# cloneofsimo/paint-with-words-sd

Measured on AMD Instinct MI355X. Metric: 512x512 images/sec (30 steps, CFG) SD1.5+PwW, higher is better.
Workload: dtype bf16

## Files before the change

paint-with-words-sd_amd/build.py:

```python
import os
import subprocess
import sys

HERE = os.path.dirname(os.path.abspath(__file__))
REPO = os.path.dirname(HERE)
CSRC = os.path.join(HERE, "csrc")
LIB = os.path.join(HERE, "pww_hip", "libpww_hip.so")
LIB_EXPERIMENTS = os.path.join(HERE, "pww_hip", "libpww_hip_experiments.so")
UNITS = [("pww_api.hip", [], ""), ("pww_attn.hip", [], ""), ("pww_cross.hip", [], ""), ("pww_cross_lean.hip", [], ""), ("pww_reduce.hip", [], ""),
         ("pww_mask.hip", [], ""), ("pww_qproj.hip", [], ""), ("pww_norm.hip", [], ""), ("pww_blocks.hip", [], ""), ("pww_conv.hip", [], ""), ("pww_probs.hip", [], ""),
         ("pww_attn_inst.hip", ["-DPWW_INST_F16"], ".f16"), ("pww_attn_inst.hip", ["-DPWW_INST_BF16"], ".bf16"),
         ("pww_cross_inst.hip", ["-DPWW_INST_F16", "-DPWW_INST_NW=2"], ".f16.nw2"), ("pww_cross_inst.hip", ["-DPWW_INST_F16", "-DPWW_INST_NW=4"], ".f16.nw4"),
         ("pww_cross_inst.hip", ["-DPWW_INST_BF16", "-DPWW_INST_NW=2"], ".bf16.nw2"), ("pww_cross_inst.hip", ["-DPWW_INST_BF16", "-DPWW_INST_NW=4"], ".bf16.nw4")]
EXPERIMENT_UNITS = [("pww_cross_out.hip", [], "")]
_ATTN_HEADERS = ["pww_tile.h", "pww_attn_core.h", "pww_cross_tile.h"]
SIDE_FLAGS = ["-fvisibility=hidden"]
SIDE_LIBS = {
    "long": ("pww_long.hip", _ATTN_HEADERS, "the long-prompt launches"),
    "scope": ("pww_scope.hip", _ATTN_HEADERS, "cross-attention with per-head / per-row score statistics"),
    "linear": ("pww_linear.hip", [], "linear layers with a bias / residual / GEGLU epilogue"),
    "regions": ("pww_regions.hip", [], "region masks and the per-pixel blend of the noise predictions"),
    "lora": ("pww_lora.hip", [], "the per-row low-rank update of unmerged LoRA adapters"),
}
SIDE_LIBS_CONV = {
    "convtail": ("pww_conv_tail.hip", [], "conv2 of a ResnetBlock2D with the 1 x 1 shortcut as further K-slabs"),
}
SIDE_LIBS_EXTRA = {
    "canvas": ("pww_canvas.hip", [], "canvases larger than the UNet's window: the windows' gather and the combine of their noise predictions"),
    "concat": ("pww_concat.hip", [], "the up blocks without torch.cat: GroupNorm and conv2 + shortcut over the two halves of the concatenation"),
    "hold": ("pww_hold.hip", [], "region strength: the strength map, its feather and the per-step hold of the pixels not yet released"),
}
ALL_SIDE_LIBS = {**SIDE_LIBS, **SIDE_LIBS_CONV, **SIDE_LIBS_EXTRA}
SOURCES = sorted({u[0] for u in UNITS + EXPERIMENT_UNITS})
HEADERS = ["pww_common.h", "pww_tile.h", "pww_attn_core.h", "pww_attn_kernel.h", "pww_cross_tile.h", "pww_cross_kernel.h", os.path.join(REPO, "include", "pww_hip.h")]
SIDE_PATHS = {n: os.path.join(HERE, "pww_hip", "libpww_hip_%s.so" % n) for n in ALL_SIDE_LIBS}
SIDE_UNITS = {n: [(v[0], SIDE_FLAGS, "")] for n, v in ALL_SIDE_LIBS.items()}
LIB_LONG, LIB_SCOPE, LIB_LINEAR, LIB_REGIONS, LIB_LORA = (SIDE_PATHS[n] for n in ("long", "scope", "linear", "regions", "lora"))
LONG_UNITS, SCOPE_UNITS, LINEAR_UNITS, REGIONS_UNITS, LORA_UNITS = (SIDE_UNITS[n] for n in ("long", "scope", "linear", "regions", "lora"))
LIB_CONVTAIL, CONVTAIL_UNITS = SIDE_PATHS["convtail"], SIDE_UNITS["convtail"]
LIB_CANVAS, CANVAS_UNITS = SIDE_PATHS["canvas"], SIDE_UNITS["canvas"]
LIB_CONCAT, CONCAT_UNITS = SIDE_PATHS["concat"], SIDE_UNITS["concat"]
LIB_HOLD, HOLD_UNITS = SIDE_PATHS["hold"], SIDE_UNITS["hold"]
SIDE_PUBLIC_HEADERS = {"canvas": ["pww_hip_regions.h"]}
HIPCC = os.environ.get("HIPCC", "/opt/rocm/bin/hipcc")
FLAGS = ["--offload-arch=gfx950", "-O3", "-std=c++17", "-fPIC", "-Wall",
         "-Wno-unused-function", "-mllvm", "-amdgpu-kernarg-preload-count=16"]


PER_FILE_FLAGS = {"pww_mask.hip": ["-ffp-contract=off"], "pww_regions.hip": ["-ffp-contract=off"], "pww_canvas.hip": ["-ffp-contract=off"],
                  "pww_hold.hip": ["-ffp-contract=off"]}


def _newer(target, deps):
    if not os.path.exists(target):
        return True
    t = os.path.getmtime(target)
    return any(os.path.getmtime(d) > t for d in deps)


def _deps():
    return ([os.path.join(CSRC, s) for s in SOURCES] + [h if os.path.isabs(h) else os.path.join(CSRC, h) for h in HEADERS] + [__file__])


def _build(lib, units, defines, objdir, verbose, jobs=None):
    os.makedirs(objdir, exist_ok=True)
    order = sorted(units, key=lambda u: {"pww_cross_inst.hip": 0, "pww_attn_inst.hip": 1, "pww_cross_lean.hip": 2}.get(u[0], 3))
    jobs = jobs or max(2, min(len(order), os.cpu_count() or 4, int(os.environ.get("MAX_JOBS", 16))))
    pending, running, objs = list(order), [], []
    while pending or running:
        while pending and len(running) < jobs:
            src, defs, suffix = pending.pop(0)
            o = os.path.join(objdir, src + suffix + ".o")
            objs.append(o)
            cmd = [HIPCC] + FLAGS + defines + defs + PER_FILE_FLAGS.get(src, []) + ["-c", os.path.join(CSRC, src), "-o", o]
            if verbose:
                print(" ".join(cmd))
            running.append((cmd, subprocess.Popen(cmd, stdout=subprocess.PIPE, stderr=subprocess.STDOUT, text=True)))
        cmd, p = running.pop(0)
        out, _ = p.communicate()
        if p.returncode != 0:
            for _, q in running:
                q.kill()
            raise RuntimeError("hipcc failed: %s\n%s" % (" ".join(cmd), out))
        if verbose and out.strip():
            print(out)
    subprocess.run([HIPCC, "--offload-arch=gfx950", "-shared", "-fPIC", "-s"] + sorted(objs) + ["-o", lib], check=True)
    return lib


def build_lib(force=False, verbose=False):
    if not force and not _newer(LIB, _deps()):
        return LIB
    return _build(LIB, UNITS, [], os.path.join(HERE, "build"), verbose)


def build_experiments(force=False, verbose=False):
    if not force and not _newer(LIB_EXPERIMENTS, _deps()):
        return LIB_EXPERIMENTS
    return _build(LIB_EXPERIMENTS, UNITS + EXPERIMENT_UNITS, ["-DPWW_EXPERIMENTS=1"], os.path.join(HERE, "build", "experiments"), verbose)


def build_side(name, force=False, verbose=False):
    unit, headers, _ = ALL_SIDE_LIBS[name]
    lib = SIDE_PATHS[name]
    public = ["pww_hip.h", "pww_hip_%s.h" % name] + SIDE_PUBLIC_HEADERS.get(name, [])
    deps = [os.path.join(CSRC, f) for f in [unit, "pww_common.h", "pww_side_host.h"] + headers] + [os.path.join(REPO, "include", h) for h in public] + [__file__]
    if not force and not _newer(lib, deps):
        return lib
    return _build(lib, SIDE_UNITS[name], [], os.path.join(HERE, "build", name), verbose)


def build_long(force=False, verbose=False): return build_side("long", force, verbose)
def build_scope(force=False, verbose=False): return build_side("scope", force, verbose)
def build_linear(force=False, verbose=False): return build_side("linear", force, verbose)
def build_regions(force=False, verbose=False): return build_side("regions", force, verbose)
def build_lora(force=False, verbose=False): return build_side("lora", force, verbose)
def build_convtail(force=False, verbose=False): return build_side("convtail", force, verbose)
def build_canvas(force=False, verbose=False): return build_side("canvas", force, verbose)
def build_concat(force=False, verbose=False): return build_side("concat", force, verbose)
def build_hold(force=False, verbose=False): return build_side("hold", force, verbose)


def _build_check(exe, lib, libname, defines, force):
    src = os.path.join(REPO, "tests", "native", "attn_check.cpp")
    if not force and not _newer(exe, [src, lib, os.path.join(REPO, "include", "pww_hip.h")]):
        return exe
    cmd = [HIPCC, "--offload-arch=gfx950", "-O2", "-std=c++17"] + defines + [src, "-o", exe, "-L" + os.path.dirname(lib), "-l" + libname,
                                                                              "-Wl,-rpath,$ORIGIN/../../paint-with-words-sd_amd/pww_hip"]
    subprocess.run(cmd, check=True)
    return exe


def build_native_check(force=False):
    return _build_check(os.path.join(REPO, "tests", "native", "attn_check"), build_lib(), "pww_hip", [], force)


def build_native_check_experiments(force=False):
    return _build_check(os.path.join(REPO, "tests", "native", "attn_check_experiments"), build_experiments(), "pww_hip_experiments", ["-DPWW_EXPERIMENTS=1"], force)


if __name__ == "__main__":
    force = "--force" in sys.argv
    print(build_lib(force=force, verbose=True))
    print(build_native_check(force=force))
    for name in ALL_SIDE_LIBS:
        print(build_side(name, force=force, verbose=True))
    if "--experiments" in sys.argv:
        print(build_experiments(force=force, verbose=True))
        print(build_native_check_experiments(force=force))
```

paint-with-words-sd_amd/csrc/pww_common.h:

```cpp
#pragma once
#include <hip/hip_runtime.h>
#include <hip/hip_ext.h>
#include <stdint.h>
#include <stdio.h>
#include <stdarg.h>
#include "../../include/pww_hip.h"

#ifndef PWW_EXPERIMENTS
#define PWW_EXPERIMENTS 0
#endif

namespace pww {

typedef _Float16 f16;
typedef __bf16 bf16;
typedef float f32x16 __attribute__((ext_vector_type(16)));
typedef _Float16 f16x8 __attribute__((ext_vector_type(8)));
typedef __bf16 bf16x8 __attribute__((ext_vector_type(8)));
typedef unsigned int u32x4 __attribute__((ext_vector_type(4)));
typedef unsigned int u32x2 __attribute__((ext_vector_type(2)));
typedef float f32x4 __attribute__((ext_vector_type(4)));
typedef _Float16 f16x4 __attribute__((ext_vector_type(4)));
typedef __bf16 bf16x4 __attribute__((ext_vector_type(4)));

template <typename T> struct Vec;
template <> struct Vec<f16> { typedef f16x8 v8; typedef f16x4 v4; };
template <> struct Vec<bf16> { typedef bf16x8 v8; typedef bf16x4 v4; };

__device__ __forceinline__ f32x16 mfma32(f16x8 a, f16x8 b, f32x16 c) {
    return __builtin_amdgcn_mfma_f32_32x32x16_f16(a, b, c, 0, 0, 0);
}
__device__ __forceinline__ f32x16 mfma32(bf16x8 a, bf16x8 b, f32x16 c) {
    return __builtin_amdgcn_mfma_f32_32x32x16_bf16(a, b, c, 0, 0, 0);
}

template <typename V8> __device__ __forceinline__ V8 zero8() {
    const u32x4 z = {0u, 0u, 0u, 0u};
    return __builtin_bit_cast(V8, z);
}

__device__ __forceinline__ int swap23(int i) { return (i & ~12) | ((i & 4) << 1) | ((i & 8) >> 1); }

struct DebugKnobs {
    int attn_rf = 1;
    int attn_ksplit = 1;
    int attn_fold = 1;
    int attn_nw8 = 1;
    int attn_pair_major = 16;
    int attn_head_pairs = 2;
    int cross_head_major = 1;
    int attn_wide_store = 1;
    int cross_wg_per_cu = 4;
    int cross_assume_resident = 0;
    int cross_gate_weight = 2;
    int cross_tile_nbuf = 2;
    int cross_bias_lds = 2;
    int cross_lean = 1;
    int cross_lean_multi = 1;
    int cross_lean_nw = 0;
    int attn_ksplit1 = 0;
    int attn_hot_sum = 8;
    int attn_fold_limit_f16 = 0;
    int attn_ksplit_half = 0;
    int attn_ksplit_nw = 2;
};
const DebugKnobs &debug_knobs();

void set_error(const char *fmt, ...);
int check_hip(hipError_t e, const char *what);
bool arch_ok();

bool profile_take(hipEvent_t *start, hipEvent_t *stop, hipStream_t stream);

unsigned long long *debug_timeline();
size_t debug_timeline_bytes();

void record_attn_route(int kind, int ks, int dt, int nw, int kg, int nsub, bool has_bias, bool rowsum_mfma, bool rf);

template <typename K, typename P>
static inline void launch_attn_kernel(K kern, dim3 grid, dim3 block, size_t lds, hipStream_t stream, const P &params) {
    hipEvent_t e0, e1;
    if (profile_take(&e0, &e1, stream)) hipExtLaunchKernelGGL(kern, grid, block, (unsigned)lds, stream, e0, e1, 0, params);
    else hipLaunchKernelGGL(kern, grid, block, lds, stream, params);
}

template <typename K, typename... A>
static inline void launch_timed(K kern, dim3 grid, dim3 block, size_t lds, hipStream_t stream, A... args) {
    hipEvent_t e0, e1;
    if (profile_take(&e0, &e1, stream)) hipExtLaunchKernelGGL(kern, grid, block, (unsigned)lds, stream, e0, e1, 0, args...);
    else hipLaunchKernelGGL(kern, grid, block, lds, stream, args...);
}

}
```

paint-with-words-sd_amd/csrc/pww_concat.hip:

```cpp
#define PWW_SIDE_LIB "libpww_hip_concat"
#include "pww_side_host.h"
#include "../../include/pww_hip_concat.h"

#define PWW_CONCAT_API extern "C" __attribute__((visibility("default")))

namespace pww {

namespace {

constexpr int GN_NT = 256;
constexpr int GN_UN = 8;
constexpr int GN_MAX_SLABS = 64;
constexpr int GN_GROUP_PIECES = 24;

struct CatGnCold {
    const void *gamma, *beta;
    void *y;
    float eps;
};
#define CG_KARGS const void *x1_, const void *x2_, double *partial_, int C1_, int C2_, int HW_, int G_, int cg_, int nslab_, int slab_px_, int apply_px_, const CatGnCold cold_
struct CatGnParams {
    const void *x1, *x2, *gamma, *beta;
    void *y;
    double *partial;
// ... 52 lines not shown
    const T *base = reinterpret_cast<const T *>(second ? p.x2 : p.x1);
    return base + (long)b * p.HW * pitch + (second ? c0 - p.C1 : c0);
}

template <typename T, int NT>
__global__ void __launch_bounds__(NT) cat_gn_moments(CG_KARGS) {
    CG_UNPACK
    extern __shared__ __attribute__((aligned(16))) char smem[];
    typedef typename Vec<T>::v8 V8;
    const int tid = threadIdx.x, b = blockIdx.y, slab = blockIdx.x;
    const int CH = p.C >> 3, PL = NT / CH;
    const int pl = tid / CH, ch = tid - pl * CH;
    float *ls = reinterpret_cast<float *>(smem);
    float *lq = ls + PL * p.C;
    double *lk = reinterpret_cast<double *>(lq + PL * p.C);

    if (pl < PL) {
        float s[8], q[8];
#pragma unroll
        for (int j = 0; j < 8; ++j) s[j] = q[j] = 0.f;
        int pitch;
        const T *x = cat_source<T>(p, b, ch * 8, pitch);
        float c = 0.f;
        const int p0 = slab * p.slab_px, p1 = min(p0 + p.slab_px, p.HW);
#pragma unroll 1
        for (int px = p0 + pl; px < p1; px += GN_UN * PL) {
            V8 r[GN_UN];
#pragma unroll
            for (int u = 0; u < GN_UN; ++u) {
                const int pu = px + u * PL;
                r[u] = *reinterpret_cast<const V8 *>(x + (long)(pu < p1 ? pu : px) * pitch);
            }
            if constexpr (GnPivot<T>::on) {
                if (px == p0 + pl) c = (float)r[0][0];
            }
#pragma unroll
            for (int u = 0; u < GN_UN; ++u) {
                const bool ok = px + u * PL < p1;
#pragma unroll
                for (int j = 0; j < 8; ++j) {
                    float h = (float)r[u][j];
                    if constexpr (GnPivot<T>::on) h -= c;
                    h = ok ? h : 0.f;
                    s[j] += h;
                    q[j] = fmaf(h, h, q[j]);
                }
            }
        }
#pragma unroll
        for (int j = 0; j < 8; ++j) { ls[pl * p.C + ch * 8 + j] = s[j]; lq[pl * p.C + ch * 8 + j] = q[j]; }
        if constexpr (GnPivot<T>::on) reinterpret_cast<float *>(lk + (NT / p.G) * p.G * 2)[tid] = c;
    }
    __syncthreads();
    const int K = NT / p.G, g = tid % p.G, k = tid / p.G;
    if (k < K) {
        double S = 0.0, Q = 0.0;
        const int n = PL * p.cg;
        for (int e = k; e < n; e += K) {
            const int r = e / p.cg, c = g * p.cg + (e - r * p.cg);
            if constexpr (GnPivot<T>::on) {
                const float *lc = reinterpret_cast<const float *>(lk + K * p.G * 2);
                const int p0 = slab * p.slab_px, p1 = min(p0 + p.slab_px, p.HW);
                const int cnt = p0 + r < p1 ? (p1 - p0 - r + PL - 1) / PL : 0;
                unpivot(S, Q, (double)ls[r * p.C + c], (double)lq[r * p.C + c], (double)lc[r * CH + (c >> 3)], (double)cnt);
            } else {
                S += (double)ls[r * p.C + c]; Q += (double)lq[r * p.C + c];
            }
        }
        lk[(k * p.G + g) * 2] = S; lk[(k * p.G + g) * 2 + 1] = Q;
    }
    __syncthreads();
    if (tid < p.G) {
        double S = 0.0, Q = 0.0;
        for (int r = 0; r < K; ++r) { S += lk[(r * p.G + tid) * 2]; Q += lk[(r * p.G + tid) * 2 + 1]; }
        f64x2 v; v[0] = S; v[1] = Q;
        reinterpret_cast<f64x2 *>(p.partial)[((long)b * p.nslab + slab) * p.G + tid] = v;
    }
}

template <typename T, int ACT, int NT>
__global__ void __launch_bounds__(NT) cat_gn_apply(CG_KARGS) {
    CG_UNPACK
    extern __shared__ __attribute__((aligned(16))) char smem[];
    typedef typename Vec<T>::v8 V8;
    constexpr int NPART = 8;
    const int tid = threadIdx.x, b = blockIdx.y;
    const int CH = p.C >> 3, PL = NT / CH;
    const int pl = tid / CH, ch = tid - pl * CH;
    const bool active = pl < PL;
    double *lk = reinterpret_cast<double *>(smem);
    const int K = NT / p.G, g = tid % p.G, k = tid / p.G;
    float *stat = reinterpret_cast<float *>(lk + K * p.G * 2);

    f64x2 part[NPART];
#pragma unroll
    for (int i = 0; i < NPART; ++i) {
        const int sl = k + i * K;
        part[i] = reinterpret_cast<const f64x2 *>(p.partial)[((long)b * p.nslab + (k < K && sl < p.nslab ? sl : 0)) * p.G + g];
    }
    const int c0 = ch * 8;
    V8 gv = zero8<V8>(), bv = zero8<V8>();
    int pitch;
    const T *x = cat_source<T>(p, b, c0, pitch);
    T *y = reinterpret_cast<T *>(p.y) + (long)b * p.HW * p.C + c0;
    const int p0 = blockIdx.x * p.apply_px, p1 = min(p0 + p.apply_px, p.HW);
    V8 r[GN_UN];
    if (active) {
        if (p.gamma) gv = *reinterpret_cast<const V8 *>(reinterpret_cast<const T *>(p.gamma) + c0);
        if (p.beta) bv = *reinterpret_cast<const V8 *>(reinterpret_cast<const T *>(p.beta) + c0);
#pragma unroll
        for (int u = 0; u < GN_UN; ++u) {
            const int pu = p0 + pl + u * PL;
            r[u] = *reinterpret_cast<const V8 *>(x + (long)(pu < p1 ? pu : p0) * pitch);
        }
    }
    if (k < K) {
        double S = 0.0, Q = 0.0;
#pragma unroll
        for (int i = 0; i < NPART; ++i)
            if (k + i * K < p.nslab) { S += part[i][0]; Q += part[i][1]; }
        lk[(k * p.G + g) * 2] = S; lk[(k * p.G + g) * 2 + 1] = Q;
    }
    __syncthreads();
    if (tid < p.G) {
        double S = 0.0, Q = 0.0;
        for (int rr = 0; rr < K; ++rr) { S += lk[(rr * p.G + tid) * 2]; Q += lk[(rr * p.G + tid) * 2 + 1]; }
        float mean, rstd;
        mean_rstd(S, Q, (double)p.cg * (double)p.HW, p.eps, mean, rstd);
        stat[tid * 2] = mean; stat[tid * 2 + 1] = rstd;
    }
    __syncthreads();
    if (!active) return;
    float a[8], bb[8];
#pragma unroll
    for (int j = 0; j < 8; ++j) {
        const int gg = (c0 + j) / p.cg;
        a[j] = stat[gg * 2 + 1] * (p.gamma ? (float)gv[j] : 1.f);
        bb[j] = (p.beta ? (float)bv[j] : 0.f) - a[j] * stat[gg * 2];
    }
    for (int px = p0 + pl; px < p1; px += GN_UN * PL) {
        if (px != p0 + pl) {
#pragma unroll
            for (int u = 0; u < GN_UN; ++u) {
                const int pu = px + u * PL;
                r[u] = *reinterpret_cast<const V8 *>(x + (long)(pu < p1 ? pu : px) * pitch);
            }
        }
#pragma unroll
        for (int u = 0; u < GN_UN; ++u) {
            V8 o;
#pragma unroll
            for (int j = 0; j < 8; ++j) o[j] = (T)finish<T, ACT>((float)r[u][j], a[j], bb[j]);
            if (px + u * PL < p1) *reinterpret_cast<V8 *>(y + (long)(px + u * PL) * p.C) = o;
        }
    }
}

template <typename T, int ACT>
__global__ void __launch_bounds__(GN_NT) cat_gn_group(CG_KARGS) {
    CG_UNPACK
    typedef T TV __attribute__((ext_vector_type(4)));
    __shared__ double red[GN_NT / 64][2];
    const int tid = threadIdx.x, g = blockIdx.x, b = blockIdx.y;
    const int ppp = p.cg >> 2, PLs = GN_NT / ppp;
    const int pl = tid / ppp, sub = tid - pl * ppp;
    const bool active = pl < PLs;
    const int pc = pl < p.HW ? pl : 0;
    const int c0 = g * p.cg + sub * 4;
    int pitch;
    const T *x = cat_source<T>(p, b, c0, pitch);
    T *y = reinterpret_cast<T *>(p.y) + (long)b * p.HW * p.C + c0;
    TV raw[GN_GROUP_PIECES];
    const TV z = {(T)0.f, (T)0.f, (T)0.f, (T)0.f};
    TV gv = z, bv = z;
    if (active) {
#pragma unroll
        for (int j = 0; j < GN_GROUP_PIECES; ++j) {
            const int px = pl + j * PLs;
            raw[j] = *reinterpret_cast<const TV *>(x + (long)(px < p.HW ? px : pc) * pitch);
        }
        if (p.gamma) gv = *reinterpret_cast<const TV *>(reinterpret_cast<const T *>(p.gamma) + c0);
        if (p.beta) bv = *reinterpret_cast<const TV *>(reinterpret_cast<const T *>(p.beta) + c0);
    }
    float v[GN_GROUP_PIECES][4];
    float s = 0.f, q = 0.f, c = 0.f;
    int cnt = 0;
    if (active) {
#pragma unroll
        for (int j = 0; j < GN_GROUP_PIECES; ++j) {
            const bool ok = pl + j * PLs < p.HW;
#pragma unroll
            for (int e = 0; e < 4; ++e) {
                float h = (float)raw[j][e];
                h = ok ? h : 0.f;
                v[j][e] = h;
                if constexpr (GnPivot<T>::on) {
                    if (j == 0 && e == 0) c = h;
                    h = ok ? h - c : 0.f;
                }
                s += h;
                q = fmaf(h, h, q);
            }
            if constexpr (GnPivot<T>::on) cnt += ok ? 4 : 0;
        }
    }
    double S = (double)s, Q = (double)q;
    if constexpr (GnPivot<T>::on) { S = 0.0; Q = 0.0; unpivot(S, Q, (double)s, (double)q, (double)c, (double)cnt); }
    wg_sum(S, Q, red, tid);
    float mean, rstd;
    mean_rstd(S, Q, (double)p.cg * (double)p.HW, p.eps, mean, rstd);
    if (!active) return;
    float a[4], bb[4];
#pragma unroll
    for (int e = 0; e < 4; ++e) {
        a[e] = rstd * (p.gamma ? (float)gv[e] : 1.f);
        bb[e] = (p.beta ? (float)bv[e] : 0.f) - a[e] * mean;
    }
#pragma unroll
    for (int j = 0; j < GN_GROUP_PIECES; ++j) {
        const int px = pl + j * PLs;
        if (px < p.HW) {
            TV o;
#pragma unroll
            for (int e = 0; e < 4; ++e) o[e] = (T)finish<T, ACT>(v[j][e], a[e], bb[e]);
            *reinterpret_cast<TV *>(y + (long)px * p.C) = o;
        }
    }
}

struct CatGnPlan { int nslab, slab_px, apply_px, nt; bool group; size_t partial_bytes, lds_m, lds_a; };

bool desc_ok(const void *d, uint32_t size, size_t want, const char *what) {
    if (d && size >= want) return true;
    set_error("%s: descriptor missing or older than this library (size %u)", what, d ? size : 0u);
    return false;
}

bool cat_gn_plan(const pww_concat_gn_desc_t *d, CatGnPlan &pl) {
    const long C = (long)d->C1 + d->C2;
    const bool ok = d->B >= 1 && d->B <= 65535 && d->C1 >= 8 && d->C2 >= 8 && d->C1 % 8 == 0 && d->C2 % 8 == 0 && C <= 4096 && d->HW >= 8 && d->HW % 8 == 0
                    && d->G >= 1 && d->G <= 32 && C % d->G == 0 && (d->dtype == PWW_DTYPE_F16 || d->dtype == PWW_DTYPE_BF16)
                    && (d->act == PWW_ACT_NONE || d->act == PWW_ACT_SILU) && (long)d->B * d->HW * C < (1L << 40);
    if (!ok) {
        set_error("concat_group_norm: unsupported (dtype %d B %d C1 %d C2 %d HW %d G %d act %d): C1, C2 and HW multiples of 8, (C1 + C2) %% G == 0, "
                  "G <= 32, C1 + C2 <= 4096", d->dtype, d->B, d->C1, d->C2, d->HW, d->G, d->act);
        return false;
    }
    pl = CatGnPlan();
    const int Ct = (int)C, cg = Ct / d->G, CH = Ct / 8;
    pl.nt = CH <= 256 ? 256 : 512;
    const int PL = pl.nt / CH;
    if (cg % 4 == 0 && cg / 4 <= GN_NT) {
        const int PLs = GN_NT / (cg / 4);
        pl.group = (d->HW + PLs - 1) / PLs <= GN_GROUP_PIECES;
    }
    int px = (d->HW + GN_MAX_SLABS - 1) / GN_MAX_SLABS;
    if (px < GN_UN * PL) px = GN_UN * PL;
    if (px > d->HW) px = d->HW;
    pl.slab_px = px;
    pl.nslab = (d->HW + px - 1) / px;
    int want = (512 + d->B - 1) / d->B;
    int apx = (d->HW + want - 1) / want;
    if (apx < GN_UN * PL) apx = GN_UN * PL;
    if (apx > d->HW) apx = d->HW;
    pl.apply_px = apx;
    pl.partial_bytes = (size_t)d->B * pl.nslab * d->G * 2 * sizeof(double);
    const size_t lk = (size_t)(pl.nt / d->G) * d->G * 2 * sizeof(double);
    pl.lds_m = (size_t)2 * PL * Ct * sizeof(float) + lk + (d->dtype == PWW_DTYPE_F16 ? (size_t)pl.nt * sizeof(float) : 0);
    pl.lds_a = lk + (size_t)d->G * 2 * sizeof(float);
    return true;
}

template <typename T>
int cat_gn_launch(const CatGnParams &p, const pww_concat_gn_desc_t *d, const CatGnPlan &pl, hipStream_t stream) {
    const bool silu = d->act == PWW_ACT_SILU;
    if (pl.group) {
        const dim3 grid(d->G, d->B);
        if (silu) hipLaunchKernelGGL((cat_gn_group<T, 1>), grid, dim3(GN_NT), 0, stream, CG_LARGS(p));
        else hipLaunchKernelGGL((cat_gn_group<T, 0>), grid, dim3(GN_NT), 0, stream, CG_LARGS(p));
        return check_hip(hipGetLastError(), "concat_group_norm launch");
    }
    const dim3 gm(pl.nslab, d->B), ga((d->HW + pl.apply_px - 1) / pl.apply_px, d->B);
    if (pl.nt == 256) {
        hipLaunchKernelGGL((cat_gn_moments<T, 256>), gm, dim3(256), pl.lds_m, stream, CG_LARGS(p));
        if (silu) hipLaunchKernelGGL((cat_gn_apply<T, 1, 256>), ga, dim3(256), pl.lds_a, stream, CG_LARGS(p));
        else hipLaunchKernelGGL((cat_gn_apply<T, 0, 256>), ga, dim3(256), pl.lds_a, stream, CG_LARGS(p));
    } else {
        hipLaunchKernelGGL((cat_gn_moments<T, 512>), gm, dim3(512), pl.lds_m, stream, CG_LARGS(p));
        if (silu) hipLaunchKernelGGL((cat_gn_apply<T, 1, 512>), ga, dim3(512), pl.lds_a, stream, CG_LARGS(p));
        else hipLaunchKernelGGL((cat_gn_apply<T, 0, 512>), ga, dim3(512), pl.lds_a, stream, CG_LARGS(p));
    }
    return check_hip(hipGetLastError(), "concat_group_norm launch");
}

constexpr int CT_BM = 128, CT_THREADS = 256;
constexpr int CT_PF = 2;

__device__ __forceinline__ f32x4 mfma16(f16x8 a, f16x8 b, f32x4 c) { return __builtin_amdgcn_mfma_f32_16x16x32_f16(a, b, c, 0, 0, 0); }
__device__ __forceinline__ f32x4 mfma16(bf16x8 a, bf16x8 b, f32x4 c) { return __builtin_amdgcn_mfma_f32_16x16x32_bf16(a, b, c, 0, 0, 0); }

struct CatTailCold {
    const void *x1, *x2, *wsc, *bias, *bias2;
    int nsplit, nmain, ntail;
};

__device__ __forceinline__ int xcd_remap(int orig, int nwg) {
    const int xcd = orig & 7, q = nwg >> 3, r = nwg & 7;
    return (xcd < r ? xcd * (q + 1) : r * (q + 1) + (xcd - r) * q) + (orig >> 3);
}

template <typename T>
__device__ __forceinline__ void epilogue4(const f32x4 &a, const CatTailCold &cold, T *y, long off, int n) {
    typedef typename Vec<T>::v4 V4;
    const V4 b = *reinterpret_cast<const V4 *>(reinterpret_cast<const T *>(cold.bias) + n);
    const V4 b2 = *reinterpret_cast<const V4 *>(reinterpret_cast<const T *>(cold.bias2) + n);
    V4 o;
#pragma unroll
    for (int j = 0; j < 4; ++j) o[j] = (T)(a[j] + (float)b[j] + (float)b2[j]);
    *reinterpret_cast<V4 *>(y + off) = o;
}

template <typename T, int BN>
__global__ void __launch_bounds__(CT_THREADS, 2) cat_tail_kernel(const T *__restrict__ x, const T *__restrict__ w, void *__restrict__ out, int M, int N,
                                                                 int Cin, int C1, int C2, int H, int W, const CatTailCold cold) {
    typedef typename Vec<T>::v8 V8;
    constexpr int BM = CT_BM, PF = CT_PF, XL = BM * 8 / CT_THREADS, WL = BN * 8 / CT_THREADS, RM = 4, RN = BN / 32;
    constexpr int XBYTES = BM * 128, STAGE = (BM + BN) * 128;
    __shared__ __attribute__((aligned(16))) char lds[2 * STAGE];

    const int tid = threadIdx.x, lane = tid & 63, wave = tid >> 6, wm = wave >> 1, wn = wave & 1;
    const int ntm = (M + BM - 1) / BM;
    const int bid = xcd_remap(blockIdx.x, gridDim.x);
    const bool split = cold.nsplit > 1;
    const int tile = bid / cold.nsplit, ks = bid - tile * cold.nsplit;
    const int tm = tile % ntm, tn = tile / ntm;
    const int nmain = cold.nmain, nslab = nmain + cold.ntail;
    const int s_begin = (int)((long)ks * nslab / cold.nsplit), s_end = (int)((long)(ks + 1) * nslab / cold.nsplit);
    const int K9 = 9 * Cin, HW = H * W, Ct = C1 + C2;
    const T *__restrict__ xa = reinterpret_cast<const T *>(cold.x1);
    const T *__restrict__ xb2 = reinterpret_cast<const T *>(cold.x2);
    const T *__restrict__ w2 = reinterpret_cast<const T *>(cold.wsc);

    const int c = tid & 7;
    int pix[XL], y0[XL], x0[XL];
#pragma unroll
    for (int i = 0; i < XL; ++i) {
        int m = tm * BM + (tid >> 3) + 32 * i;
        m = m < M ? m : M - 1;
        const int b = m / HW, rem = m - b * HW, oy = rem / W, ox = rem - oy * W;
        pix[i] = b * HW;
        y0[i] = oy - 1;
        x0[i] = ox - 1;
    }
    const unsigned wrow = (unsigned)(tn * BN + (tid >> 3));
    const unsigned woff_main = wrow * (unsigned)K9 + c * 8, woff_tail = wrow * (unsigned)Ct + c * 8;
    const int swz = ((c ^ ((tid >> 3) & 7)) << 4);

    u32x4 xr[PF][XL], wr[PF][WL];
    unsigned xok[PF];
    const bool tail0 = s_begin >= nmain;
    int tap = tail0 ? 9 : s_begin / (Cin >> 6);
    int ci0 = tail0 ? (s_begin - nmain) << 6 : (s_begin - tap * (Cin >> 6)) << 6;
    int kmain = s_begin * 64;
    const bool second0 = tail0 && ci0 >= C1;
    const T *xs = second0 ? xb2 - C1 : xa;
    int ps = second0 ? C2 : C1;
    auto load = [&](int p) {
        const bool tail = tap >= 9;
        const int ky = tail ? 1 : tap / 3, kx = tail ? 1 : tap - (tap / 3) * 3;
        const T *xb = tail ? xs : x;
        const T *wb = tail ? w2 : w;
        const int pitch = tail ? ps : Cin;
        const unsigned wpitch = (unsigned)(tail ? Ct : K9);
        const unsigned wo = (tail ? woff_tail : woff_main) + (unsigned)(tail ? ci0 : kmain);
        xok[p] = 0;
#pragma unroll
        for (int i = 0; i < XL; ++i) {
            const int iy = y0[i] + ky, ix = x0[i] + kx;
            const bool ok = (unsigned)iy < (unsigned)H && (unsigned)ix < (unsigned)W;
            xr[p][i] = *reinterpret_cast<const u32x4 *>(xb + (unsigned)((pix[i] + (ok ? iy : 0) * W + (ok ? ix : 0)) * pitch + ci0 + c * 8));
            xok[p] |= (unsigned)ok << i;
        }
#pragma unroll
        for (int j = 0; j < WL; ++j) wr[p][j] = *reinterpret_cast<const u32x4 *>(wb + (wo + (unsigned)(32 * j) * wpitch));
        kmain += 64;
        ci0 += 64;
        const bool wrap = ci0 == Cin && !tail;
        ci0 = wrap ? 0 : ci0;
        tap += wrap ? 1 : 0;
        const bool cross = ci0 == C1 && tail;
        xs = cross ? xb2 - C1 : xs;
        ps = cross ? C2 : ps;
    };
    auto store = [&](int p, int buf) {
        char *base = lds + buf * STAGE;
#pragma unroll
        for (int i = 0; i < XL; ++i) {
            const u32x4 z = {0u, 0u, 0u, 0u};
            *reinterpret_cast<u32x4 *>(base + ((tid >> 3) + 32 * i) * 128 + swz) = (xok[p] >> i) & 1u ? xr[p][i] : z;
        }
#pragma unroll
        for (int j = 0; j < WL; ++j) *reinterpret_cast<u32x4 *>(base + XBYTES + ((tid >> 3) + 32 * j) * 128 + swz) = wr[p][j];
    };

    f32x4 acc[RN][RM];
#pragma unroll
    for (int r = 0; r < RN; ++r)
#pragma unroll
        for (int i = 0; i < RM; ++i) acc[r][i] = f32x4{0.f, 0.f, 0.f, 0.f};

    const int fr = lane & 15, fq = lane >> 4;
    auto compute = [&](int buf) {
        const char *bx = lds + buf * STAGE, *bw = bx + XBYTES;
#pragma unroll
        for (int kk = 0; kk < 2; ++kk) {
            V8 xf[RM], wf[RN];
#pragma unroll
            for (int q = 0; q < RM; ++q) {
                const int row = wm * 64 + q * 16 + fr;
                xf[q] = *reinterpret_cast<const V8 *>(bx + row * 128 + (((kk * 4 + fq) ^ (row & 7)) << 4));
            }
#pragma unroll
            for (int r = 0; r < RN; ++r) {
                const int row = wn * (BN / 2) + r * 16 + fr;
                wf[r] = *reinterpret_cast<const V8 *>(bw + row * 128 + (((kk * 4 + fq) ^ (row & 7)) << 4));
            }
#pragma unroll
            for (int r = 0; r < RN; ++r)
#pragma unroll
                for (int q = 0; q < RM; ++q) acc[r][q] = mfma16(wf[r], xf[q], acc[r][q]);
        }
    };

    const int n = s_end - s_begin;
    load(0);
#pragma unroll
    for (int p = 1; p < PF; ++p)
        if (p < n) load(p);
    store(0, 0);
    __syncthreads();
    int i = 0;
    for (; i + 2 * PF <= n; i += PF) {
#pragma unroll
        for (int p = 0; p < PF; ++p) {
            load(p);
            compute((i + p) & 1);
            __builtin_amdgcn_sched_barrier(0);
            store((p + 1) % PF, (i + p + 1) & 1);
            __syncthreads();
        }
    }
#pragma unroll
    for (int t = 0; t < 2 * PF - 1; ++t) {
        if (i + t < n) {
            if (i + t + PF < n) load(t % PF);
            compute((i + t) & 1);
            if (i + t + 1 < n) store((t + 1) % PF, (i + t + 1) & 1);
            __syncthreads();
        }
    }

#pragma unroll
    for (int i = 0; i < RM; ++i) {
        const int m = tm * BM + wm * 64 + i * 16 + fr;
        if (m >= M) continue;
#pragma unroll
        for (int r = 0; r < RN; ++r) {
            const int n = tn * BN + wn * (BN / 2) + r * 16 + fq * 4;
            if (split) *reinterpret_cast<f32x4 *>(reinterpret_cast<float *>(out) + ((long)ks * M + m) * N + n) = acc[r][i];
            else epilogue4<T>(acc[r][i], cold, reinterpret_cast<T *>(out), (long)m * N + n, n);
        }
    }
}

template <typename T>
__global__ void __launch_bounds__(256) cat_tail_fold_kernel(const float *__restrict__ ws, T *__restrict__ y, long n4, int N, long MN, const CatTailCold cold) {
    const long q = (long)blockIdx.x * 256 + threadIdx.x;
    if (q >= n4) return;
    const long off = q * 4;
    f32x4 a = *reinterpret_cast<const f32x4 *>(ws + off);
    for (int s = 1; s < cold.nsplit; ++s) a += *reinterpret_cast<const f32x4 *>(ws + s * MN + off);
    epilogue4<T>(a, cold, y, off, (int)(off % N));
}

struct TailTune { int M, N, nmain, ntail, bn, nsplit; };
constexpr TailTune TAIL_TUNED[] = {
    {128, 1280, 180, 40, 64, 12},
    {512, 1280, 180, 40, 128, 12}, {512, 1280, 180, 30, 128, 12}, {512, 1280, 180, 10, 128, 12},
    {2048, 640, 90, 30, 128, 6}, {2048, 640, 90, 20, 128, 6}, {2048, 640, 90, 15, 128, 6}, {2048, 640, 90, 5, 128, 6},
    {8192, 320, 45, 15, 64, 4}, {8192, 320, 45, 10, 64, 4},
};

struct TailPlan {
    int M, bn, nsplit, nmain, ntail, ntiles;
};

bool cat_tail_plan(const pww_concat_tail_desc_t *d, TailPlan *p) {
    if ((d->dtype != PWW_DTYPE_F16 && d->dtype != PWW_DTYPE_BF16) || d->B < 1 || d->H < 1 || d->W < 1 || d->Cin < 64 || d->Cin % 64 != 0 || d->C1 < 64
        || d->C1 % 64 != 0 || d->C2 < 64 || d->C2 % 64 != 0 || d->Cout < 64 || d->Cout % 64 != 0 || d->Cin > 65536 || d->C1 > 32768 || d->C2 > 32768
        || d->Cout > 65536) {
        set_error("concat_convtail: unsupported (dtype %d B %d %dx%d Cin %d C1 %d C2 %d Cout %d): Cin, C1, C2 and Cout multiples of 64", d->dtype, d->B,
                  d->H, d->W, d->Cin, d->C1, d->C2, d->Cout);
        return false;
    }
    const long M = (long)d->B * d->H * d->W, Ct = (long)d->C1 + d->C2;
    if (M * d->Cin >= (1L << 31) || M * Ct >= (1L << 31) || M * d->Cout >= (1L << 31) || 9L * d->Cin * d->Cout >= (1L << 31) || Ct * d->Cout >= (1L << 31)) {
        set_error("concat_convtail: tensor of 2^31 elements or more");
        return false;
    }
    p->M = (int)M;
    p->nmain = 9 * d->Cin / 64;
    p->ntail = (int)(Ct / 64);
    const int nslab = p->nmain + p->ntail;
    const TailTune *tuned = nullptr;
    for (const TailTune &t : TAIL_TUNED)
        if (t.M == p->M && t.N == d->Cout && t.nmain == p->nmain && t.ntail == p->ntail) tuned = &t;
    p->bn = d->tile_n ? d->tile_n : tuned ? tuned->bn : (d->Cout % 128 == 0 ? 128 : 64);
    if ((p->bn != 64 && p->bn != 128) || d->Cout % p->bn != 0) { set_error("concat_convtail: tile_n %d does not divide Cout %d", d->tile_n, d->Cout); return false; }
    p->ntiles = (p->M + CT_BM - 1) / CT_BM * (d->Cout / p->bn);
    int ns = d->splitk;
    if (ns <= 0 && tuned && p->bn == tuned->bn) ns = tuned->nsplit;
    if (ns <= 0) {
        ns = (480 + p->ntiles / 2) / p->ntiles;
        if (ns > nslab / 8) ns = nslab / 8;
        if (ns < 1) ns = 1;
    }
    if (ns > nslab || ns > 64) { set_error("concat_convtail: split %d exceeds the %d K-slabs (or 64)", ns, nslab); return false; }
    p->nsplit = ns;
    return true;
}

template <typename T>
int cat_tail_launch(const TailPlan &p, const pww_concat_tail_desc_t *d, const void *x, const void *w, const CatTailCold &cold, void *y, void *ws,
                    hipStream_t stream) {
    const T *xt = static_cast<const T *>(x), *wt = static_cast<const T *>(w);
    const int N = d->Cout;
    const dim3 grid(p.ntiles * p.nsplit), block(CT_THREADS);
    void *out = p.nsplit == 1 ? y : ws;
    if (p.bn == 128) launch_timed(cat_tail_kernel<T, 128>, grid, block, 0, stream, xt, wt, out, p.M, N, d->Cin, d->C1, d->C2, d->H, d->W, cold);
    else launch_timed(cat_tail_kernel<T, 64>, grid, block, 0, stream, xt, wt, out, p.M, N, d->Cin, d->C1, d->C2, d->H, d->W, cold);
    if (p.nsplit == 1) return check_hip(hipGetLastError(), "concat_convtail launch");
    const long MN = (long)p.M * N, n4 = MN / 4;
    launch_timed(cat_tail_fold_kernel<T>, dim3((unsigned)((n4 + 255) / 256)), dim3(256), 0, stream, static_cast<const float *>(ws), static_cast<T *>(y), n4,
                 N, MN, cold);
    return check_hip(hipGetLastError(), "concat_convtail fold launch");
}

}

size_t concat_group_norm_workspace_bytes(const pww_concat_gn_desc_t *d) {
    CatGnPlan pl;
    if (!desc_ok(d, d ? d->size : 0u, sizeof(pww_concat_gn_desc_t), "concat_group_norm") || !cat_gn_plan(d, pl)) return 0;
    return pl.group ? 16 : pl.partial_bytes;
}

int concat_group_norm_fwd(const void *x1, const void *x2, const void *gamma, const void *beta, void *y, const pww_concat_gn_desc_t *d, void *workspace,
                          size_t workspace_bytes, hipStream_t stream) {
    if (!desc_ok(d, d ? d->size : 0u, sizeof(pww_concat_gn_desc_t), "concat_group_norm")) return PWW_EINVAL;
    CatGnPlan pl;
    if (!cat_gn_plan(d, pl)) return PWW_ENOTSUP;
    if (!x1 || !x2 || !y || !workspace) { set_error("concat_group_norm: x1, x2, y and workspace are required"); return PWW_EINVAL; }
    if (!aligned16(x1) || !aligned16(x2) || !aligned16(y) || !aligned16(workspace) || !aligned16(gamma) || !aligned16(beta)) {
        set_error("concat_group_norm: pointers must be 16-byte aligned");
        return PWW_EINVAL;
    }
    const size_t need = pl.group ? 16 : pl.partial_bytes;
    if (workspace_bytes < need) { set_error("concat_group_norm: workspace of %zu bytes, need %zu", workspace_bytes, need); return PWW_EINVAL; }
    if (!arch_ok()) return PWW_ENOTSUP;
    CatGnParams p;
    p.x1 = x1; p.x2 = x2; p.gamma = gamma; p.beta = beta; p.y = y;
    p.partial = static_cast<double *>(workspace);
    p.C1 = d->C1; p.C2 = d->C2; p.C = d->C1 + d->C2; p.HW = d->HW; p.G = d->G; p.cg = p.C / d->G;
    p.nslab = pl.nslab; p.slab_px = pl.slab_px; p.apply_px = pl.apply_px;
    p.eps = d->eps;
    return d->dtype == PWW_DTYPE_F16 ? cat_gn_launch<f16>(p, d, pl, stream) : cat_gn_launch<bf16>(p, d, pl, stream);
}

size_t concat_convtail_workspace_bytes(const pww_concat_tail_desc_t *d) {
    TailPlan p;
    if (!desc_ok(d, d ? d->size : 0u, sizeof(pww_concat_tail_desc_t), "concat_convtail") || !cat_tail_plan(d, &p)) return 0;
    return p.nsplit > 1 ? (size_t)p.nsplit * p.M * d->Cout * sizeof(float) : 0;
}

int concat_convtail_fwd(const void *x, const void *w, const void *x1, const void *x2, const void *wsc, const void *bias, const void *bias2, void *y,
                        const pww_concat_tail_desc_t *d, void *workspace, size_t workspace_bytes, hipStream_t stream) {
    if (!desc_ok(d, d ? d->size : 0u, sizeof(pww_concat_tail_desc_t), "concat_convtail")) return PWW_EINVAL;
    TailPlan p;
    if (!cat_tail_plan(d, &p)) return PWW_ENOTSUP;
    if (!x || !w || !x1 || !x2 || !wsc || !bias || !bias2 || !y) { set_error("concat_convtail: x, w, x1, x2, wsc, bias, bias2 and y are required"); return PWW_EINVAL; }
    if (!aligned16(x) || !aligned16(w) || !aligned16(x1) || !aligned16(x2) || !aligned16(wsc) || !aligned16(y) || (reinterpret_cast<uintptr_t>(bias) & 7)
        || (reinterpret_cast<uintptr_t>(bias2) & 7)) {
        set_error("concat_convtail: x, w, x1, x2, wsc, y must be 16-byte aligned, the biases 8-byte aligned");
        return PWW_EINVAL;
    }
    const size_t need = p.nsplit > 1 ? (size_t)p.nsplit * p.M * d->Cout * sizeof(float) : 0;
    if (need && (!workspace || !aligned16(workspace) || workspace_bytes < need)) {
        set_error("concat_convtail: split %d needs a 16-byte aligned workspace of %zu bytes (got %zu)", p.nsplit, need, workspace_bytes);
        return PWW_EINVAL;
    }
    if (!arch_ok()) return PWW_ENOTSUP;
    const CatTailCold cold{x1, x2, wsc, bias, bias2, p.nsplit, p.nmain, p.ntail};
    if (d->dtype == PWW_DTYPE_F16) return cat_tail_launch<f16>(p, d, x, w, cold, y, workspace, stream);
    return cat_tail_launch<bf16>(p, d, x, w, cold, y, workspace, stream);
}

}

PWW_CONCAT_API int pww_concat_version(void) { return PWW_CONCAT_VERSION; }
PWW_CONCAT_API const char *pww_concat_last_error(void) { return pww::last_error(); }
PWW_CONCAT_API size_t pww_concat_group_norm_workspace_bytes(const pww_concat_gn_desc_t *desc) { return pww::concat_group_norm_workspace_bytes(desc); }
PWW_CONCAT_API int pww_concat_group_norm_fwd(const void *x1, const void *x2, const void *gamma, const void *beta, void *y, const pww_concat_gn_desc_t *desc,
                                             void *workspace, size_t workspace_bytes, void *stream) {
    return pww::concat_group_norm_fwd(x1, x2, gamma, beta, y, desc, workspace, workspace_bytes, static_cast<hipStream_t>(stream));
}
PWW_CONCAT_API size_t pww_concat_convtail_workspace_bytes(const pww_concat_tail_desc_t *desc) { return pww::concat_convtail_workspace_bytes(desc); }
PWW_CONCAT_API int pww_concat_convtail_fwd(const void *x, const void *w, const void *x1, const void *x2, const void *wsc, const void *bias, const void *bias2,
                                           void *y, const pww_concat_tail_desc_t *desc, void *workspace, size_t workspace_bytes, void *stream) {
    return pww::concat_convtail_fwd(x, w, x1, x2, wsc, bias, bias2, y, desc, workspace, workspace_bytes, static_cast<hipStream_t>(stream));
}
```

paint-with-words-sd_amd/csrc/pww_conv.hip:

```cpp
#include "pww_common.h"

namespace pww {

namespace {

constexpr int CV_BM = 128, CV_THREADS = 256;
constexpr int CV_PF = 2;

__device__ __forceinline__ f32x4 mfma16(f16x8 a, f16x8 b, f32x4 c) { return __builtin_amdgcn_mfma_f32_16x16x32_f16(a, b, c, 0, 0, 0); }
__device__ __forceinline__ f32x4 mfma16(bf16x8 a, bf16x8 b, f32x4 c) { return __builtin_amdgcn_mfma_f32_16x16x32_bf16(a, b, c, 0, 0, 0); }

struct ConvCold {
    const void *bias, *residual;
    int nsplit, nslab;
};

__device__ __forceinline__ int xcd_remap(int orig, int nwg) {
    const int xcd = orig & 7, q = nwg >> 3, r = nwg & 7;
    return (xcd < r ? xcd * (q + 1) : r * (q + 1) + (xcd - r) * q) + (orig >> 3);
}

template <typename T>
__device__ __forceinline__ void epilogue4(const f32x4 &a, const ConvCold &cold, T *y, long off, int n) {
    typedef typename Vec<T>::v4 V4;
    V4 o;
#pragma unroll
    for (int j = 0; j < 4; ++j) o[j] = (T)a[j];
    if (cold.bias) {
        const V4 b = *reinterpret_cast<const V4 *>(reinterpret_cast<const T *>(cold.bias) + n);
#pragma unroll
        for (int j = 0; j < 4; ++j) o[j] = (T)((float)o[j] + (float)b[j]);
    }
    if (cold.residual) {
        const V4 r = *reinterpret_cast<const V4 *>(reinterpret_cast<const T *>(cold.residual) + off);
#pragma unroll
        for (int j = 0; j < 4; ++j) o[j] = (T)((float)r[j] + (float)o[j]);
    }
    *reinterpret_cast<V4 *>(y + off) = o;
}

template <typename T, int BN>
__global__ void __launch_bounds__(CV_THREADS, 2) conv3x3_kernel(const T *__restrict__ x, const T *__restrict__ w, void *__restrict__ out, int M, int N,
                                                            int Cin, int Hin, int Win, int Wo, int HWo, const ConvCold cold) {
    typedef typename Vec<T>::v8 V8;
    constexpr int BM = CV_BM, PF = CV_PF, XL = BM * 8 / CV_THREADS, WL = BN * 8 / CV_THREADS, RM = 4, RN = BN / 32;
    constexpr int XBYTES = BM * 128, STAGE = (BM + BN) * 128;
    __shared__ __attribute__((aligned(16))) char lds[2 * STAGE];

    const int geo = cold.nslab >> 24;
    const int nslab = cold.nslab & 0xffffff;
    const int stride = geo & 15, up = geo >> 4;
    const int Hv = Hin << up, Wv = Win << up;
    const int tid = threadIdx.x, lane = tid & 63, wave = tid >> 6, wm = wave >> 1, wn = wave & 1;
    const int ntm = (M + BM - 1) / BM;
    const int bid = xcd_remap(blockIdx.x, gridDim.x);
    const bool split = cold.nsplit > 1;
    const int tile = bid / cold.nsplit, ks = bid - tile * cold.nsplit;
    const int tm = tile % ntm, tn = tile / ntm;
    const int s_begin = (int)((long)ks * nslab / cold.nsplit), s_end = (int)((long)(ks + 1) * nslab / cold.nsplit);
    const int K9 = 9 * Cin;

    const int c = tid & 7;
    int pix[XL], y0[XL], x0[XL];
#pragma unroll
    for (int i = 0; i < XL; ++i) {
        int m = tm * BM + (tid >> 3) + 32 * i;
        m = m < M ? m : M - 1;
        const int b = m / HWo, rem = m - b * HWo, oy = rem / Wo, ox = rem - oy * Wo;
        pix[i] = b * Hin * Win;
        y0[i] = oy * stride - 1;
        x0[i] = ox * stride - 1;
    }
    const T *wrow = w + (long)(tn * BN + (tid >> 3)) * K9 + c * 8;
    const int swz = ((c ^ ((tid >> 3) & 7)) << 4);

    u32x4 xr[PF][XL], wr[PF][WL];
    unsigned xok[PF];
    int tap = s_begin / (Cin >> 6), ci0 = (s_begin - tap * (Cin >> 6)) << 6;
    const T *wnext = wrow + s_begin * 64;
    auto load = [&](int p) {
        const int ky = tap / 3, kx = tap - ky * 3;
        xok[p] = 0;
#pragma unroll
        for (int i = 0; i < XL; ++i) {
            const int iyv = y0[i] + ky, ixv = x0[i] + kx;
            const bool ok = (unsigned)iyv < (unsigned)Hv && (unsigned)ixv < (unsigned)Wv;
            const int iy = ok ? iyv >> up : 0, ix = ok ? ixv >> up : 0;
            xr[p][i] = *reinterpret_cast<const u32x4 *>(x + (unsigned)((pix[i] + iy * Win + ix) * Cin + ci0 + c * 8));
            xok[p] |= (unsigned)ok << i;
        }
#pragma unroll
        for (int j = 0; j < WL; ++j) wr[p][j] = *reinterpret_cast<const u32x4 *>(wnext + (long)(32 * j) * K9);
        wnext += 64;
        ci0 += 64;
        if (ci0 == Cin) { ci0 = 0; ++tap; }
    };
    auto store = [&](int p, int buf) {
        char *base = lds + buf * STAGE;
#pragma unroll
        for (int i = 0; i < XL; ++i) {
            const u32x4 z = {0u, 0u, 0u, 0u};
            *reinterpret_cast<u32x4 *>(base + ((tid >> 3) + 32 * i) * 128 + swz) = (xok[p] >> i) & 1u ? xr[p][i] : z;
        }
#pragma unroll
        for (int j = 0; j < WL; ++j) *reinterpret_cast<u32x4 *>(base + XBYTES + ((tid >> 3) + 32 * j) * 128 + swz) = wr[p][j];
    };

    f32x4 acc[RN][RM];
#pragma unroll
    for (int r = 0; r < RN; ++r)
#pragma unroll
        for (int i = 0; i < RM; ++i) acc[r][i] = f32x4{0.f, 0.f, 0.f, 0.f};

    const int fr = lane & 15, fq = lane >> 4;
    auto compute = [&](int buf) {
        const char *bx = lds + buf * STAGE, *bw = bx + XBYTES;
#pragma unroll
        for (int kk = 0; kk < 2; ++kk) {
            V8 xf[RM], wf[RN];
#pragma unroll
            for (int q = 0; q < RM; ++q) {
                const int row = wm * 64 + q * 16 + fr;
                xf[q] = *reinterpret_cast<const V8 *>(bx + row * 128 + (((kk * 4 + fq) ^ (row & 7)) << 4));
            }
#pragma unroll
            for (int r = 0; r < RN; ++r) {
                const int row = wn * (BN / 2) + r * 16 + fr;
                wf[r] = *reinterpret_cast<const V8 *>(bw + row * 128 + (((kk * 4 + fq) ^ (row & 7)) << 4));
            }
#pragma unroll
            for (int r = 0; r < RN; ++r)
#pragma unroll
                for (int q = 0; q < RM; ++q) acc[r][q] = mfma16(wf[r], xf[q], acc[r][q]);
        }
    };

    const int n = s_end - s_begin;
    load(0);
#pragma unroll
    for (int p = 1; p < PF; ++p)
        if (p < n) load(p);
    store(0, 0);
    __syncthreads();
    int i = 0;
    for (; i + 2 * PF <= n; i += PF) {
#pragma unroll
        for (int p = 0; p < PF; ++p) {
            load(p);
            compute((i + p) & 1);
            store((p + 1) % PF, (i + p + 1) & 1);
            __syncthreads();
        }
    }
#pragma unroll
    for (int t = 0; t < 2 * PF - 1; ++t) {
        if (i + t < n) {
            if (i + t + PF < n) load(t % PF);
            compute((i + t) & 1);
            if (i + t + 1 < n) store((t + 1) % PF, (i + t + 1) & 1);
            __syncthreads();
        }
    }

#pragma unroll
    for (int i = 0; i < RM; ++i) {
        const int m = tm * BM + wm * 64 + i * 16 + fr;
        if (m >= M) continue;
#pragma unroll
        for (int r = 0; r < RN; ++r) {
            const int n = tn * BN + wn * (BN / 2) + r * 16 + fq * 4;
            if (split) *reinterpret_cast<f32x4 *>(reinterpret_cast<float *>(out) + ((long)ks * M + m) * N + n) = acc[r][i];
            else epilogue4<T>(acc[r][i], cold, reinterpret_cast<T *>(out), (long)m * N + n, n);
        }
    }
}

template <typename T>
__global__ void __launch_bounds__(256) conv3x3_fold_kernel(const float *__restrict__ ws, T *__restrict__ y, long n4, int N, long MN, const ConvCold cold) {
    const long q = (long)blockIdx.x * 256 + threadIdx.x;
    if (q >= n4) return;
    const long off = q * 4;
    f32x4 a = *reinterpret_cast<const f32x4 *>(ws + off);
    for (int s = 1; s < cold.nsplit; ++s) a += *reinterpret_cast<const f32x4 *>(ws + s * MN + off);
    epilogue4<T>(a, cold, y, off, (int)(off % N));
}

struct ConvTune { int M, N, nslab, bn, nsplit; };
constexpr ConvTune CONV_TUNED[] = {
    {8192, 320, 45, 64, 3}, {8192, 320, 90, 64, 4}, {8192, 320, 135, 64, 3}, {8192, 640, 90, 128, 3},
    {2048, 320, 45, 64, 6}, {2048, 640, 45, 64, 3}, {2048, 640, 90, 128, 6}, {2048, 640, 135, 128, 6}, {2048, 640, 180, 128, 6},
    {2048, 640, 270, 128, 6}, {2048, 1280, 180, 128, 3},
    {512, 640, 90, 64, 6}, {512, 1280, 90, 128, 6}, {512, 1280, 180, 128, 12}, {512, 1280, 270, 128, 12}, {512, 1280, 360, 128, 12},
    {128, 1280, 180, 64, 12}, {128, 1280, 360, 64, 24},
    {65536, 640, 90, 128, 1}, {16384, 1280, 180, 128, 1},
    {4096, 640, 90, 128, 3}, {4096, 1280, 90, 128, 3}, {4096, 1280, 180, 128, 3}, {4096, 1280, 270, 128, 3}, {4096, 1280, 360, 128, 3},
    {1024, 1280, 180, 128, 6}, {1024, 1280, 360, 128, 6},
};

struct ConvPlan {
    int M, Ho, Wo, bn, nsplit, nslab, ntiles;
};

bool plan_conv(const pww_conv_desc_t *d, ConvPlan *p) {
    if (!d || d->size < sizeof(pww_conv_desc_t)) { set_error("conv3x3: descriptor missing or older than this library (size %u)", d ? d->size : 0u); return false; }
    const int up = d->upsample, s = d->stride;
    if ((d->dtype != PWW_DTYPE_F16 && d->dtype != PWW_DTYPE_BF16) || d->B < 1 || d->Hin < 1 || d->Win < 1 || d->Cin < 64 || d->Cin % 64 != 0
        || d->Cout < 64 || d->Cout % 64 != 0 || (s != 1 && s != 2) || (up != 0 && up != 1) || (up && s != 1) || d->Cin > 65536 || d->Cout > 65536) {
        set_error("conv3x3: unsupported (dtype %d B %d %dx%d Cin %d Cout %d stride %d upsample %d): Cin and Cout multiples of 64, stride 1 or 2, "
                  "upsample only at stride 1", d->dtype, d->B, d->Hin, d->Win, d->Cin, d->Cout, s, up);
        return false;
    }
    const int Hv = d->Hin << up, Wv = d->Win << up;
    p->Ho = (Hv - 1) / s + 1;
    p->Wo = (Wv - 1) / s + 1;
    const long M = (long)d->B * p->Ho * p->Wo;
    if ((long)d->B * d->Hin * d->Win * d->Cin >= (1L << 31) || M * d->Cout >= (1L << 31)) { set_error("conv3x3: tensor of 2^31 elements or more"); return false; }
    p->M = (int)M;
    p->nslab = 9 * d->Cin / 64;
    const ConvTune *tuned = nullptr;
    for (const ConvTune &t : CONV_TUNED)
        if (t.M == p->M && t.N == d->Cout && t.nslab == p->nslab) tuned = &t;
    p->bn = d->tile_n ? d->tile_n : tuned ? tuned->bn : (d->Cout % 128 == 0 ? 128 : 64);
    if ((p->bn != 64 && p->bn != 128) || d->Cout % p->bn != 0) { set_error("conv3x3: tile_n %d does not divide Cout %d", d->tile_n, d->Cout); return false; }
    p->ntiles = (p->M + CV_BM - 1) / CV_BM * (d->Cout / p->bn);
    int ns = d->splitk;
    if (ns <= 0 && tuned && p->bn == tuned->bn) ns = tuned->nsplit;
    if (ns <= 0) {
        ns = (480 + p->ntiles / 2) / p->ntiles;
        if (ns > p->nslab / 8) ns = p->nslab / 8;
        if (ns < 1) ns = 1;
    }
    if (ns > p->nslab || ns > 64) { set_error("conv3x3: split %d exceeds the %d K-slabs (or 64)", ns, p->nslab); return false; }
    p->nsplit = ns;
    return true;
}

template <typename T>
int conv_launch(const ConvPlan &p, const pww_conv_desc_t *d, const void *x, const void *w, const void *bias, const void *residual, void *y, void *ws,
                hipStream_t stream) {
    ConvCold cold{bias, residual, p.nsplit, p.nslab | ((d->stride | (d->upsample << 4)) << 24)};
    const T *xt = static_cast<const T *>(x), *wt = static_cast<const T *>(w);
    const int N = d->Cout, HWo = p.Ho * p.Wo;
    const dim3 grid(p.ntiles * p.nsplit), block(CV_THREADS);
    void *out = p.nsplit == 1 ? y : ws;
    if (p.bn == 128) launch_timed(conv3x3_kernel<T, 128>, grid, block, 0, stream, xt, wt, out, p.M, N, d->Cin, d->Hin, d->Win, p.Wo, HWo, cold);
    else launch_timed(conv3x3_kernel<T, 64>, grid, block, 0, stream, xt, wt, out, p.M, N, d->Cin, d->Hin, d->Win, p.Wo, HWo, cold);
    if (p.nsplit == 1) return check_hip(hipGetLastError(), "conv3x3 launch");
    const long MN = (long)p.M * N, n4 = MN / 4;
    launch_timed(conv3x3_fold_kernel<T>, dim3((unsigned)((n4 + 255) / 256)), dim3(256), 0, stream, static_cast<const float *>(ws), static_cast<T *>(y), n4,
                 N, MN, cold);
    return check_hip(hipGetLastError(), "conv3x3 fold launch");
}

bool al16(const void *a) { return (reinterpret_cast<uintptr_t>(a) & 15) == 0; }

}

size_t conv3x3_workspace_bytes(const pww_conv_desc_t *d) {
    ConvPlan p;
    if (!plan_conv(d, &p)) return 0;
    return p.nsplit > 1 ? (size_t)p.nsplit * p.M * d->Cout * sizeof(float) : 0;
}

int conv3x3_fwd(const void *x, const void *w, const void *bias, const void *residual, void *y, const pww_conv_desc_t *d, void *workspace,
                size_t workspace_bytes, hipStream_t stream) {
    ConvPlan p;
    if (!plan_conv(d, &p)) return PWW_ENOTSUP;
    if (!x || !w || !y) { set_error("conv3x3: x, w and y are required"); return PWW_EINVAL; }
    if (!al16(x) || !al16(w) || !al16(y) || (reinterpret_cast<uintptr_t>(bias) & 7) || (reinterpret_cast<uintptr_t>(residual) & 7)) {
        set_error("conv3x3: x, w, y must be 16-byte aligned, bias and residual 8-byte aligned");
        return PWW_EINVAL;
    }
    if (p.nsplit > 1 && (!workspace || !al16(workspace) || workspace_bytes < (size_t)p.nsplit * p.M * d->Cout * sizeof(float))) {
        set_error("conv3x3: split %d needs a 16-byte aligned workspace of %zu bytes (got %zu)", p.nsplit, (size_t)p.nsplit * p.M * d->Cout * sizeof(float),
                  workspace_bytes);
        return PWW_EINVAL;
    }
    if (!arch_ok()) return PWW_ENOTSUP;
    if (d->dtype == PWW_DTYPE_F16) return conv_launch<f16>(p, d, x, w, bias, residual, y, workspace, stream);
    return conv_launch<bf16>(p, d, x, w, bias, residual, y, workspace, stream);
}

}
```

paint-with-words-sd_amd/csrc/pww_conv_tail.hip:

```cpp
#define PWW_SIDE_LIB "libpww_hip_convtail"
#include "pww_side_host.h"
#include "../../include/pww_hip_convtail.h"

#define PWW_CONVTAIL_API extern "C" __attribute__((visibility("default")))

namespace pww {

namespace {

constexpr int CT_BM = 128, CT_THREADS = 256;
constexpr int CT_PF = 2;

__device__ __forceinline__ f32x4 mfma16(f16x8 a, f16x8 b, f32x4 c) { return __builtin_amdgcn_mfma_f32_16x16x32_f16(a, b, c, 0, 0, 0); }
__device__ __forceinline__ f32x4 mfma16(bf16x8 a, bf16x8 b, f32x4 c) { return __builtin_amdgcn_mfma_f32_16x16x32_bf16(a, b, c, 0, 0, 0); }

struct TailCold {
    const void *x2, *w2, *bias, *bias2;
    int nsplit, nmain, ntail;
};

__device__ __forceinline__ int xcd_remap(int orig, int nwg) {
    const int xcd = orig & 7, q = nwg >> 3, r = nwg & 7;
    return (xcd < r ? xcd * (q + 1) : r * (q + 1) + (xcd - r) * q) + (orig >> 3);
}

template <typename T>
__device__ __forceinline__ void epilogue4(const f32x4 &a, const TailCold &cold, T *y, long off, int n) {
    typedef typename Vec<T>::v4 V4;
    const V4 b = *reinterpret_cast<const V4 *>(reinterpret_cast<const T *>(cold.bias) + n);
    const V4 b2 = *reinterpret_cast<const V4 *>(reinterpret_cast<const T *>(cold.bias2) + n);
    V4 o;
#pragma unroll
    for (int j = 0; j < 4; ++j) o[j] = (T)(a[j] + (float)b[j] + (float)b2[j]);
    *reinterpret_cast<V4 *>(y + off) = o;
}

template <typename T, int BN>
__global__ void __launch_bounds__(CT_THREADS, 2) convtail_kernel(const T *__restrict__ x, const T *__restrict__ w, void *__restrict__ out, int M, int N,
                                                                 int Cin, int C2, int H, int W, const TailCold cold) {
    typedef typename Vec<T>::v8 V8;
    constexpr int BM = CT_BM, PF = CT_PF, XL = BM * 8 / CT_THREADS, WL = BN * 8 / CT_THREADS, RM = 4, RN = BN / 32;
    constexpr int XBYTES = BM * 128, STAGE = (BM + BN) * 128;
    __shared__ __attribute__((aligned(16))) char lds[2 * STAGE];

    const int tid = threadIdx.x, lane = tid & 63, wave = tid >> 6, wm = wave >> 1, wn = wave & 1;
    const int ntm = (M + BM - 1) / BM;
    const int bid = xcd_remap(blockIdx.x, gridDim.x);
    const bool split = cold.nsplit > 1;
    const int tile = bid / cold.nsplit, ks = bid - tile * cold.nsplit;
    const int tm = tile % ntm, tn = tile / ntm;
    const int nmain = cold.nmain, nslab = nmain + cold.ntail;
    const int s_begin = (int)((long)ks * nslab / cold.nsplit), s_end = (int)((long)(ks + 1) * nslab / cold.nsplit);
    const int K9 = 9 * Cin, HW = H * W;
    const T *__restrict__ x2 = reinterpret_cast<const T *>(cold.x2);
    const T *__restrict__ w2 = reinterpret_cast<const T *>(cold.w2);

    const int c = tid & 7;
    int pix[XL], y0[XL], x0[XL];
#pragma unroll
    for (int i = 0; i < XL; ++i) {
        int m = tm * BM + (tid >> 3) + 32 * i;
        m = m < M ? m : M - 1;
        const int b = m / HW, rem = m - b * HW, oy = rem / W, ox = rem - oy * W;
        pix[i] = b * HW;
        y0[i] = oy - 1;
        x0[i] = ox - 1;
    }
    const unsigned wrow = (unsigned)(tn * BN + (tid >> 3));
    const unsigned woff_main = wrow * (unsigned)K9 + c * 8, woff_tail = wrow * (unsigned)C2 + c * 8;
    const int swz = ((c ^ ((tid >> 3) & 7)) << 4);

    u32x4 xr[PF][XL], wr[PF][WL];
    unsigned xok[PF];
    const bool tail0 = s_begin >= nmain;
    int tap = tail0 ? 9 : s_begin / (Cin >> 6);
    int ci0 = tail0 ? (s_begin - nmain) << 6 : (s_begin - tap * (Cin >> 6)) << 6;
    int kmain = s_begin * 64;
    auto load = [&](int p) {
        const bool tail = tap >= 9;
        const int ky = tail ? 1 : tap / 3, kx = tail ? 1 : tap - (tap / 3) * 3;
        const T *xb = tail ? x2 : x;
        const T *wb = tail ? w2 : w;
        const int pitch = tail ? C2 : Cin;
        const unsigned wpitch = (unsigned)(tail ? C2 : K9);
        const unsigned wo = (tail ? woff_tail : woff_main) + (unsigned)(tail ? ci0 : kmain);
        xok[p] = 0;
#pragma unroll
        for (int i = 0; i < XL; ++i) {
            const int iy = y0[i] + ky, ix = x0[i] + kx;
            const bool ok = (unsigned)iy < (unsigned)H && (unsigned)ix < (unsigned)W;
            xr[p][i] = *reinterpret_cast<const u32x4 *>(xb + (unsigned)((pix[i] + (ok ? iy : 0) * W + (ok ? ix : 0)) * pitch + ci0 + c * 8));
            xok[p] |= (unsigned)ok << i;
        }
#pragma unroll
        for (int j = 0; j < WL; ++j) wr[p][j] = *reinterpret_cast<const u32x4 *>(wb + (wo + (unsigned)(32 * j) * wpitch));
        kmain += 64;
        ci0 += 64;
        const bool wrap = ci0 == Cin && !tail;
        ci0 = wrap ? 0 : ci0;
        tap += wrap ? 1 : 0;
    };
    auto store = [&](int p, int buf) {
        char *base = lds + buf * STAGE;
#pragma unroll
        for (int i = 0; i < XL; ++i) {
            const u32x4 z = {0u, 0u, 0u, 0u};
            *reinterpret_cast<u32x4 *>(base + ((tid >> 3) + 32 * i) * 128 + swz) = (xok[p] >> i) & 1u ? xr[p][i] : z;
        }
#pragma unroll
        for (int j = 0; j < WL; ++j) *reinterpret_cast<u32x4 *>(base + XBYTES + ((tid >> 3) + 32 * j) * 128 + swz) = wr[p][j];
    };

    f32x4 acc[RN][RM];
#pragma unroll
    for (int r = 0; r < RN; ++r)
#pragma unroll
        for (int i = 0; i < RM; ++i) acc[r][i] = f32x4{0.f, 0.f, 0.f, 0.f};

    const int fr = lane & 15, fq = lane >> 4;
    auto compute = [&](int buf) {
        const char *bx = lds + buf * STAGE, *bw = bx + XBYTES;
#pragma unroll
        for (int kk = 0; kk < 2; ++kk) {
            V8 xf[RM], wf[RN];
#pragma unroll
            for (int q = 0; q < RM; ++q) {
                const int row = wm * 64 + q * 16 + fr;
                xf[q] = *reinterpret_cast<const V8 *>(bx + row * 128 + (((kk * 4 + fq) ^ (row & 7)) << 4));
            }
#pragma unroll
            for (int r = 0; r < RN; ++r) {
                const int row = wn * (BN / 2) + r * 16 + fr;
                wf[r] = *reinterpret_cast<const V8 *>(bw + row * 128 + (((kk * 4 + fq) ^ (row & 7)) << 4));
            }
#pragma unroll
            for (int r = 0; r < RN; ++r)
#pragma unroll
                for (int q = 0; q < RM; ++q) acc[r][q] = mfma16(wf[r], xf[q], acc[r][q]);
        }
    };

    const int n = s_end - s_begin;
    load(0);
#pragma unroll
    for (int p = 1; p < PF; ++p)
        if (p < n) load(p);
    store(0, 0);
    __syncthreads();
    int i = 0;
    for (; i + 2 * PF <= n; i += PF) {
#pragma unroll
        for (int p = 0; p < PF; ++p) {
            load(p);
            compute((i + p) & 1);
            __builtin_amdgcn_sched_barrier(0);
            store((p + 1) % PF, (i + p + 1) & 1);
            __syncthreads();
        }
    }
#pragma unroll
    for (int t = 0; t < 2 * PF - 1; ++t) {
        if (i + t < n) {
            if (i + t + PF < n) load(t % PF);
            compute((i + t) & 1);
            if (i + t + 1 < n) store((t + 1) % PF, (i + t + 1) & 1);
            __syncthreads();
        }
    }

#pragma unroll
    for (int i = 0; i < RM; ++i) {
        const int m = tm * BM + wm * 64 + i * 16 + fr;
        if (m >= M) continue;
#pragma unroll
        for (int r = 0; r < RN; ++r) {
            const int n = tn * BN + wn * (BN / 2) + r * 16 + fq * 4;
            if (split) *reinterpret_cast<f32x4 *>(reinterpret_cast<float *>(out) + ((long)ks * M + m) * N + n) = acc[r][i];
            else epilogue4<T>(acc[r][i], cold, reinterpret_cast<T *>(out), (long)m * N + n, n);
        }
    }
}

template <typename T>
__global__ void __launch_bounds__(256) convtail_fold_kernel(const float *__restrict__ ws, T *__restrict__ y, long n4, int N, long MN, const TailCold cold) {
    const long q = (long)blockIdx.x * 256 + threadIdx.x;
    if (q >= n4) return;
    const long off = q * 4;
    f32x4 a = *reinterpret_cast<const f32x4 *>(ws + off);
    for (int s = 1; s < cold.nsplit; ++s) a += *reinterpret_cast<const f32x4 *>(ws + s * MN + off);
    epilogue4<T>(a, cold, y, off, (int)(off % N));
}

struct TailTune { int M, N, nmain, ntail, bn, nsplit; };
constexpr TailTune TAIL_TUNED[] = {
    {128, 1280, 180, 40, 64, 12},
    {512, 1280, 180, 40, 128, 12}, {512, 1280, 180, 30, 128, 12}, {512, 1280, 180, 10, 128, 12},
    {2048, 640, 90, 30, 128, 6}, {2048, 640, 90, 20, 128, 6}, {2048, 640, 90, 15, 128, 6}, {2048, 640, 90, 5, 128, 6},
    {8192, 320, 45, 15, 64, 4}, {8192, 320, 45, 10, 64, 4},
};

struct TailPlan {
    int M, bn, nsplit, nmain, ntail, ntiles;
};

bool plan_tail(const pww_convtail_desc_t *d, TailPlan *p) {
    if (!d || d->size < sizeof(pww_convtail_desc_t)) { set_error("convtail: descriptor missing or older than this library (size %u)", d ? d->size : 0u); return false; }
    if ((d->dtype != PWW_DTYPE_F16 && d->dtype != PWW_DTYPE_BF16) || d->B < 1 || d->H < 1 || d->W < 1 || d->Cin < 64 || d->Cin % 64 != 0 || d->C2 < 64
        || d->C2 % 64 != 0 || d->Cout < 64 || d->Cout % 64 != 0 || d->Cin > 65536 || d->C2 > 65536 || d->Cout > 65536) {
        set_error("convtail: unsupported (dtype %d B %d %dx%d Cin %d C2 %d Cout %d): Cin, C2 and Cout multiples of 64", d->dtype, d->B, d->H, d->W, d->Cin,
                  d->C2, d->Cout);
        return false;
    }
    const long M = (long)d->B * d->H * d->W;
    if (M * d->Cin >= (1L << 31) || M * d->C2 >= (1L << 31) || M * d->Cout >= (1L << 31) || 9L * d->Cin * d->Cout >= (1L << 31)
        || (long)d->C2 * d->Cout >= (1L << 31)) {
        set_error("convtail: tensor of 2^31 elements or more");
        return false;
    }
    p->M = (int)M;
    p->nmain = 9 * d->Cin / 64;
    p->ntail = d->C2 / 64;
    const int nslab = p->nmain + p->ntail;
    const TailTune *tuned = nullptr;
    for (const TailTune &t : TAIL_TUNED)
        if (t.M == p->M && t.N == d->Cout && t.nmain == p->nmain && t.ntail == p->ntail) tuned = &t;
    p->bn = d->tile_n ? d->tile_n : tuned ? tuned->bn : (d->Cout % 128 == 0 ? 128 : 64);
    if ((p->bn != 64 && p->bn != 128) || d->Cout % p->bn != 0) { set_error("convtail: tile_n %d does not divide Cout %d", d->tile_n, d->Cout); return false; }
    p->ntiles = (p->M + CT_BM - 1) / CT_BM * (d->Cout / p->bn);
    int ns = d->splitk;
    if (ns <= 0 && tuned && p->bn == tuned->bn) ns = tuned->nsplit;
    if (ns <= 0) {
        ns = (480 + p->ntiles / 2) / p->ntiles;
        if (ns > nslab / 8) ns = nslab / 8;
        if (ns < 1) ns = 1;
    }
    if (ns > nslab || ns > 64) { set_error("convtail: split %d exceeds the %d K-slabs (or 64)", ns, nslab); return false; }
    p->nsplit = ns;
    return true;
}

template <typename T>
int tail_launch(const TailPlan &p, const pww_convtail_desc_t *d, const void *x, const void *w, const void *x2, const void *w2, const void *bias,
                const void *bias2, void *y, void *ws, hipStream_t stream) {
    TailCold cold{x2, w2, bias, bias2, p.nsplit, p.nmain, p.ntail};
    const T *xt = static_cast<const T *>(x), *wt = static_cast<const T *>(w);
    const int N = d->Cout;
    const dim3 grid(p.ntiles * p.nsplit), block(CT_THREADS);
    void *out = p.nsplit == 1 ? y : ws;
    if (p.bn == 128) launch_timed(convtail_kernel<T, 128>, grid, block, 0, stream, xt, wt, out, p.M, N, d->Cin, d->C2, d->H, d->W, cold);
    else launch_timed(convtail_kernel<T, 64>, grid, block, 0, stream, xt, wt, out, p.M, N, d->Cin, d->C2, d->H, d->W, cold);
    if (p.nsplit == 1) return check_hip(hipGetLastError(), "convtail launch");
    const long MN = (long)p.M * N, n4 = MN / 4;
    launch_timed(convtail_fold_kernel<T>, dim3((unsigned)((n4 + 255) / 256)), dim3(256), 0, stream, static_cast<const float *>(ws), static_cast<T *>(y), n4,
                 N, MN, cold);
    return check_hip(hipGetLastError(), "convtail fold launch");
}

}

size_t convtail_workspace_bytes(const pww_convtail_desc_t *d) {
    TailPlan p;
    if (!plan_tail(d, &p)) return 0;
    return p.nsplit > 1 ? (size_t)p.nsplit * p.M * d->Cout * sizeof(float) : 0;
}

int convtail_fwd(const void *x, const void *w, const void *x2, const void *w2, const void *bias, const void *bias2, void *y, const pww_convtail_desc_t *d,
                 void *workspace, size_t workspace_bytes, hipStream_t stream) {
    if (!d || d->size < sizeof(pww_convtail_desc_t)) { set_error("convtail: descriptor missing or older than this library (size %u)", d ? d->size : 0u); return PWW_EINVAL; }
    TailPlan p;
    if (!plan_tail(d, &p)) return PWW_ENOTSUP;
    if (!x || !w || !x2 || !w2 || !bias || !bias2 || !y) { set_error("convtail: x, w, x2, w2, bias, bias2 and y are required"); return PWW_EINVAL; }
    if (!aligned16(x) || !aligned16(w) || !aligned16(x2) || !aligned16(w2) || !aligned16(y) || (reinterpret_cast<uintptr_t>(bias) & 7)
        || (reinterpret_cast<uintptr_t>(bias2) & 7)) {
        set_error("convtail: x, w, x2, w2, y must be 16-byte aligned, the biases 8-byte aligned");
        return PWW_EINVAL;
    }
    const size_t need = p.nsplit > 1 ? (size_t)p.nsplit * p.M * d->Cout * sizeof(float) : 0;
    if (need && (!workspace || !aligned16(workspace) || workspace_bytes < need)) {
        set_error("convtail: split %d needs a 16-byte aligned workspace of %zu bytes (got %zu)", p.nsplit, need, workspace_bytes);
        return PWW_EINVAL;
    }
    if (!arch_ok()) return PWW_ENOTSUP;
    if (d->dtype == PWW_DTYPE_F16) return tail_launch<f16>(p, d, x, w, x2, w2, bias, bias2, y, workspace, stream);
    return tail_launch<bf16>(p, d, x, w, x2, w2, bias, bias2, y, workspace, stream);
}

}

PWW_CONVTAIL_API int pww_convtail_version(void) { return PWW_CONVTAIL_VERSION; }
PWW_CONVTAIL_API const char *pww_convtail_last_error(void) { return pww::last_error(); }
PWW_CONVTAIL_API size_t pww_convtail_workspace_bytes(const pww_convtail_desc_t *desc) { return pww::convtail_workspace_bytes(desc); }
PWW_CONVTAIL_API int pww_convtail_fwd(const void *x, const void *w, const void *x2, const void *w2, const void *bias, const void *bias2, void *y,
                                      const pww_convtail_desc_t *desc, void *workspace, size_t workspace_bytes, void *stream) {
    return pww::convtail_fwd(x, w, x2, w2, bias, bias2, y, desc, workspace, workspace_bytes, static_cast<hipStream_t>(stream));
}
```

paint-with-words-sd_amd/csrc/pww_linear.hip:

```cpp
#define PWW_SIDE_LIB "libpww_hip_linear"
#include "pww_side_host.h"
#include "../../include/pww_hip_linear.h"

#define PWW_LINEAR_API extern "C" __attribute__((visibility("default")))

namespace pww {

namespace {

constexpr int LN_BM = 128, LN_THREADS = 256;
constexpr int LN_PF = 2;

__device__ __forceinline__ f32x4 mfma16(f16x8 a, f16x8 b, f32x4 c) { return __builtin_amdgcn_mfma_f32_16x16x32_f16(a, b, c, 0, 0, 0); }
__device__ __forceinline__ f32x4 mfma16(bf16x8 a, bf16x8 b, f32x4 c) { return __builtin_amdgcn_mfma_f32_16x16x32_bf16(a, b, c, 0, 0, 0); }

struct LinCold {
    const void *bias, *residual;
    long ys, rs;
    int nsplit, nslab, mode, inner;
};

__device__ __forceinline__ int xcd_remap(int orig, int nwg) {
    const int xcd = orig & 7, q = nwg >> 3, r = nwg & 7;
    return (xcd < r ? xcd * (q + 1) : r * (q + 1) + (xcd - r) * q) + (orig >> 3);
}

template <typename T> __device__ __forceinline__ float rnd(float v) { return (float)(T)v; }

template <typename T>
__device__ __forceinline__ void epilogue4(const f32x4 &a, const LinCold &cold, T *y, int m, int n) {
    typedef typename Vec<T>::v4 V4;
    V4 o;
#pragma unroll
    for (int j = 0; j < 4; ++j) o[j] = (T)a[j];
    if (cold.mode >= PWW_LINEAR_BIAS) {
        const V4 b = *reinterpret_cast<const V4 *>(reinterpret_cast<const T *>(cold.bias) + n);
#pragma unroll
        for (int j = 0; j < 4; ++j) o[j] = (T)((float)o[j] + (float)b[j]);
    }
    if (cold.mode == PWW_LINEAR_BIAS_RESIDUAL) {
        const V4 r = *reinterpret_cast<const V4 *>(reinterpret_cast<const T *>(cold.residual) + (long)m * cold.rs + n);
#pragma unroll
        for (int j = 0; j < 4; ++j) o[j] = (T)((float)r[j] + (float)o[j]);
    }
    *reinterpret_cast<V4 *>(y + (long)m * cold.ys + n) = o;
}

template <typename T>
__device__ __forceinline__ void geglu4(const f32x4 &av, const f32x4 &ag, const LinCold &cold, T *y, int m, int j0) {
    typedef typename Vec<T>::v4 V4;
    const V4 bv = *reinterpret_cast<const V4 *>(reinterpret_cast<const T *>(cold.bias) + j0);
    const V4 bg = *reinterpret_cast<const V4 *>(reinterpret_cast<const T *>(cold.bias) + cold.inner + j0);
    V4 o;
#pragma unroll
    for (int j = 0; j < 4; ++j) {
        const float hv = rnd<T>(rnd<T>(av[j]) + (float)bv[j]);
        const float g = rnd<T>(rnd<T>(ag[j]) + (float)bg[j]);
        const float ge = rnd<T>(0.5f * g * (1.f + erff(g * 0.70710678118654752440f)));
        o[j] = (T)(hv * ge);
    }
    *reinterpret_cast<V4 *>(y + (long)m * cold.ys + j0) = o;
}

template <typename T, int BN>
__global__ void __launch_bounds__(LN_THREADS, 2) linear_kernel(const T *__restrict__ x, const T *__restrict__ w, void *out, int M, int N, int K, int xs,
                                                               const LinCold cold) {
    typedef typename Vec<T>::v8 V8;
    constexpr int BM = LN_BM, PF = LN_PF, XL = BM * 8 / LN_THREADS, WL = BN * 8 / LN_THREADS, RM = 4, RN = BN / 32;
    constexpr int XBYTES = BM * 128, STAGE = (BM + BN) * 128;
    __shared__ __attribute__((aligned(16))) char lds[2 * STAGE];

    const int tid = threadIdx.x, lane = tid & 63, wave = tid >> 6, wm = wave >> 1, wn = wave & 1;
    const int ntm = (M + BM - 1) / BM;
    const int bid = xcd_remap(blockIdx.x, gridDim.x);
    const bool split = cold.nsplit > 1;
    const bool geglu = cold.mode == PWW_LINEAR_BIAS_GEGLU;
    const int tile = bid / cold.nsplit, ks = bid - tile * cold.nsplit;
    const int tm = tile % ntm, tn = tile / ntm;
    const int s_begin = (int)((long)ks * cold.nslab / cold.nsplit), s_end = (int)((long)(ks + 1) * cold.nslab / cold.nsplit);

    const int c = tid & 7;
    unsigned xoff[XL], woff[WL];
#pragma unroll
    for (int i = 0; i < XL; ++i) {
        int m = tm * BM + (tid >> 3) + 32 * i;
        m = m < M ? m : M - 1;
        xoff[i] = (unsigned)(m * xs + c * 8);
    }
#pragma unroll
    for (int j = 0; j < WL; ++j) {
        const int t = (tid >> 3) + 32 * j;
        const int u = t % (BN / 2);
        const int row = geglu ? (u >= BN / 4 ? cold.inner : 0) + tn * (BN / 2) + (t / (BN / 2)) * (BN / 4) + u % (BN / 4) : tn * BN + t;
        woff[j] = (unsigned)(row * K + c * 8);
    }
    const int swz = ((c ^ ((tid >> 3) & 7)) << 4);

    u32x4 xr[PF][XL], wr[PF][WL];
    const T *xnext = x + s_begin * 64, *wnext = w + s_begin * 64;
    auto load = [&](int p) {
#pragma unroll
        for (int i = 0; i < XL; ++i) xr[p][i] = *reinterpret_cast<const u32x4 *>(xnext + xoff[i]);
#pragma unroll
        for (int j = 0; j < WL; ++j) wr[p][j] = *reinterpret_cast<const u32x4 *>(wnext + woff[j]);
        xnext += 64;
        wnext += 64;
    };
    auto store = [&](int p, int buf) {
        char *base = lds + buf * STAGE;
#pragma unroll
        for (int i = 0; i < XL; ++i) *reinterpret_cast<u32x4 *>(base + ((tid >> 3) + 32 * i) * 128 + swz) = xr[p][i];
#pragma unroll
        for (int j = 0; j < WL; ++j) *reinterpret_cast<u32x4 *>(base + XBYTES + ((tid >> 3) + 32 * j) * 128 + swz) = wr[p][j];
    };

    f32x4 acc[RN][RM];
#pragma unroll
    for (int r = 0; r < RN; ++r)
#pragma unroll
        for (int i = 0; i < RM; ++i) acc[r][i] = f32x4{0.f, 0.f, 0.f, 0.f};

    const int fr = lane & 15, fq = lane >> 4;
    auto compute = [&](int buf) {
        const char *bx = lds + buf * STAGE, *bw = bx + XBYTES;
#pragma unroll
        for (int kk = 0; kk < 2; ++kk) {
            V8 xf[RM], wf[RN];
#pragma unroll
            for (int q = 0; q < RM; ++q) {
                const int row = wm * 64 + q * 16 + fr;
                xf[q] = *reinterpret_cast<const V8 *>(bx + row * 128 + (((kk * 4 + fq) ^ (row & 7)) << 4));
            }
#pragma unroll
            for (int r = 0; r < RN; ++r) {
                const int row = wn * (BN / 2) + r * 16 + fr;
                wf[r] = *reinterpret_cast<const V8 *>(bw + row * 128 + (((kk * 4 + fq) ^ (row & 7)) << 4));
            }
#pragma unroll
            for (int r = 0; r < RN; ++r)
#pragma unroll
                for (int q = 0; q < RM; ++q) acc[r][q] = mfma16(wf[r], xf[q], acc[r][q]);
        }
    };

    const int n = s_end - s_begin;
    load(0);
#pragma unroll
    for (int p = 1; p < PF; ++p)
        if (p < n) load(p);
    store(0, 0);
    __syncthreads();
    int i = 0;
    for (; i + 2 * PF <= n; i += PF) {
#pragma unroll
        for (int p = 0; p < PF; ++p) {
            load(p);
            compute((i + p) & 1);
            store((p + 1) % PF, (i + p + 1) & 1);
            __syncthreads();
        }
    }
#pragma unroll
    for (int t = 0; t < 2 * PF - 1; ++t) {
        if (i + t < n) {
            if (i + t + PF < n) load(t % PF);
            compute((i + t) & 1);
            if (i + t + 1 < n) store((t + 1) % PF, (i + t + 1) & 1);
            __syncthreads();
        }
    }

#pragma unroll
    for (int i = 0; i < RM; ++i) {
        const int m = tm * BM + wm * 64 + i * 16 + fr;
        if (m >= M) continue;
        if (split) {
#pragma unroll
            for (int r = 0; r < RN; ++r) {
                const int col = geglu ? (r >= RN / 2 ? cold.inner : 0) + tn * (BN / 2) + wn * (BN / 4) + (r % (RN / 2)) * 16 + fq * 4
                                      : tn * BN + wn * (BN / 2) + r * 16 + fq * 4;
                *reinterpret_cast<f32x4 *>(reinterpret_cast<float *>(out) + ((long)ks * M + m) * N + col) = acc[r][i];
            }
        } else if (geglu) {
#pragma unroll
            for (int r = 0; r < RN / 2; ++r)
                geglu4<T>(acc[r][i], acc[r + RN / 2][i], cold, reinterpret_cast<T *>(out), m, tn * (BN / 2) + wn * (BN / 4) + r * 16 + fq * 4);
        } else {
#pragma unroll
            for (int r = 0; r < RN; ++r) epilogue4<T>(acc[r][i], cold, reinterpret_cast<T *>(out), m, tn * BN + wn * (BN / 2) + r * 16 + fq * 4);
        }
    }
}

template <typename T>
__global__ void __launch_bounds__(256) linear_fold_kernel(const float *__restrict__ ws, T *y, long n4, int N, long MN, const LinCold cold) {
    const long q = (long)blockIdx.x * 256 + threadIdx.x;
    if (q >= n4) return;
    const bool geglu = cold.mode == PWW_LINEAR_BIAS_GEGLU;
    const int nout = geglu ? cold.inner : N;
    const long o4 = q * 4;
    const int m = (int)(o4 / nout), n = (int)(o4 - (long)m * nout);
    const float *p = ws + (long)m * N + n;
    f32x4 a = *reinterpret_cast<const f32x4 *>(p);
    for (int s = 1; s < cold.nsplit; ++s) a += *reinterpret_cast<const f32x4 *>(p + s * MN);
    if (geglu) {
        f32x4 g = *reinterpret_cast<const f32x4 *>(p + cold.inner);
        for (int s = 1; s < cold.nsplit; ++s) g += *reinterpret_cast<const f32x4 *>(p + s * MN + cold.inner);
        geglu4<T>(a, g, cold, y, m, n);
    } else {
        epilogue4<T>(a, cold, y, m, n);
    }
}

struct LinTune { int M, N, nslab, geglu, bn, nsplit; };
constexpr LinTune LIN_TUNED[] = {
    {8192, 2560, 5, 1, 64, 1}, {2048, 5120, 10, 1, 64, 1}, {512, 10240, 20, 1, 64, 1}, {128, 10240, 20, 1, 64, 1},
    {8192, 320, 20, 0, 64, 1}, {8192, 320, 5, 0, 64, 1}, {2048, 640, 40, 0, 128, 3}, {2048, 640, 10, 0, 64, 1},
    {512, 1280, 80, 0, 64, 3}, {512, 1280, 20, 0, 64, 2}, {128, 1280, 80, 0, 64, 5}, {128, 1280, 20, 0, 64, 4},
};

struct LinPlan {
    int bn, nsplit, nslab, ntiles, nout;
    long xs, ys, rs;
};

bool plan_linear(const pww_linear_desc_t *d, LinPlan *p) {
    if (!d || d->size < sizeof(pww_linear_desc_t)) { set_error("linear: descriptor missing or older than this library (size %u)", d ? d->size : 0u); return false; }
    const int e = d->epilogue;
    const bool geglu = e == PWW_LINEAR_BIAS_GEGLU;
    if ((d->dtype != PWW_DTYPE_F16 && d->dtype != PWW_DTYPE_BF16) || d->M < 1 || d->K < 64 || d->K % 64 != 0 || d->N < 64 || d->N % 64 != 0
        || e < PWW_LINEAR_NONE || e > PWW_LINEAR_BIAS_GEGLU || (geglu && d->N % 128 != 0)) {
        set_error("linear: unsupported (dtype %d M %d N %d K %d epilogue %d): K and N multiples of 64, GEGLU's inner = N / 2 a multiple of 64", d->dtype,
                  d->M, d->N, d->K, e);
        return false;
    }
    p->nout = geglu ? d->N / 2 : d->N;
    p->xs = d->x_stride ? d->x_stride : d->K;
    p->ys = d->y_stride ? d->y_stride : p->nout;
    p->rs = d->r_stride ? d->r_stride : p->nout;
    if (p->xs < d->K || p->ys < p->nout || p->rs < p->nout || ((p->xs | p->ys | p->rs) & 7)) {
        set_error("linear: row strides must cover their rows and be multiples of 8 elements (x %ld y %ld r %ld)", p->xs, p->ys, p->rs);
        return false;
    }
    if ((long)d->M * p->xs >= (1L << 31) || (long)d->N * d->K >= (1L << 31) || (long)d->M * d->N >= (1L << 31)) { set_error("linear: tensor of 2^31 elements or more"); return false; }
    p->nslab = d->K / 64;
    const LinTune *tuned = nullptr;
    for (const LinTune &t : LIN_TUNED)
        if (t.M == d->M && t.N == d->N && t.nslab == p->nslab && t.geglu == (int)geglu) tuned = &t;
    p->bn = d->tile_n ? d->tile_n : tuned ? tuned->bn : (d->N % 128 == 0 ? 128 : 64);
    if ((p->bn != 64 && p->bn != 128) || d->N % p->bn != 0) { set_error("linear: tile_n %d does not divide N %d", d->tile_n, d->N); return false; }
    p->ntiles = (d->M + LN_BM - 1) / LN_BM * (d->N / p->bn);
    int ns = d->splitk;
    if (ns <= 0 && tuned && p->bn == tuned->bn) ns = tuned->nsplit;
    if (ns <= 0) {
        ns = (480 + p->ntiles / 2) / p->ntiles;
        if (ns > p->nslab / 4) ns = p->nslab / 4;
        if (ns < 1) ns = 1;
    }
    if (ns > p->nslab || ns > 64) { set_error("linear: split %d exceeds the %d K-slabs (or 64)", ns, p->nslab); return false; }
    p->nsplit = ns;
    return true;
}

template <typename T>
int linear_launch(const LinPlan &p, const pww_linear_desc_t *d, const void *x, const void *w, const void *bias, const void *residual, void *y, void *ws,
                  hipStream_t stream) {
    LinCold cold{bias, residual, p.ys, p.rs, p.nsplit, p.nslab, d->epilogue, d->N / 2};
    const T *xt = static_cast<const T *>(x), *wt = static_cast<const T *>(w);
    const dim3 grid(p.ntiles * p.nsplit), block(LN_THREADS);
    void *out = p.nsplit == 1 ? y : ws;
    if (p.bn == 128) launch_timed(linear_kernel<T, 128>, grid, block, 0, stream, xt, wt, out, d->M, d->N, d->K, (int)p.xs, cold);
    else launch_timed(linear_kernel<T, 64>, grid, block, 0, stream, xt, wt, out, d->M, d->N, d->K, (int)p.xs, cold);
    if (p.nsplit == 1) return check_hip(hipGetLastError(), "linear launch");
    const long MN = (long)d->M * d->N, n4 = (long)d->M * p.nout / 4;
    launch_timed(linear_fold_kernel<T>, dim3((unsigned)((n4 + 255) / 256)), dim3(256), 0, stream, static_cast<const float *>(ws), static_cast<T *>(y), n4,
                 d->N, MN, cold);
    return check_hip(hipGetLastError(), "linear fold launch");
}

bool al16(const void *a) { return (reinterpret_cast<uintptr_t>(a) & 15) == 0; }

}

size_t linear_workspace_bytes(const pww_linear_desc_t *d) {
    LinPlan p;
    if (!plan_linear(d, &p)) return 0;
    return p.nsplit > 1 ? (size_t)p.nsplit * d->M * d->N * sizeof(float) : 0;
}

int linear_fwd(const void *x, const void *w, const void *bias, const void *residual, void *y, const pww_linear_desc_t *d, void *workspace,
               size_t workspace_bytes, hipStream_t stream) {
    LinPlan p;
    if (!plan_linear(d, &p)) return PWW_ENOTSUP;
    if (!x || !w || !y) { set_error("linear: x, w and y are required"); return PWW_EINVAL; }
    if ((d->epilogue >= PWW_LINEAR_BIAS && !bias) || (d->epilogue == PWW_LINEAR_BIAS_RESIDUAL && !residual)) {
        set_error("linear: epilogue %d needs its bias%s", d->epilogue, d->epilogue == PWW_LINEAR_BIAS_RESIDUAL ? " and residual" : "");
        return PWW_EINVAL;
    }
    if (!al16(x) || !al16(w) || !al16(y) || (reinterpret_cast<uintptr_t>(bias) & 7) || (reinterpret_cast<uintptr_t>(residual) & 7)) {
        set_error("linear: x, w, y must be 16-byte aligned, bias and residual 8-byte aligned");
        return PWW_EINVAL;
    }
    const size_t need = p.nsplit > 1 ? (size_t)p.nsplit * d->M * d->N * sizeof(float) : 0;
    if (need && (!workspace || !al16(workspace) || workspace_bytes < need)) {
        set_error("linear: split %d needs a 16-byte aligned workspace of %zu bytes (got %zu)", p.nsplit, need, workspace_bytes);
        return PWW_EINVAL;
    }
    if (!arch_ok()) return PWW_ENOTSUP;
    if (d->dtype == PWW_DTYPE_F16) return linear_launch<f16>(p, d, x, w, bias, residual, y, workspace, stream);
    return linear_launch<bf16>(p, d, x, w, bias, residual, y, workspace, stream);
}

}

PWW_LINEAR_API int pww_linear_version(void) { return PWW_LINEAR_VERSION; }
PWW_LINEAR_API const char *pww_linear_last_error(void) { return pww::last_error(); }
PWW_LINEAR_API size_t pww_linear_workspace_bytes(const pww_linear_desc_t *desc) { return pww::linear_workspace_bytes(desc); }
PWW_LINEAR_API int pww_linear_fwd(const void *x, const void *w, const void *bias, const void *residual, void *y, const pww_linear_desc_t *desc,
                                  void *workspace, size_t workspace_bytes, void *stream) {
    return pww::linear_fwd(x, w, bias, residual, y, desc, workspace, workspace_bytes, static_cast<hipStream_t>(stream));
}
```

paint-with-words-sd_amd/pww_hip/_lib.py:

```python
import ctypes
import os

_HERE = os.path.dirname(os.path.abspath(__file__))
LIB_PATH = os.environ.get("PWW_HIP_LIB", os.path.join(_HERE, "libpww_hip.so"))
EXPERIMENTS_LIB_PATH = os.environ.get("PWW_HIP_EXPERIMENTS_LIB", os.path.join(_HERE, "libpww_hip_experiments.so"))

LONG_LIB_PATH = os.environ.get("PWW_HIP_LONG_LIB", os.path.join(_HERE, "libpww_hip_long.so"))
SCOPE_LIB_PATH = os.environ.get("PWW_HIP_SCOPE_LIB", os.path.join(_HERE, "libpww_hip_scope.so"))
LINEAR_LIB_PATH = os.environ.get("PWW_HIP_LINEAR_LIB", os.path.join(_HERE, "libpww_hip_linear.so"))
REGIONS_LIB_PATH = os.environ.get("PWW_HIP_REGIONS_LIB", os.path.join(_HERE, "libpww_hip_regions.so"))
LORA_LIB_PATH = os.environ.get("PWW_HIP_LORA_LIB", os.path.join(_HERE, "libpww_hip_lora.so"))
CONVTAIL_LIB_PATH = os.environ.get("PWW_HIP_CONVTAIL_LIB", os.path.join(_HERE, "libpww_hip_convtail.so"))
CANVAS_LIB_PATH = os.environ.get("PWW_HIP_CANVAS_LIB", os.path.join(_HERE, "libpww_hip_canvas.so"))
CONCAT_LIB_PATH = os.environ.get("PWW_HIP_CONCAT_LIB", os.path.join(_HERE, "libpww_hip_concat.so"))
HOLD_LIB_PATH = os.environ.get("PWW_HIP_HOLD_LIB", os.path.join(_HERE, "libpww_hip_hold.so"))

PWW_OK, PWW_EINVAL, PWW_ENOTSUP, PWW_EHIP = 0, -22, -95, -5
MIN_VERSION = 127
DTYPE_F16, DTYPE_BF16 = 0, 1
LAYOUT_NCHW, LAYOUT_NHWC = 0, 1
ACT_NONE, ACT_SILU = 0, 1
LINEAR_NONE, LINEAR_BIAS, LINEAR_BIAS_RESIDUAL, LINEAR_BIAS_GEGLU = 0, 1, 2, 3
MAX_HEAD_DIM = 160

EXPORTS = ("pww_version", "pww_has_experiments", "pww_last_error", "pww_device_arch", "pww_self_attn_fwd", "pww_cross_attn_fwd",
           "pww_cross_attn_fwd_stat", "pww_cross_attn_fwd_stat_ex",
           "pww_qk_reduce", "pww_mask_build", "pww_mask_build_rgb", "pww_mask_build_f32", "pww_resize_tokens", "pww_gauss_blur", "pww_inpaint_prep", "pww_cfg_combine", "pww_store_f32",
           "pww_workspace_bytes", "pww_profile_arm", "pww_profile_elapsed_us", "pww_profile_reset", "pww_debug_timeline", "pww_debug_path_counts",
           "pww_debug_last_attn_route",
           "pww_qproj_stat", "pww_qproj_parts", "pww_cross_attn_fwd_parts", "pww_mask_build_f32_levels", "pww_qk_parts", "pww_qk_parts_count",
           "pww_group_norm_fwd", "pww_group_norm_workspace_bytes", "pww_add_layer_norm", "pww_add_layer_norm_bias", "pww_geglu", "pww_bias_residual",
           "pww_conv3x3_workspace_bytes", "pww_conv3x3_fwd", "pww_cross_attn_probs")
EXPERIMENT_EXPORTS = ("pww_cross_attn_fwd_fused", "pww_cross_attn_fwd_fused_ex", "pww_cross_fused_workspace_bytes", "pww_cross_fused_state_bytes",
                      "pww_cross_attn_fwd_parts_out", "pww_cross_attn_out_supported")


LONG_EXPORTS = ("pww_long_version", "pww_long_last_error", "pww_long_qk_parts", "pww_long_qk_parts_count", "pww_long_cross_attn_fwd_parts",
                "pww_long_cross_attn_probs", "pww_long_profile_arm", "pww_long_profile_elapsed_us")
LONG_MIN_VERSION = 100
LONG_MIN_KEYS, LONG_MAX_KEYS = 129, 256


SCOPE_EXPORTS = ("pww_scope_version", "pww_scope_last_error", "pww_scope_head_parts_count", "pww_scope_head_parts", "pww_scope_cross_attn_fwd")
SCOPE_MIN_VERSION = 100
SCOPE_HEAD, SCOPE_ROW = 1, 2


LINEAR_EXPORTS = ("pww_linear_version", "pww_linear_last_error", "pww_linear_workspace_bytes", "pww_linear_fwd")
LINEAR_MIN_VERSION = 100


REGIONS_EXPORTS = ("pww_regions_version", "pww_regions_last_error", "pww_regions_masks", "pww_regions_combine")
REGIONS_MIN_VERSION = 100
REGIONS_MAX, REGIONS_MAX_PLANE, REGIONS_MAX_FEATHER = 8, 9216, 8.0


LORA_EXPORTS = ("pww_lora_version", "pww_lora_last_error", "pww_lora_fwd")
LORA_MIN_VERSION = 100
LORA_MAX_ADAPTERS, LORA_MAX_RANK, LORA_MAX_SEGMENTS = 8, 128, 3


CONVTAIL_EXPORTS = ("pww_convtail_version", "pww_convtail_last_error", "pww_convtail_workspace_bytes", "pww_convtail_fwd")
CONVTAIL_MIN_VERSION = 100


CANVAS_EXPORTS = ("pww_canvas_version", "pww_canvas_last_error", "pww_canvas_gather", "pww_canvas_combine")
CANVAS_MIN_VERSION = 100
CANVAS_MAX_WINDOWS, CANVAS_MAX_RAMP, CANVAS_MIN_WINDOW, CANVAS_MAX_WINDOW = 64, 64, 8, 128


CONCAT_EXPORTS = ("pww_concat_version", "pww_concat_last_error", "pww_concat_group_norm_workspace_bytes", "pww_concat_group_norm_fwd",
                  "pww_concat_convtail_workspace_bytes", "pww_concat_convtail_fwd")
CONCAT_MIN_VERSION = 100


HOLD_EXPORTS = ("pww_hold_version", "pww_hold_last_error", "pww_hold_strength_map", "pww_hold_feather", "pww_hold_apply", "pww_hold_taps",
                "pww_hold_thresholds")
HOLD_MIN_VERSION = 100
HOLD_MAX_COLORS, HOLD_MAX_FEATHER, HOLD_MAX_RADIUS, HOLD_MAX_STEPS = 8, 8.0, 24, 100000


class AttnDesc(ctypes.Structure):
    _fields_ = [("dtype", ctypes.c_int32), ("B", ctypes.c_int32), ("H", ctypes.c_int32), ("N", ctypes.c_int32),
                ("M", ctypes.c_int32), ("D", ctypes.c_int32),
                ("q_stride", ctypes.c_int64 * 3), ("k_stride", ctypes.c_int64 * 3),
                ("v_stride", ctypes.c_int64 * 3), ("o_stride", ctypes.c_int64 * 3),
                ("scale", ctypes.c_float), ("bias_stride", ctypes.c_int64 * 4)]


class CrossOpts(ctypes.Structure):
    _fields_ = [("size", ctypes.c_uint32), ("bias_cols", ctypes.c_int32), ("coeff_scalar_dev", ctypes.c_void_p),
                ("bias_compact", ctypes.c_void_p), ("col_idx", ctypes.c_void_p), ("R", ctypes.c_int32), ("gated_images", ctypes.c_int32),
                ("compact_stride", ctypes.c_int64 * 2), ("col_idx_stride", ctypes.c_int64)]


class QprojDesc(ctypes.Structure):
    _fields_ = [("dtype", ctypes.c_int32), ("B", ctypes.c_int32), ("N", ctypes.c_int32), ("Cin", ctypes.c_int32), ("H", ctypes.c_int32),
                ("D", ctypes.c_int32), ("M", ctypes.c_int32), ("x_stride", ctypes.c_int64 * 2), ("q_stride", ctypes.c_int64 * 2),
                ("k_stride", ctypes.c_int64 * 2)]


class GnDesc(ctypes.Structure):
    _fields_ = [("dtype", ctypes.c_int32), ("layout", ctypes.c_int32), ("B", ctypes.c_int32), ("C", ctypes.c_int32), ("HW", ctypes.c_int32),
                ("G", ctypes.c_int32), ("eps", ctypes.c_float), ("act", ctypes.c_int32), ("add_stride", ctypes.c_int32), ("_pad", ctypes.c_int32)]


class LnDesc(ctypes.Structure):
    _fields_ = [("dtype", ctypes.c_int32), ("C", ctypes.c_int32), ("rows", ctypes.c_int64), ("a_stride", ctypes.c_int64), ("x_stride", ctypes.c_int64),
                ("s_stride", ctypes.c_int64), ("y_stride", ctypes.c_int64), ("eps", ctypes.c_float), ("_pad", ctypes.c_int32)]


class ConvDesc(ctypes.Structure):
    _fields_ = [("size", ctypes.c_uint32), ("dtype", ctypes.c_int32), ("B", ctypes.c_int32), ("Hin", ctypes.c_int32), ("Win", ctypes.c_int32),
                ("Cin", ctypes.c_int32), ("Cout", ctypes.c_int32), ("stride", ctypes.c_int32), ("upsample", ctypes.c_int32), ("tile_n", ctypes.c_int32),
                ("splitk", ctypes.c_int32), ("_pad", ctypes.c_int32)]


class LinearDesc(ctypes.Structure):
    _fields_ = [("size", ctypes.c_uint32), ("dtype", ctypes.c_int32), ("M", ctypes.c_int32), ("N", ctypes.c_int32), ("K", ctypes.c_int32),
                ("epilogue", ctypes.c_int32), ("x_stride", ctypes.c_int64), ("y_stride", ctypes.c_int64), ("r_stride", ctypes.c_int64),
                ("tile_n", ctypes.c_int32), ("splitk", ctypes.c_int32)]


class ProbsDesc(ctypes.Structure):
    _fields_ = [("size", ctypes.c_uint32), ("images", ctypes.c_int32), ("accumulate", ctypes.c_int32), ("weight", ctypes.c_float),
                ("out_stride", ctypes.c_int64 * 2)]


class LoraDesc(ctypes.Structure):
    _fields_ = [("size", ctypes.c_uint32), ("dtype", ctypes.c_int32), ("R", ctypes.c_int32), ("T", ctypes.c_int32), ("K", ctypes.c_int32),
                ("N", ctypes.c_int32), ("n_seg", ctypes.c_int32), ("rank", ctypes.c_int32), ("n_adapters", ctypes.c_int32), ("_pad", ctypes.c_int32),
                ("x_row_stride", ctypes.c_int64), ("x_tok_stride", ctypes.c_int64), ("y_row_stride", ctypes.c_int64), ("y_tok_stride", ctypes.c_int64)]


class ConvTailDesc(ctypes.Structure):
    _fields_ = [("size", ctypes.c_uint32), ("dtype", ctypes.c_int32), ("B", ctypes.c_int32), ("H", ctypes.c_int32), ("W", ctypes.c_int32),
                ("Cin", ctypes.c_int32), ("C2", ctypes.c_int32), ("Cout", ctypes.c_int32), ("tile_n", ctypes.c_int32), ("splitk", ctypes.c_int32)]


class ConcatGnDesc(ctypes.Structure):
    _fields_ = [("size", ctypes.c_uint32), ("dtype", ctypes.c_int32), ("B", ctypes.c_int32), ("C1", ctypes.c_int32), ("C2", ctypes.c_int32),
                ("HW", ctypes.c_int32), ("G", ctypes.c_int32), ("eps", ctypes.c_float), ("act", ctypes.c_int32), ("_pad", ctypes.c_int32)]


class ConcatTailDesc(ctypes.Structure):
    _fields_ = [("size", ctypes.c_uint32), ("dtype", ctypes.c_int32), ("B", ctypes.c_int32), ("H", ctypes.c_int32), ("W", ctypes.c_int32),
                ("Cin", ctypes.c_int32), ("C1", ctypes.c_int32), ("C2", ctypes.c_int32), ("Cout", ctypes.c_int32), ("tile_n", ctypes.c_int32),
                ("splitk", ctypes.c_int32), ("_pad", ctypes.c_int32)]


class Region(ctypes.Structure):
    _fields_ = [("r", ctypes.c_uint8), ("g", ctypes.c_uint8), ("b", ctypes.c_uint8), ("_pad", ctypes.c_uint8),
                ("strength", ctypes.c_float)]


class PwwHipError(RuntimeError):
    pass


_lib = None
_exp = None


def _bind(lib, experiments):
    vp, i32, i64, f32 = ctypes.c_void_p, ctypes.c_int32, ctypes.c_int64, ctypes.c_float
    lib.pww_version.restype = ctypes.c_int
    if lib.pww_version() // 100 != 1 or lib.pww_version() < MIN_VERSION:
        raise PwwHipError("libpww_hip ABI version %d.%02d is not 1.x >= 1.%02d (rebuild: python paint-with-words-sd_amd/build.py)"
                          % (lib.pww_version() // 100, lib.pww_version() % 100, MIN_VERSION % 100))
    lib.pww_last_error.restype = ctypes.c_char_p
    lib.pww_device_arch.argtypes = [ctypes.c_char_p, ctypes.c_size_t]
    lib.pww_self_attn_fwd.argtypes = [vp, vp, vp, vp, ctypes.POINTER(AttnDesc), vp]
    lib.pww_cross_attn_fwd.argtypes = [vp, vp, vp, vp, vp, vp, ctypes.POINTER(AttnDesc), vp]
    lib.pww_cross_attn_fwd_stat.argtypes = [vp, vp, vp, vp, vp, vp, i32, ctypes.c_double, f32, vp, ctypes.POINTER(AttnDesc), vp]
    lib.pww_cross_attn_fwd_stat_ex.argtypes = [vp, vp, vp, vp, vp, vp, i32, ctypes.c_double, f32, vp, ctypes.POINTER(AttnDesc),
                                               ctypes.POINTER(CrossOpts), vp]
    lib.pww_qproj_stat.argtypes = [vp, vp, vp, vp, vp, ctypes.POINTER(QprojDesc), i32, vp, ctypes.c_size_t, vp]
    lib.pww_qproj_stat.restype = ctypes.c_int
    lib.pww_qproj_parts.argtypes = [ctypes.POINTER(QprojDesc)]
    lib.pww_qproj_parts.restype = ctypes.c_int32
    lib.pww_cross_attn_fwd_parts.argtypes = [vp, vp, vp, vp, vp, i32, f32, vp, ctypes.POINTER(AttnDesc), vp, i32, vp, ctypes.POINTER(CrossOpts), vp]
    lib.pww_cross_attn_fwd_parts.restype = ctypes.c_int
    lib.pww_qk_parts.argtypes = [vp, vp, vp, ctypes.POINTER(AttnDesc), i32, i32, vp, ctypes.c_size_t, vp]
    lib.pww_qk_parts.restype = ctypes.c_int
    lib.pww_qk_parts_count.argtypes = [ctypes.POINTER(AttnDesc)]
    lib.pww_qk_parts_count.restype = ctypes.c_int32
    lib.pww_mask_build_f32_levels.argtypes = [vp, i32, i32, i32, vp, vp, i32, vp, vp, vp, vp, vp]
    lib.pww_mask_build_f32_levels.restype = ctypes.c_int
    lib.pww_group_norm_workspace_bytes.argtypes = [ctypes.POINTER(GnDesc)]
    lib.pww_group_norm_workspace_bytes.restype = ctypes.c_size_t
    lib.pww_group_norm_fwd.argtypes = [vp, vp, vp, vp, vp, vp, ctypes.POINTER(GnDesc), vp, ctypes.c_size_t, vp]
    lib.pww_group_norm_fwd.restype = ctypes.c_int
    lib.pww_add_layer_norm.argtypes = [vp, vp, vp, vp, vp, vp, ctypes.POINTER(LnDesc), vp]
    lib.pww_add_layer_norm.restype = ctypes.c_int
    lib.pww_add_layer_norm_bias.argtypes = [vp, vp, vp, vp, vp, vp, vp, ctypes.POINTER(LnDesc), vp]
    lib.pww_add_layer_norm_bias.restype = ctypes.c_int
    lib.pww_geglu.argtypes = [vp, vp, ctypes.c_int64, i32, ctypes.c_int64, ctypes.c_int64, i32, vp]
    lib.pww_geglu.restype = ctypes.c_int
    lib.pww_bias_residual.argtypes = [vp, vp, vp, vp, i32, i32, i32, i32, i32, vp]
    lib.pww_bias_residual.restype = ctypes.c_int
    lib.pww_conv3x3_workspace_bytes.argtypes = [ctypes.POINTER(ConvDesc)]
    lib.pww_conv3x3_workspace_bytes.restype = ctypes.c_size_t
    lib.pww_conv3x3_fwd.argtypes = [vp, vp, vp, vp, vp, ctypes.POINTER(ConvDesc), vp, ctypes.c_size_t, vp]
    lib.pww_conv3x3_fwd.restype = ctypes.c_int
    lib.pww_cross_attn_probs.argtypes = [vp, vp, vp, vp, i32, ctypes.c_double, f32, vp, ctypes.POINTER(AttnDesc), ctypes.POINTER(CrossOpts), vp,
                                         ctypes.POINTER(ProbsDesc), vp]
    lib.pww_cross_attn_probs.restype = ctypes.c_int
    lib.pww_debug_timeline.argtypes = [vp, ctypes.c_size_t]
    lib.pww_debug_timeline.restype = None
    lib.pww_debug_path_counts.argtypes = [vp]
    lib.pww_debug_path_counts.restype = None
    lib.pww_debug_last_attn_route.argtypes = [ctypes.POINTER(i32), ctypes.c_int]
    lib.pww_debug_last_attn_route.restype = ctypes.c_int
    lib.pww_qk_reduce.argtypes = [vp, vp, ctypes.POINTER(AttnDesc), vp, vp, ctypes.c_size_t, vp]
    lib.pww_mask_build.argtypes = [vp, i32, i32, vp, i32, vp, vp, i32, vp, vp, vp, vp, vp]
    lib.pww_mask_build_rgb.argtypes = [vp, i32, i32, vp, i32, vp, vp, i32, i32, vp, vp]
    lib.pww_mask_build_f32.argtypes = [vp, i32, i32, i32, vp, vp, i32, i32, vp, vp]
    lib.pww_resize_tokens.argtypes = [vp, i32, i32, i32, i32, i32, i32, vp, vp]
    lib.pww_gauss_blur.argtypes = [vp, vp, i32, i32, vp, i32, vp, vp]
    lib.pww_inpaint_prep.argtypes = [vp, vp, i32, i32, i32, i32, vp, vp, vp, vp]
    lib.pww_cfg_combine.argtypes = [vp, vp, f32, vp, i64, i32, vp]
    lib.pww_store_f32.argtypes = [vp, ctypes.POINTER(ctypes.c_float), i32, vp]
    lib.pww_store_f32.restype = ctypes.c_int
    lib.pww_workspace_bytes.argtypes = [ctypes.POINTER(AttnDesc)]
    lib.pww_workspace_bytes.restype = ctypes.c_size_t
    lib.pww_profile_arm.argtypes = []
    lib.pww_profile_arm.restype = ctypes.c_int
    lib.pww_profile_elapsed_us.argtypes = [i32, ctypes.POINTER(ctypes.c_float)]
    lib.pww_profile_elapsed_us.restype = ctypes.c_int
    lib.pww_profile_reset.argtypes = []
    lib.pww_profile_reset.restype = None
    for name in ("pww_device_arch", "pww_self_attn_fwd", "pww_cross_attn_fwd", "pww_cross_attn_fwd_stat", "pww_cross_attn_fwd_stat_ex", "pww_qk_reduce",
                 "pww_mask_build", "pww_mask_build_rgb", "pww_mask_build_f32", "pww_resize_tokens", "pww_gauss_blur", "pww_inpaint_prep", "pww_cfg_combine"):
        getattr(lib, name).restype = ctypes.c_int
    lib.pww_has_experiments.restype = ctypes.c_int
    if experiments:
        lib.pww_cross_attn_fwd_fused.argtypes = [vp, vp, vp, vp, vp, i32, f32, vp, ctypes.POINTER(AttnDesc), vp, vp, ctypes.c_size_t, vp, ctypes.c_size_t, vp]
        lib.pww_cross_attn_fwd_fused_ex.argtypes = [vp, vp, vp, vp, vp, i32, f32, vp, ctypes.POINTER(AttnDesc), vp, vp, ctypes.c_size_t, vp,
                                                    ctypes.c_size_t, ctypes.POINTER(CrossOpts), vp]
        lib.pww_cross_attn_fwd_fused.restype = lib.pww_cross_attn_fwd_fused_ex.restype = ctypes.c_int
        lib.pww_cross_fused_workspace_bytes.argtypes = [ctypes.POINTER(AttnDesc)]
        lib.pww_cross_fused_workspace_bytes.restype = ctypes.c_size_t
        lib.pww_cross_fused_state_bytes.argtypes = [ctypes.POINTER(AttnDesc)]
        lib.pww_cross_fused_state_bytes.restype = ctypes.c_size_t
        lib.pww_cross_attn_fwd_parts_out.argtypes = [vp, vp, vp, vp, vp, i32, f32, vp, ctypes.POINTER(AttnDesc), vp, i32, vp, ctypes.POINTER(CrossOpts),
                                                     vp, vp, vp, ctypes.POINTER(ctypes.c_int64), vp]
        lib.pww_cross_attn_fwd_parts_out.restype = ctypes.c_int
        lib.pww_cross_attn_out_supported.argtypes = [ctypes.POINTER(AttnDesc), ctypes.c_int32, ctypes.c_int32]
        lib.pww_cross_attn_out_supported.restype = ctypes.c_int32
    return lib


def load():
    global _lib
    if _lib is not None:
        return _lib
    if not os.path.isfile(LIB_PATH):
        raise PwwHipError(
            "libpww_hip.so not found at %s. Build it with `python paint-with-words-sd_amd/build.py` "
            "(or __graft_entry__.build()). There is no CPU/PyTorch fallback for the PwW kernels." % LIB_PATH)
    lib = ctypes.CDLL(LIB_PATH)
    _lib = _bind(lib, hasattr(lib, "pww_has_experiments") and bool(lib.pww_has_experiments()))
    return _lib


def has_experiments():
    return bool(load().pww_has_experiments())


def load_experiments():
    global _exp
    if _exp is not None:
        return _exp
    if has_experiments():
        _exp = load()
        return _exp
    if not os.path.isfile(EXPERIMENTS_LIB_PATH):
        raise PwwHipError("libpww_hip_experiments.so not found at %s: this entry point is not part of the product library. Build it with "
                          "`python paint-with-words-sd_amd/build.py --experiments` (tests: the `experiments_lib` fixture does)." % EXPERIMENTS_LIB_PATH)
    lib = ctypes.CDLL(EXPERIMENTS_LIB_PATH)
    lib.pww_has_experiments.restype = ctypes.c_int
    if not lib.pww_has_experiments():
        raise PwwHipError("%s was not built with -DPWW_EXPERIMENTS=1" % EXPERIMENTS_LIB_PATH)
    _exp = _bind(lib, True)
    return _exp


_P = ctypes.POINTER
_vp, _i32, _i64, _f32, _f64, _sz, _int = ctypes.c_void_p, ctypes.c_int32, ctypes.c_int64, ctypes.c_float, ctypes.c_double, ctypes.c_size_t, ctypes.c_int
_HINT = "(rebuild: python paint-with-words-sd_amd/build.py, or __graft_entry__.build())"
SIDE = {
    "long": dict(path="LONG_LIB_PATH", exports=LONG_EXPORTS, min_version=LONG_MIN_VERSION, missing_ok=False, needs="prompts longer than 77 tokens need it", sigs={
        "pww_long_qk_parts": ([_vp, _vp, _vp, _P(AttnDesc), _i32, _i32, _vp, _sz, _vp], _int),
        "pww_long_qk_parts_count": ([_P(AttnDesc)], _i32),
        "pww_long_cross_attn_fwd_parts": ([_vp, _vp, _vp, _vp, _vp, _i32, _f32, _vp, _P(AttnDesc), _vp, _i32, _vp, _P(CrossOpts), _vp], _int),
        "pww_long_cross_attn_probs": ([_vp, _vp, _vp, _vp, _i32, _f64, _f32, _vp, _P(AttnDesc), _P(CrossOpts), _vp, _P(ProbsDesc), _vp], _int),
        "pww_long_profile_arm": ([], _int),
        "pww_long_profile_elapsed_us": ([_P(_f32)], _int)}),
    "scope": dict(path="SCOPE_LIB_PATH", exports=SCOPE_EXPORTS, min_version=SCOPE_MIN_VERSION, missing_ok=True, needs="per-head / per-row score statistics need it", sigs={
        "pww_scope_head_parts_count": ([_P(AttnDesc)], _i32),
        "pww_scope_head_parts": ([_vp, _vp, _vp, _P(AttnDesc), _i32, _vp, _sz, _vp], _int),
        "pww_scope_cross_attn_fwd": ([_vp, _vp, _vp, _vp, _vp, _i32, _i32, _f32, _vp, _P(AttnDesc), _vp, _i32, _vp, _P(CrossOpts), _vp], _int)}),
    "linear": dict(path="LINEAR_LIB_PATH", exports=LINEAR_EXPORTS, min_version=LINEAR_MIN_VERSION, missing_ok=False, needs="linear layers on the native kernel need it", sigs={
        "pww_linear_workspace_bytes": ([_P(LinearDesc)], _sz),
        "pww_linear_fwd": ([_vp, _vp, _vp, _vp, _vp, _P(LinearDesc), _vp, _sz, _vp], _int)}),
    "regions": dict(path="REGIONS_LIB_PATH", exports=REGIONS_EXPORTS, min_version=REGIONS_MIN_VERSION, missing_ok=False, needs="region prompts need it", sigs={
        "pww_regions_masks": ([_vp, _i32, _i32, _vp, _i32, _f32, _vp, _vp], _int),
        "pww_regions_combine": ([_vp, _vp, _vp, _vp, _f32, _vp, _i32, _i32, _i32, _i64, _i32, _vp], _int)}),
}
SIDE_MORE = {
    "lora": dict(path="LORA_LIB_PATH", exports=LORA_EXPORTS, min_version=LORA_MIN_VERSION, missing_ok=False, needs="LoRA adapters on the native kernel need it", sigs={
        "pww_lora_fwd": ([_vp, _vp, _vp, _vp, _vp, _vp, _P(LoraDesc), _vp], _int)}),
}
SIDE_CONV = {
    "convtail": dict(path="CONVTAIL_LIB_PATH", exports=CONVTAIL_EXPORTS, min_version=CONVTAIL_MIN_VERSION, missing_ok=True, needs="conv2 with the shortcut as K-slabs needs it", sigs={
        "pww_convtail_workspace_bytes": ([_P(ConvTailDesc)], _sz),
        "pww_convtail_fwd": ([_vp, _vp, _vp, _vp, _vp, _vp, _vp, _P(ConvTailDesc), _vp, _sz, _vp], _int)}),
}
SIDE_EXTRA = {
    "canvas": dict(path="CANVAS_LIB_PATH", exports=CANVAS_EXPORTS, min_version=CANVAS_MIN_VERSION, missing_ok=False, needs="canvases larger than the window need it", sigs={
        "pww_canvas_gather": ([_vp, _vp, _P(_i32), _i32, _P(_i32), _i32, _i32, _i32, _i32, _i32, _i32, _f32, _i32, _i32, _vp], _int),
        "pww_canvas_combine": ([_vp, _vp, _vp, _vp, _f32, _vp, _P(_i32), _i32, _P(_i32), _i32, _i32, _i32, _i32, _i32, _i32, _i32, _i32, _i32, _vp], _int)}),
    "concat": dict(path="CONCAT_LIB_PATH", exports=CONCAT_EXPORTS, min_version=CONCAT_MIN_VERSION, missing_ok=True, needs="the up blocks without torch.cat need it", sigs={
        "pww_concat_group_norm_workspace_bytes": ([_P(ConcatGnDesc)], _sz),
        "pww_concat_group_norm_fwd": ([_vp, _vp, _vp, _vp, _vp, _P(ConcatGnDesc), _vp, _sz, _vp], _int),
        "pww_concat_convtail_workspace_bytes": ([_P(ConcatTailDesc)], _sz),
        "pww_concat_convtail_fwd": ([_vp, _vp, _vp, _vp, _vp, _vp, _vp, _vp, _P(ConcatTailDesc), _vp, _sz, _vp], _int)}),
    "hold": dict(path="HOLD_LIB_PATH", exports=HOLD_EXPORTS, min_version=HOLD_MIN_VERSION, missing_ok=False, needs="region strengths (img2img) need it", sigs={
        "pww_hold_strength_map": ([_vp, _P(ctypes.c_uint8), _P(_f32), _f32, _vp, _i32, _i32, _i32, _vp], _int),
        "pww_hold_feather": ([_vp, _vp, _vp, _i32, _i32, _f32, _vp], _int),
        "pww_hold_apply": ([_vp, _vp, _vp, _vp, _f32, _f32, _f32, _i32, _i32, _i64, _vp], _int),
        "pww_hold_taps": ([_f32, _P(_f32), _i32], _int),
        "pww_hold_thresholds": ([_i32, _P(_f32)], _int)}),
}
_side = {}


def side_spec(name):
    for table in (SIDE, SIDE_MORE, SIDE_CONV):
        if name in table:
            return table[name]
    return SIDE_EXTRA[name]


def load_side(name):
    lib = _side.get(name)
    if lib is not None:
        return lib
    spec = side_spec(name)
    path, so, pre = globals()[spec["path"]], "libpww_hip_%s.so" % name, "pww_%s_" % name
    if not os.path.isfile(path):
        if spec["missing_ok"]:
            return None
        raise PwwHipError("%s not found at %s: %s %s" % (so, path, spec["needs"], _HINT))
    try:
        lib = ctypes.CDLL(path)
        getattr(lib, pre + "version").restype = _int
        version = getattr(lib, pre + "version")()
    except (OSError, AttributeError) as e:
        raise PwwHipError("%s at %s cannot be loaded: %s %s" % (so, path, e, _HINT))
    if version // 100 != 1 or version < spec["min_version"]:
        raise PwwHipError("%s ABI version %d is not 1.x >= %d %s" % (so[:-3], version, spec["min_version"], _HINT))
    missing = [n for n in spec["exports"] if not hasattr(lib, n)]
    if missing:
        raise PwwHipError("%s at %s lacks %s %s" % (so, path, missing, _HINT))
    for fn, (argtypes, restype) in spec["sigs"].items():
        getattr(lib, fn).argtypes, getattr(lib, fn).restype = argtypes, restype
    getattr(lib, pre + "last_error").restype = ctypes.c_char_p
    lib.pww_last_error = getattr(lib, pre + "last_error")
    _side[name] = lib
    return lib


def load_long():
    lib = _side.get("long")
    return lib if lib is not None else load_side("long")


def load_scope():
    lib = _side.get("scope")
    return lib if lib is not None else load_side("scope")


def load_linear():
    lib = _side.get("linear")
    return lib if lib is not None else load_side("linear")


def load_regions():
    lib = _side.get("regions")
    return lib if lib is not None else load_side("regions")


def load_lora():
    lib = _side.get("lora")
    return lib if lib is not None else load_side("lora")


def load_convtail():
    lib = _side.get("convtail")
    return lib if lib is not None else load_side("convtail")


def load_canvas():
    lib = _side.get("canvas")
    return lib if lib is not None else load_side("canvas")


def load_concat():
    lib = _side.get("concat")
    return lib if lib is not None else load_side("concat")


def load_hold():
    lib = _side.get("hold")
    return lib if lib is not None else load_side("hold")


class experiments:

    def __enter__(self):
        global _lib
        load()
        self._prev = _lib
        _lib = load_experiments()
        return _lib

    def __exit__(self, *exc):
        global _lib
        _lib = self._prev
        return False


def check(rc, what, lib=None):
    if rc != PWW_OK:
        msg = (lib or load()).pww_last_error().decode("utf-8", "replace")
        raise PwwHipError("%s failed (rc=%d): %s" % (what, rc, msg))


def device_arch():
    buf = ctypes.create_string_buffer(64)
    check(load().pww_device_arch(buf, 64), "pww_device_arch")
    return buf.value.decode()
```

paint-with-words-sd_amd/pww_hip/ops.py:

```python
import ctypes

import torch

from . import _lib
from ._lib import AttnDesc, CrossOpts, ProbsDesc, QprojDesc, Region, PwwHipError

_DT = {torch.float16: _lib.DTYPE_F16, torch.bfloat16: _lib.DTYPE_BF16}


def _stream():
    return ctypes.c_void_p(torch.cuda.current_stream().cuda_stream)


def _ptr(t):
    return ctypes.c_void_p(t.data_ptr()) if t is not None else ctypes.c_void_p(0)


def _require_gpu(*tensors):
    for t in tensors:
        if t is not None and not t.is_cuda:
            raise PwwHipError("pww_hip ops need tensors on a HIP device (got %s); there is no CPU path" % t.device)


def _rows_ok(t):
# ... 710 lines not shown
    _require_gpu(rgb)
    if rgb.dtype != torch.uint8 or rgb.dim() != 3 or rgb.shape[2] != 3:
        raise PwwHipError("region_masks needs a uint8 colour map [H, W, 3]")
    rgb = rgb.contiguous()
    H, W = int(rgb.shape[0]), int(rgb.shape[1])
    K = len(colors)
    flat = [int(v) for c in colors for v in c]
    if len(flat) != 3 * K or any(not 0 <= v <= 255 for v in flat):
        raise PwwHipError("region_masks needs (r, g, b) colours of 8-bit values")
    host = (ctypes.c_uint8 * max(len(flat), 1))(*flat)
    out = torch.empty((K, H // 8, W // 8), dtype=torch.float32, device=rgb.device)
    lib = _lib.load_regions()
    with torch.cuda.device(rgb.device):
        _lib.check(lib.pww_regions_masks(_ptr(rgb), H, W, host, K, float(feather), _ptr(out), _stream()), "pww_regions_masks", lib)
    return out


def region_combine(eps, masks, weights, scales, guidance_scale):
    _require_gpu(eps, masks, weights, scales)
    if eps.dtype not in _DT or eps.dim() != 4 or masks.dim() != 4:
        raise PwwHipError("region_combine needs a float16 / bfloat16 [(K + 2) n, C, h, w] tensor and fp32 masks [n, K, h, w]")
    n, K = int(masks.shape[0]), int(masks.shape[1])
    if (eps.shape[0] != (K + 2) * n or tuple(eps.shape[-2:]) != tuple(masks.shape[-2:]) or tuple(weights.shape) != (n, K) or tuple(scales.shape) != (n, K)
            or any(t.dtype != torch.float32 for t in (masks, weights, scales))):
        raise PwwHipError("region_combine: eps %s does not go with masks %s, weights %s and scales %s (fp32)"
                          % (tuple(eps.shape), tuple(masks.shape), tuple(weights.shape), tuple(scales.shape)))
    eps, masks, weights, scales = eps.contiguous(), masks.contiguous(), weights.contiguous(), scales.contiguous()
    C, h, w = (int(v) for v in eps.shape[1:])
    out = torch.empty((n, C, h, w), dtype=torch.float32, device=eps.device)
    lib = _lib.load_regions()
    with torch.cuda.device(eps.device):
        _lib.check(lib.pww_regions_combine(_ptr(eps), _ptr(masks), _ptr(weights), _ptr(scales), float(guidance_scale), _ptr(out), n, K, C, h * w,
                                           _DT[eps.dtype], _stream()), "pww_regions_combine", lib)
    return out


def canvas_windows(L, win, stride):
    L, win, stride = int(L), int(win), int(stride)
    if win < 1 or L < win or not 1 <= stride <= win:
        raise ValueError("canvas_windows: length %d, window %d, stride %d (1 <= stride <= window <= length)" % (L, win, stride))
    return tuple(range(0, L - win, stride)) + (L - win,)


def _canvas_origins(ys, xs):
    ys, xs = [int(v) for v in ys], [int(v) for v in xs]
    if not ys or not xs:
        raise PwwHipError("canvas: the window origins ys and xs must not be empty")
    return ys, xs, (ctypes.c_int32 * len(ys))(*ys), (ctypes.c_int32 * len(xs))(*xs)


def canvas_gather(canvas, ys, xs, h, w, denom, copies, dtype):
    _require_gpu(canvas)
    if canvas.dim() == 4 and canvas.shape[0] == 1:
        canvas = canvas[0]
    if canvas.dtype != torch.float32 or canvas.dim() != 3:
        raise PwwHipError("canvas_gather needs a float32 canvas [C, Hc, Wc] (or [1, C, Hc, Wc])")
    if dtype not in _DT:
        raise PwwHipError("canvas_gather: the output type must be float16 or bfloat16 (got %s)" % dtype)
    ys, xs, ys_c, xs_c = _canvas_origins(ys, xs)
    canvas = canvas.contiguous()
    C, Hc, Wc = (int(v) for v in canvas.shape)
    out = torch.empty((int(copies) * len(ys) * len(xs), C, int(h), int(w)), dtype=dtype, device=canvas.device)
    lib = _lib.load_canvas()
    with torch.cuda.device(canvas.device):
        _lib.check(lib.pww_canvas_gather(_ptr(canvas), _ptr(out), ys_c, len(ys), xs_c, len(xs), C, Hc, Wc, int(h), int(w), float(denom), int(copies),
                                         _DT[dtype], _stream()), "pww_canvas_gather", lib)
    return out


def canvas_combine(eps, ys, xs, canvas_hw, guidance_scale, ramp=0, masks=None, weights=None, scales=None):
    _require_gpu(eps, masks, weights, scales)
    ys, xs, ys_c, xs_c = _canvas_origins(ys, xs)
    n_w = len(ys) * len(xs)
    if eps.dtype not in _DT or eps.dim() != 4:
        raise PwwHipError("canvas_combine needs a float16 / bfloat16 [(K + 2) n_w, C, h, w] tensor")
    K = 0
    if masks is not None or weights is not None or scales is not None:
        if masks is None or weights is None or scales is None or masks.dim() != 4:
            raise PwwHipError("canvas_combine: region prompts need masks fp32 [n_w, K, h, w] with weights and scales fp32 [n_w, K]")
        K = int(masks.shape[1])
        if (int(masks.shape[0]) != n_w or tuple(eps.shape[-2:]) != tuple(masks.shape[-2:]) or tuple(weights.shape) != (n_w, K) or tuple(scales.shape) != (n_w, K)
                or any(t.dtype != torch.float32 for t in (masks, weights, scales))):
            raise PwwHipError("canvas_combine: eps %s of %d windows does not go with masks %s, weights %s and scales %s (fp32)"
                              % (tuple(eps.shape), n_w, tuple(masks.shape), tuple(weights.shape), tuple(scales.shape)))
        masks, weights, scales = masks.contiguous(), weights.contiguous(), scales.contiguous()
    if eps.shape[0] != (K + 2) * n_w:
        raise PwwHipError("canvas_combine: eps has %d rows for %d windows and %d regions ((K + 2) n_w = %d)" % (eps.shape[0], n_w, K, (K + 2) * n_w))
    eps = eps.contiguous()
    C, h, w = (int(v) for v in eps.shape[1:])
    Hc, Wc = (int(v) for v in canvas_hw)
    out = torch.empty((1, C, Hc, Wc), dtype=torch.float32, device=eps.device)
    lib = _lib.load_canvas()
    with torch.cuda.device(eps.device):
        _lib.check(lib.pww_canvas_combine(_ptr(eps), _ptr(masks), _ptr(weights), _ptr(scales), float(guidance_scale), _ptr(out), ys_c, len(ys), xs_c,
                                          len(xs), K, C, Hc, Wc, h, w, int(ramp), _DT[eps.dtype], _stream()), "pww_canvas_combine", lib)
    return out


def hold_strength_map(rgb, colors, strengths, s0, feather=0.0):
    import numpy as np
    _require_gpu(rgb)
    if rgb.dtype != torch.uint8 or rgb.dim() != 3 or rgb.shape[2] != 3:
        raise PwwHipError("hold_strength_map needs a uint8 colour map [H, W, 3]")
    rgb = rgb.contiguous()
    H, W = int(rgb.shape[0]), int(rgb.shape[1])
    K = len(colors)
    flat = [int(v) for c in colors for v in c]
    if len(flat) != 3 * K or any(not 0 <= v <= 255 for v in flat):
        raise PwwHipError("hold_strength_map needs (r, g, b) colours of 8-bit values")
    if len(strengths) != K:
        raise PwwHipError("hold_strength_map: %d strengths for %d colours" % (len(strengths), K))
    base = np.float32(s0)
    deltas = [float(np.float32(s) - base) for s in strengths]
    host_c = (ctypes.c_uint8 * max(len(flat), 1))(*flat)
    host_d = (ctypes.c_float * max(K, 1))(*deltas)
    out = torch.empty((H // 8, W // 8), dtype=torch.float32, device=rgb.device)
    lib = _lib.load_hold()
    with torch.cuda.device(rgb.device):
        _lib.check(lib.pww_hold_strength_map(_ptr(rgb), host_c, host_d, float(base), _ptr(out), H, W, K, _stream()), "pww_hold_strength_map", lib)
        if float(feather) != 0.0:
            tmp = torch.empty_like(out)
            _lib.check(lib.pww_hold_feather(_ptr(out), _ptr(tmp), _ptr(out), H // 8, W // 8, float(feather), _stream()), "pww_hold_feather", lib)
    return out


def hold_feather(plane, sigma):
    _require_gpu(plane)
    if plane.dtype != torch.float32 or plane.dim() != 2:
        raise PwwHipError("hold_feather needs a float32 plane [h, w]")
    plane = plane.contiguous()
    tmp, out = torch.empty_like(plane), torch.empty_like(plane)
    lib = _lib.load_hold()
    with torch.cuda.device(plane.device):
        _lib.check(lib.pww_hold_feather(_ptr(plane), _ptr(tmp), _ptr(out), int(plane.shape[0]), int(plane.shape[1]), float(sigma), _stream()),
                   "pww_hold_feather", lib)
    return out


def hold_apply(x, x0, z, S, theta, a, b):
    _require_gpu(x, x0, z, S)
    if any(t.dtype != torch.float32 for t in (x, x0, z, S)):
        raise PwwHipError("hold_apply needs float32 tensors (got %s)" % [str(t.dtype) for t in (x, x0, z, S)])
    if x.dim() < 2 or x0.shape != x.shape or z.shape != x.shape or tuple(S.shape) != (x.shape[0],) + tuple(x.shape[2:]):
        raise PwwHipError("hold_apply: x %s does not go with x0 %s, z %s and S %s ([n, C, ...] three times and [n, ...])"
                          % (tuple(x.shape), tuple(x0.shape), tuple(z.shape), tuple(S.shape)))
    if not all(t.is_contiguous() for t in (x, x0, z, S)):
        raise PwwHipError("hold_apply needs contiguous tensors (x is written in place)")
    if len({t.device for t in (x, x0, z, S)}) != 1:
        raise PwwHipError("hold_apply needs its tensors on one device")
    n, C = int(x.shape[0]), int(x.shape[1])
    hw = x[0, 0].numel()
    lib = _lib.load_hold()
    with torch.cuda.device(x.device):
        _lib.check(lib.pww_hold_apply(_ptr(x), _ptr(x0), _ptr(z), _ptr(S), float(theta), float(a), float(b), n, C, hw, _stream()), "pww_hold_apply", lib)
    return x


def group_norm(x, num_groups, weight=None, bias=None, eps=1e-5, add=None, act=None, workspace=None, out=None, pre_bias=None):
    _require_gpu(x)
    if x.dim() != 4 or x.dtype not in _DT:
        raise PwwHipError("group_norm needs a 4-d float16/bfloat16 tensor (got %s %s)" % (tuple(x.shape), x.dtype))
    B, C, H, W = x.shape
    if x.is_contiguous():
        layout = _lib.LAYOUT_NCHW
    elif x.is_contiguous(memory_format=torch.channels_last):
        layout = _lib.LAYOUT_NHWC
    else:
        x = x.contiguous()
        layout = _lib.LAYOUT_NCHW
    if out is None:
        out = torch.empty_like(x)
    elif out.shape != x.shape or out.dtype != x.dtype or out.stride() != x.stride():
        raise PwwHipError("group_norm: `out` must have x's shape, dtype and strides")
    for name, t, shape in (("weight", weight, (C,)), ("bias", bias, (C,)), ("add", add, (B, C)), ("pre_bias", pre_bias, (C,))):
        if t is not None and (t.dtype != x.dtype or tuple(t.shape) != shape or t.device != x.device):
            raise PwwHipError("group_norm: `%s` must be %s %s on %s (got %s %s)" % (name, x.dtype, shape, x.device, t.dtype, tuple(t.shape)))
    weight = weight.contiguous() if weight is not None else None
    bias = bias.contiguous() if bias is not None else None
    pre_bias = pre_bias.contiguous() if pre_bias is not None else None
    add_stride = 0
    if add is not None:
        if add.stride(1) != 1 or add.stride(0) % 8 != 0 or add.data_ptr() % 16 != 0:
            add = add.contiguous()
        add_stride = add.stride(0) if B > 1 else C
    if act not in (None, "silu"):
        raise PwwHipError("group_norm: act must be None or 'silu'")
    d = _lib.GnDesc(_DT[x.dtype], layout, B, C, H * W, int(num_groups), float(eps), _lib.ACT_SILU if act == "silu" else _lib.ACT_NONE, add_stride, 0)
    lib = _lib.load()
    need = lib.pww_group_norm_workspace_bytes(ctypes.byref(d))
    if need == 0:
        raise PwwHipError("group_norm: unsupported shape B %d C %d HW %d groups %d (C and H*W multiples of 8, C %% groups == 0, "
                          "groups <= 32, C <= 4096 in channels_last)" % (B, C, H * W, num_groups))
    ws = workspace if workspace is not None else torch.empty(int(need), dtype=torch.uint8, device=x.device)
    with torch.cuda.device(x.device):
        _lib.check(lib.pww_group_norm_fwd(_ptr(x), _ptr(pre_bias), _ptr(add), _ptr(weight), _ptr(bias), _ptr(out), ctypes.byref(d), _ptr(ws), ws.numel(),
                                          _stream()), "pww_group_norm_fwd")
    return out


def _rows(t, name):
    if t.dtype not in _DT or t.dim() < 2:
        raise PwwHipError("%s: a float16/bfloat16 tensor of at least two dims is needed (got %s %s)" % (name, t.dtype, tuple(t.shape)))
    if t.stride(-1) != 1 or t.stride(-2) % 8 != 0 or t.data_ptr() % 16 != 0:
        return None
    C = t.shape[-1]
    rows = t.numel() // C
    stride = t.stride(-2)
    exp = stride
    for d in range(t.dim() - 2, -1, -1):
        if t.shape[d] != 1 and t.stride(d) != exp:
            return None
        exp *= t.shape[d]
    return rows, C, stride


def add_layer_norm(x, weight, bias, eps, a=None, post_bias=None):
    _require_gpu(x)
    rx = _rows(x, "add_layer_norm")
    if rx is None:
        x = x.contiguous()
        rx = _rows(x, "add_layer_norm")
    if rx is None:
        raise PwwHipError("add_layer_norm: the last dim must be a multiple of 8 (got %d)" % x.shape[-1])
    rows, C, xs = rx
    ra = None
    if a is not None:
        if a.shape != x.shape or a.dtype != x.dtype:
            raise PwwHipError("add_layer_norm: `a` must have x's shape and dtype")
        ra = _rows(a, "add_layer_norm")
        if ra is None:
            a = a.contiguous()
            ra = _rows(a, "add_layer_norm")
    for name, t in (("weight", weight), ("bias", bias), ("post_bias", post_bias)):
        if t is not None and (t.dtype != x.dtype or tuple(t.shape) != (C,) or not t.is_contiguous()):
            raise PwwHipError("add_layer_norm: `%s` must be a contiguous %s [%d]" % (name, x.dtype, C))
    if post_bias is not None and a is None:
        raise PwwHipError("add_layer_norm: post_bias needs the add form (a)")
    y = torch.empty(x.shape, dtype=x.dtype, device=x.device)
    s = torch.empty(x.shape, dtype=x.dtype, device=x.device) if a is not None else None
    d = _lib.LnDesc(_DT[x.dtype], C, rows, ra[2] if ra else 0, xs, C, C, float(eps), 0)
    with torch.cuda.device(x.device):
        if post_bias is not None:
            _lib.check(_lib.load().pww_add_layer_norm_bias(_ptr(a), _ptr(x), _ptr(weight), _ptr(bias), _ptr(post_bias), _ptr(s), _ptr(y), ctypes.byref(d),
                                                           _stream()), "pww_add_layer_norm_bias")
        else:
            _lib.check(_lib.load().pww_add_layer_norm(_ptr(a), _ptr(x), _ptr(weight), _ptr(bias), _ptr(s), _ptr(y), ctypes.byref(d), _stream()),
                       "pww_add_layer_norm")
    return (s, y) if a is not None else y


def geglu(h):
    _require_gpu(h)
    r = _rows(h, "geglu")
    if r is None:
        h = h.contiguous()
        r = _rows(h, "geglu")
    if r is None:
        raise PwwHipError("geglu: the last dim must be 2 * D with D a multiple of 8 (got %d)" % h.shape[-1])
    rows, C2, hs = r
    if C2 % 16 != 0:
        raise PwwHipError("geglu: the last dim must be 2 * D with D a multiple of 8 (got %d)" % C2)
    D = C2 // 2
    y = torch.empty(h.shape[:-1] + (D,), dtype=h.dtype, device=h.device)
    with torch.cuda.device(h.device):
        _lib.check(_lib.load().pww_geglu(_ptr(h), _ptr(y), rows, D, hs, D, _DT[h.dtype], _stream()), "pww_geglu")
    return y


def bias_residual(residual, value, bias):
    _require_gpu(residual, value, bias)
    if residual.shape != value.shape or residual.dtype != value.dtype or residual.dtype not in _DT or residual.dim() != 4 or bias.dtype != residual.dtype:
        raise PwwHipError("bias_residual: two same-shape 4-d float16/bfloat16 tensors and a bias of that type are needed")
    B, C, H, W = residual.shape
    if tuple(bias.shape) != (C,):
        raise PwwHipError("bias_residual: bias must have shape (%d,), got %s" % (C, tuple(bias.shape)))
    nhwc = value.is_contiguous(memory_format=torch.channels_last) and not value.is_contiguous()
    fmt = torch.channels_last if nhwc else torch.contiguous_format
    value, residual = value.contiguous(memory_format=fmt), residual.contiguous(memory_format=fmt)
    layout = _lib.LAYOUT_NHWC if nhwc else _lib.LAYOUT_NCHW
    y = torch.empty_like(value)
    with torch.cuda.device(value.device):
        _lib.check(_lib.load().pww_bias_residual(_ptr(residual), _ptr(value), _ptr(bias.contiguous()), _ptr(y), B, C, H * W, layout, _DT[value.dtype], _stream()),
                   "pww_bias_residual")
    return y


def _khwc_weight(weight):
    if weight.is_contiguous(memory_format=torch.channels_last):
        return weight
    key = (weight.data_ptr(), weight._version, weight.dtype, weight.device)
    hit = weight.__dict__.get("_pww_khwc")
    if hit is not None and hit[0] == key:
        return hit[1]
    packed = weight.detach().permute(0, 2, 3, 1).contiguous()
    weight.__dict__["_pww_khwc"] = (key, packed)
    return packed


def conv3x3_takes(x, weight, stride=1, upsample=False):
    if not (torch.is_tensor(x) and x.is_cuda and x.dim() == 4 and x.dtype in _DT and torch.is_tensor(weight) and weight.dtype == x.dtype and weight.dim() == 4):
        return False
    B, C, H, W = x.shape
    Cout = weight.shape[0]
    return (tuple(weight.shape[1:]) == (C, 3, 3) and C % 64 == 0 and Cout % 64 == 0 and stride in (1, 2) and not (upsample and stride != 1)
            and x.is_contiguous(memory_format=torch.channels_last) and x.data_ptr() % 16 == 0
            and B * H * W * C < 2 ** 31 // 4)


def conv3x3(x, weight, bias=None, residual=None, stride=1, upsample=False, tile_n=0, splitk=0):
    _require_gpu(x, weight, bias, residual)
    if not conv3x3_takes(x, weight, stride, upsample):
        raise PwwHipError("conv3x3: needs a channels_last float16/bfloat16 x with Cin, Cout multiples of 64 and a 3 x 3 weight of its dtype")
    B, C, H, W = x.shape
    Cout = weight.shape[0]
    Hv, Wv = H << int(bool(upsample)), W << int(bool(upsample))
    Ho, Wo = (Hv - 1) // stride + 1, (Wv - 1) // stride + 1
    w = _khwc_weight(weight)
    if bias is not None and (bias.dtype != x.dtype or tuple(bias.shape) != (Cout,)):
        raise PwwHipError("conv3x3: bias must be a %s [%d]" % (x.dtype, Cout))
    if bias is not None:
        bias = bias.contiguous()
    if residual is not None:
        if tuple(residual.shape) != (B, Cout, Ho, Wo) or residual.dtype != x.dtype:
            raise PwwHipError("conv3x3: residual must be a %s %s" % (x.dtype, (B, Cout, Ho, Wo)))
        residual = residual.contiguous(memory_format=torch.channels_last)
    d = _lib.ConvDesc(ctypes.sizeof(_lib.ConvDesc), _DT[x.dtype], B, H, W, C, Cout, int(stride), int(bool(upsample)), int(tile_n), int(splitk), 0)
    lib = _lib.load()
    y = torch.empty((B, Cout, Ho, Wo), dtype=x.dtype, device=x.device, memory_format=torch.channels_last)
    nbytes = int(lib.pww_conv3x3_workspace_bytes(ctypes.byref(d)))
    ws = torch.empty(nbytes // 4, dtype=torch.float32, device=x.device) if nbytes else None
    with torch.cuda.device(x.device):
        _lib.check(lib.pww_conv3x3_fwd(_ptr(x), _ptr(w), _ptr(bias), _ptr(residual), _ptr(y), ctypes.byref(d), _ptr(ws), nbytes, _stream()), "pww_conv3x3_fwd")
    return y


def conv3x3_shortcut_takes(h, conv2_weight, x, shortcut_weight):
    if not (conv3x3_takes(h, conv2_weight) and torch.is_tensor(x) and x.is_cuda and x.device == h.device and x.dim() == 4 and x.dtype == h.dtype
            and torch.is_tensor(shortcut_weight) and shortcut_weight.dtype == h.dtype and shortcut_weight.device == h.device):
        return False
    w2 = _linear_weight(shortcut_weight)
    B, C2, H, W = x.shape
    return (w2 is not None and tuple(w2.shape) == (conv2_weight.shape[0], C2) and C2 % 64 == 0 and (B, H, W) == (h.shape[0], h.shape[2], h.shape[3])
            and x.is_contiguous(memory_format=torch.channels_last) and x.data_ptr() % 16 == 0 and B * H * W * C2 < 2 ** 31 // 4)


def conv3x3_shortcut(h, conv2_weight, conv2_bias, x, shortcut_weight, shortcut_bias, tile_n=0, splitk=0):
    _require_gpu(h, conv2_weight, conv2_bias, x, shortcut_weight, shortcut_bias)
    if not conv3x3_shortcut_takes(h, conv2_weight, x, shortcut_weight):
        raise PwwHipError("conv3x3_shortcut: needs channels_last float16/bfloat16 h and x of one dtype, batch and size, channel counts multiples of 64, "
                          "a 3 x 3 weight and a dense 1 x 1 weight of that dtype")
    B, C, H, W = h.shape
    Cout, C2 = conv2_weight.shape[0], x.shape[1]
    w = _khwc_weight(conv2_weight)
    w2 = _linear_weight(shortcut_weight)
    biases = []
    for name, b in (("conv2_bias", conv2_bias), ("shortcut_bias", shortcut_bias)):
        if not torch.is_tensor(b) or b.dtype != h.dtype or tuple(b.shape) != (Cout,):
            raise PwwHipError("conv3x3_shortcut: %s must be a %s [%d]" % (name, h.dtype, Cout))
        biases.append(b.contiguous() if b.data_ptr() % 8 == 0 else b.clone(memory_format=torch.contiguous_format))
    lib = _lib.load_convtail()
    if lib is None:
        raise PwwHipError("conv3x3_shortcut: libpww_hip_convtail.so is not built %s" % _lib._HINT)
    d = _lib.ConvTailDesc(ctypes.sizeof(_lib.ConvTailDesc), _DT[h.dtype], B, H, W, C, C2, Cout, int(tile_n), int(splitk))
    y = torch.empty((B, Cout, H, W), dtype=h.dtype, device=h.device, memory_format=torch.channels_last)
    nbytes = int(lib.pww_convtail_workspace_bytes(ctypes.byref(d)))
    ws = torch.empty(nbytes // 4, dtype=torch.float32, device=h.device) if nbytes else None
    with torch.cuda.device(h.device):
        _lib.check(lib.pww_convtail_fwd(_ptr(h), _ptr(w), _ptr(x), _ptr(w2), _ptr(biases[0]), _ptr(biases[1]), _ptr(y), ctypes.byref(d), _ptr(ws), nbytes,
                                        _stream()), "pww_convtail_fwd", lib)
    return y


def _cat_pair(x1, x2, grid):
    if not (torch.is_tensor(x1) and torch.is_tensor(x2) and x1.is_cuda and x1.device == x2.device and x1.dim() == 4 and x2.dim() == 4
            and x1.dtype in _DT and x2.dtype == x1.dtype):
        return False
    (B, C1, H, W), C2 = x1.shape, x2.shape[1]
    return ((x2.shape[0], x2.shape[2], x2.shape[3]) == (B, H, W) and C1 % grid == 0 and C2 % grid == 0 and C1 > 0 and C2 > 0
            and x1.is_contiguous(memory_format=torch.channels_last) and x2.is_contiguous(memory_format=torch.channels_last)
            and x1.data_ptr() % 16 == 0 and x2.data_ptr() % 16 == 0)


def _gn_cat_desc(x1, x2, num_groups, eps, act):
    B, C1, H, W = x1.shape
    return _lib.ConcatGnDesc(ctypes.sizeof(_lib.ConcatGnDesc), _DT[x1.dtype], B, C1, x2.shape[1], H * W, int(num_groups), float(eps),
                             _lib.ACT_SILU if act == "silu" else _lib.ACT_NONE, 0)


def group_norm_cat_takes(x1, x2, num_groups, weight=None, bias=None):
    if not _cat_pair(x1, x2, 8):
        return False
    C = x1.shape[1] + x2.shape[1]
    for t in (weight, bias):
        if t is not None and not (torch.is_tensor(t) and t.dtype == x1.dtype and tuple(t.shape) == (C,) and t.device == x1.device):
            return False
    lib = _lib.load_concat()
    return lib is not None and int(lib.pww_concat_group_norm_workspace_bytes(ctypes.byref(_gn_cat_desc(x1, x2, num_groups, 1e-5, None)))) > 0


def group_norm_cat(x1, x2, num_groups, weight=None, bias=None, eps=1e-5, act=None, workspace=None):
    _require_gpu(x1, x2)
    if act not in (None, "silu"):
        raise PwwHipError("group_norm_cat: act must be None or 'silu'")
    if not group_norm_cat_takes(x1, x2, num_groups, weight, bias):
        raise PwwHipError("group_norm_cat: needs two channels_last float16/bfloat16 tensors of one dtype, batch and size with channel counts multiples "
                          "of 8, C1 + C2 a shape group_norm takes, and libpww_hip_concat.so %s" % _lib._HINT)
    B, C1, H, W = x1.shape
    weight = weight.contiguous() if weight is not None else None
    bias = bias.contiguous() if bias is not None else None
    d = _gn_cat_desc(x1, x2, num_groups, eps, act)
    lib = _lib.load_concat()
    need = int(lib.pww_concat_group_norm_workspace_bytes(ctypes.byref(d)))
    ws = workspace if workspace is not None else torch.empty(need, dtype=torch.uint8, device=x1.device)
    out = torch.empty((B, C1 + x2.shape[1], H, W), dtype=x1.dtype, device=x1.device, memory_format=torch.channels_last)
    with torch.cuda.device(x1.device):
        _lib.check(lib.pww_concat_group_norm_fwd(_ptr(x1), _ptr(x2), _ptr(weight), _ptr(bias), _ptr(out), ctypes.byref(d), _ptr(ws), ws.numel(), _stream()),
                   "pww_concat_group_norm_fwd", lib)
    return out


def conv3x3_shortcut_cat_takes(h, conv2_weight, x1, x2, shortcut_weight):
    if not (conv3x3_takes(h, conv2_weight) and _cat_pair(x1, x2, 64) and x1.device == h.device and x1.dtype == h.dtype
            and torch.is_tensor(shortcut_weight) and shortcut_weight.dtype == h.dtype and shortcut_weight.device == h.device):
        return False
    w2 = _linear_weight(shortcut_weight)
    B, C1, H, W = x1.shape
    Ct = C1 + x2.shape[1]
    return (w2 is not None and tuple(w2.shape) == (conv2_weight.shape[0], Ct) and (B, H, W) == (h.shape[0], h.shape[2], h.shape[3])
            and B * H * W * Ct < 2 ** 31 // 4 and _lib.load_concat() is not None)


def conv3x3_shortcut_cat(h, conv2_weight, conv2_bias, x1, x2, shortcut_weight, shortcut_bias, tile_n=0, splitk=0):
    _require_gpu(h, conv2_weight, conv2_bias, x1, x2, shortcut_weight, shortcut_bias)
    if not conv3x3_shortcut_cat_takes(h, conv2_weight, x1, x2, shortcut_weight):
        raise PwwHipError("conv3x3_shortcut_cat: needs channels_last float16/bfloat16 h, x1 and x2 of one dtype, batch and size, channel counts multiples "
                          "of 64, a 3 x 3 weight and a dense 1 x 1 weight of that dtype over C1 + C2 channels, and libpww_hip_concat.so %s" % _lib._HINT)
    B, C, H, W = h.shape
    Cout = conv2_weight.shape[0]
    w = _khwc_weight(conv2_weight)
    w2 = _linear_weight(shortcut_weight)
    biases = []
    for name, b in (("conv2_bias", conv2_bias), ("shortcut_bias", shortcut_bias)):
        if not torch.is_tensor(b) or b.dtype != h.dtype or tuple(b.shape) != (Cout,):
            raise PwwHipError("conv3x3_shortcut_cat: %s must be a %s [%d]" % (name, h.dtype, Cout))
        biases.append(b.contiguous() if b.data_ptr() % 8 == 0 else b.clone(memory_format=torch.contiguous_format))
    lib = _lib.load_concat()
    d = _lib.ConcatTailDesc(ctypes.sizeof(_lib.ConcatTailDesc), _DT[h.dtype], B, H, W, C, x1.shape[1], x2.shape[1], Cout, int(tile_n), int(splitk), 0)
    y = torch.empty((B, Cout, H, W), dtype=h.dtype, device=h.device, memory_format=torch.channels_last)
    nbytes = int(lib.pww_concat_convtail_workspace_bytes(ctypes.byref(d)))
    ws = torch.empty(nbytes // 4, dtype=torch.float32, device=h.device) if nbytes else None
    with torch.cuda.device(h.device):
        _lib.check(lib.pww_concat_convtail_fwd(_ptr(h), _ptr(w), _ptr(x1), _ptr(x2), _ptr(w2), _ptr(biases[0]), _ptr(biases[1]), _ptr(y), ctypes.byref(d),
                                               _ptr(ws), nbytes, _stream()), "pww_concat_convtail_fwd", lib)
    return y


def _linear_weight(weight):
    if not torch.is_tensor(weight) or weight.dim() not in (2, 4) or (weight.dim() == 4 and tuple(weight.shape[2:]) != (1, 1)):
        return None
    w = weight.detach().reshape(weight.shape[0], weight.shape[1]) if weight.dim() == 4 else weight.detach()
    return w if w.is_contiguous() and w.data_ptr() == weight.data_ptr() and w.data_ptr() % 16 == 0 else None


def linear_takes(x, weight, geglu=False, bias=None, residual=None, out=None):
    if not (torch.is_tensor(x) and x.is_cuda and x.dtype in _DT and x.dim() >= 2 and torch.is_tensor(weight) and weight.dtype == x.dtype):
        return False
    w = _linear_weight(weight)
    if w is None or x.shape[-1] != w.shape[1] or x.numel() == 0 or _rows(x, "linear") is None:
        return False
    N, K = w.shape
    rows, _, xs = _rows(x, "linear")
    if not (K % 64 == 0 and N % (128 if geglu else 64) == 0 and rows * xs < 2 ** 31 and rows * N < 2 ** 31 and N * K < 2 ** 31):
        return False
    if bias is not None and not (torch.is_tensor(bias) and bias.is_cuda and bias.dtype == x.dtype and tuple(bias.shape) == (N,) and bias.is_contiguous()
                                 and bias.data_ptr() % 8 == 0):
        return False
    shape = tuple(x.shape[:-1]) + (N // 2 if geglu else N,)
    for t in (residual, out):
        if t is not None and not (torch.is_tensor(t) and t.is_cuda and t.dtype == x.dtype and tuple(t.shape) == shape and _rows(t, "linear") is not None):
            return False
    return True


def linear(x, weight, bias=None, residual=None, geglu=False, tile_n=0, splitk=0, out=None):
    _require_gpu(x, weight, bias, residual, out)
    if not linear_takes(x, weight, geglu):
        raise PwwHipError("linear: needs a float16/bfloat16 [..., K] x with one row pitch and a dense [N, K] weight of its dtype, K and N multiples of 64%s"
                          % (" (geglu: N / 2 a multiple of 64)" if geglu else ""))
    w = _linear_weight(weight)
    N, K = w.shape
    M, _, xs = _rows(x, "linear")
    nout = N // 2 if geglu else N
    if (geglu or residual is not None) and bias is None:
        raise PwwHipError("linear: the residual and GEGLU epilogues need the bias")
    if geglu and residual is not None:
        raise PwwHipError("linear: geglu and residual exclude each other")
    if bias is not None:
        if bias.dtype != x.dtype or tuple(bias.shape) != (N,):
            raise PwwHipError("linear: bias must be a %s [%d]" % (x.dtype, N))
        bias = bias.contiguous() if bias.data_ptr() % 8 == 0 else bias.clone(memory_format=torch.contiguous_format)
    shape = tuple(x.shape[:-1]) + (nout,)
    rs = 0
    if residual is not None:
        if tuple(residual.shape) != shape or residual.dtype != x.dtype:
            raise PwwHipError("linear: residual must be a %s %s" % (x.dtype, shape))
        r = _rows(residual, "linear")
        if r is None:
            residual = residual.contiguous()
            r = _rows(residual, "linear")
        rs = r[2]
    if out is None:
        out = torch.empty(shape, dtype=x.dtype, device=x.device)
    elif tuple(out.shape) != shape or out.dtype != x.dtype or _rows(out, "linear") is None:
        raise PwwHipError("linear: out must be a %s %s whose rows have one pitch" % (x.dtype, shape))
    ys = _rows(out, "linear")[2]
    epi = _lib.LINEAR_BIAS_GEGLU if geglu else _lib.LINEAR_BIAS_RESIDUAL if residual is not None else _lib.LINEAR_BIAS if bias is not None else _lib.LINEAR_NONE
    d = _lib.LinearDesc(ctypes.sizeof(_lib.LinearDesc), _DT[x.dtype], M, N, K, epi, xs, ys, rs, int(tile_n), int(splitk))
    lib = _lib.load_linear()
    nbytes = int(lib.pww_linear_workspace_bytes(ctypes.byref(d)))
    ws = torch.empty(nbytes // 4, dtype=torch.float32, device=x.device) if nbytes else None
    with torch.cuda.device(x.device):
        _lib.check(lib.pww_linear_fwd(_ptr(x), _ptr(w), _ptr(bias), _ptr(residual), _ptr(out), ctypes.byref(d), _ptr(ws), nbytes, _stream()), "pww_linear_fwd", lib)
    return out


def lora_update_torch(y, x, A, B, row_adapter, row_scale, n_seg):
    R, ns = y.shape[0], y.shape[-1] // n_seg
    ra, rs = row_adapter[:R].reshape(R, 1, 1), row_scale[:R].reshape(R, 1, 1)
    wide = torch.promote_types(y.dtype, torch.float32)
    for i in range(A.shape[0]):
        on = (ra == i) & (rs != 0)
        for g in range(n_seg):
            u = torch.matmul(torch.matmul(x, A[i, g].t()), B[i, g].t())
            seg = y[..., g * ns:(g + 1) * ns]
            seg.copy_(torch.where(on, (seg.to(wide) + rs.to(wide) * u.to(wide)).to(y.dtype), seg))
    return y


def lora_takes(y, x, A, B, n_seg):
    if not (torch.is_tensor(y) and y.is_cuda and y.dtype in _DT and y.dim() == 3 and x.dim() == 3 and x.dtype == y.dtype == A.dtype == B.dtype
            and x.is_cuda and A.is_cuda and B.is_cuda and A.is_contiguous() and B.is_contiguous() and A.dim() == 4 and B.dim() == 4):
        return False
    (R, T, N), K, (n, seg, rank, _) = y.shape, x.shape[-1], A.shape
    if not (tuple(x.shape[:2]) == (R, T) and seg == n_seg and 1 <= n_seg <= _lib.LORA_MAX_SEGMENTS and 1 <= n <= _lib.LORA_MAX_ADAPTERS and A.shape[3] == K
            and N % n_seg == 0 and tuple(B.shape) == (n, n_seg, N // n_seg, rank) and rank in (32, 64, 96, 128) and K % 32 == 0 and (N // n_seg) % 16 == 0
            and 1 <= R <= 65535 and T >= 1):
        return False
    for t, w in ((x, K), (y, N)):
        rs, ts = (T * t.stride(1) if R == 1 else t.stride(0)), t.stride(1)
        if t.stride(2) != 1 or ts < w or rs < T * ts or rs % 8 or ts % 8 or t.data_ptr() % 16 or R * rs >= 2 ** 31:
            return False
    return A.data_ptr() % 16 == 0 and B.data_ptr() % 16 == 0 and A.numel() < 2 ** 31 and B.numel() < 2 ** 31


def lora_update(y, x, layer_stack, state, n_seg):
    from . import lora as _lora
    A, B = layer_stack
    if x.dtype != y.dtype:
        x = x.to(y.dtype)
    if A.dtype != y.dtype:
        A, B = A.to(y.dtype), B.to(y.dtype)
    if x.dim() == 3 and (x.stride(2) != 1 or x.stride(1) % 8 or (x.shape[0] > 1 and (x.stride(0) % 8 or x.stride(0) < x.shape[1] * x.stride(1))) or x.data_ptr() % 16):
        x = x.contiguous()
    state._ensure_rows()
    if y.shape[0] > state.row_adapter.numel():
        raise PwwHipError("lora_update: %d rows, the assignment holds %d" % (y.shape[0], state.row_adapter.numel()))
    if not lora_takes(y, x, A, B, n_seg):
        _lora._stats["declined"] += 1
        return lora_update_torch(y, x, A, B, state.row_adapter, state.row_scale, n_seg)
    (R, T, N), K = y.shape, x.shape[-1]
    d = _lib.LoraDesc(ctypes.sizeof(_lib.LoraDesc), _DT[y.dtype], R, T, K, N, n_seg, A.shape[2], A.shape[0], 0,
                      T * x.stride(1) if R == 1 else x.stride(0), x.stride(1), T * y.stride(1) if R == 1 else y.stride(0), y.stride(1))
    lib = _lib.load_lora()
    with torch.cuda.device(y.device):
        _lib.check(lib.pww_lora_fwd(_ptr(x), _ptr(A), _ptr(B), _ptr(state.row_adapter), _ptr(state.row_scale), _ptr(y), ctypes.byref(d), _stream()),
                   "pww_lora_fwd", lib)
    _lora._stats["kernel"] += 1
    return y
```

Baseline: 5.312.

## Add 160-wide N tile for conv3x3 and conv tails with dynamic LDS

After: 5.399 (median of 6 runs). 1.6% higher.

```diff
diff --git a/include/pww_hip_convwide.h b/include/pww_hip_convwide.h
--- /dev/null
+++ b/include/pww_hip_convwide.h
@@ -0,0 +1,24 @@
+#ifndef PWW_HIP_CONVWIDE_H
+#define PWW_HIP_CONVWIDE_H
+
+#include "pww_hip.h"
+
+#ifdef __cplusplus
+extern "C" {
+#endif
+
+#define PWW_CONVWIDE_VERSION 100
+
+int pww_convwide_version(void);
+const char *pww_convwide_last_error(void);
+
+int pww_convwide_takes(const pww_conv_desc_t *desc);
+size_t pww_convwide_workspace_bytes(const pww_conv_desc_t *desc);
+int pww_convwide_fwd(const void *x, const void *w, const void *bias, const void *residual, void *y, const pww_conv_desc_t *desc, void *workspace,
+                     size_t workspace_bytes, void *stream);
+
+#ifdef __cplusplus
+}
+#endif
+
+#endif
diff --git a/paint-with-words-sd_amd/build.py b/paint-with-words-sd_amd/build.py
--- a/paint-with-words-sd_amd/build.py
+++ b/paint-with-words-sd_amd/build.py
@@ -29,6 +29,7 @@
     "canvas": ("pww_canvas.hip", [], "canvases larger than the UNet's window: the windows' gather and the combine of their noise predictions"),
     "concat": ("pww_concat.hip", [], "the up blocks without torch.cat: GroupNorm and conv2 + shortcut over the two halves of the concatenation"),
     "hold": ("pww_hold.hip", [], "region strength: the strength map, its feather and the per-step hold of the pixels not yet released"),
+    "convwide": ("pww_convwide.hip", ["pww_conv.hip"], "the 160-wide tile of the plain 3 x 3 convolution"),
 }
 ALL_SIDE_LIBS = {**SIDE_LIBS, **SIDE_LIBS_CONV, **SIDE_LIBS_EXTRA}
 SOURCES = sorted({u[0] for u in UNITS + EXPERIMENT_UNITS})
@@ -41,6 +42,7 @@
 LIB_CANVAS, CANVAS_UNITS = SIDE_PATHS["canvas"], SIDE_UNITS["canvas"]
 LIB_CONCAT, CONCAT_UNITS = SIDE_PATHS["concat"], SIDE_UNITS["concat"]
 LIB_HOLD, HOLD_UNITS = SIDE_PATHS["hold"], SIDE_UNITS["hold"]
+LIB_CONVWIDE, CONVWIDE_UNITS = SIDE_PATHS["convwide"], SIDE_UNITS["convwide"]
 SIDE_PUBLIC_HEADERS = {"canvas": ["pww_hip_regions.h"]}
 HIPCC = os.environ.get("HIPCC", "/opt/rocm/bin/hipcc")
 FLAGS = ["--offload-arch=gfx950", "-O3", "-std=c++17", "-fPIC", "-Wall",
@@ -119,6 +121,7 @@
 def build_canvas(force=False, verbose=False): return build_side("canvas", force, verbose)
 def build_concat(force=False, verbose=False): return build_side("concat", force, verbose)
 def build_hold(force=False, verbose=False): return build_side("hold", force, verbose)
+def build_convwide(force=False, verbose=False): return build_side("convwide", force, verbose)
 
 
 def _build_check(exe, lib, libname, defines, force):
diff --git a/paint-with-words-sd_amd/csrc/pww_common.h b/paint-with-words-sd_amd/csrc/pww_common.h
--- a/paint-with-words-sd_amd/csrc/pww_common.h
+++ b/paint-with-words-sd_amd/csrc/pww_common.h
@@ -4,6 +4,8 @@
 #include <stdint.h>
 #include <stdio.h>
 #include <stdarg.h>
+#include <stdlib.h>
+#include <string.h>
 #include "../../include/pww_hip.h"
 
 #ifndef PWW_EXPERIMENTS
@@ -39,6 +41,16 @@
     return __builtin_bit_cast(V8, z);
 }
 
+__device__ __forceinline__ char *launch_lds() {
+    extern __shared__ __attribute__((aligned(16))) char lds_launch[];
+    return lds_launch;
+}
+
+__device__ __forceinline__ void store_partial_through(void *ws, unsigned ws_bytes, unsigned byte_off, const f32x4 &v) {
+    const __amdgpu_buffer_rsrc_t rsrc = __builtin_amdgcn_make_buffer_rsrc(ws, 0, (int)ws_bytes, 0x00020000);
+    __builtin_amdgcn_raw_buffer_store_b128(__builtin_bit_cast(u32x4, v), rsrc, (int)byte_off, 0, 16);
+}
+
 __device__ __forceinline__ int swap23(int i) { return (i & ~12) | ((i & 4) << 1) | ((i & 8) >> 1); }
 
 struct DebugKnobs {
@@ -66,9 +78,29 @@
 };
 const DebugKnobs &debug_knobs();
 
+constexpr bool PARTIAL_STORES_THROUGH_DEFAULT = false;
+static inline int partial_stores_through(size_t ws_bytes) {
+    const char *e = getenv("PWW_PARTIAL_STORES");
+    const bool through = e && !strcmp(e, "plain") ? false : e && !strcmp(e, "through") ? true : PARTIAL_STORES_THROUGH_DEFAULT;
+    return through && ws_bytes < ((size_t)1 << 32) ? 1 : 0;
+}
+
 void set_error(const char *fmt, ...);
 int check_hip(hipError_t e, const char *what);
 bool arch_ok();
+
+struct LdsRaised { bool dev[8] = {false, false, false, false, false, false, false, false}; };
+template <typename K>
+static inline int raise_lds_limit(K kern, size_t lds, LdsRaised &raised) {
+    bool *done = raised.dev;
+    int dev = 0;
+    if (check_hip(hipGetDevice(&dev), "hipGetDevice")) return PWW_EHIP;
+    if (dev < 8 && done[dev]) return PWW_OK;
+    if (check_hip(hipFuncSetAttribute(reinterpret_cast<const void *>(kern), hipFuncAttributeMaxDynamicSharedMemorySize, (int)lds), "hipFuncSetAttribute"))
+        return PWW_EHIP;
+    if (dev < 8) done[dev] = true;
+    return PWW_OK;
+}
 
 bool profile_take(hipEvent_t *start, hipEvent_t *stop, hipStream_t stream);
 
diff --git a/paint-with-words-sd_amd/csrc/pww_concat.hip b/paint-with-words-sd_amd/csrc/pww_concat.hip
--- a/paint-with-words-sd_amd/csrc/pww_concat.hip
+++ b/paint-with-words-sd_amd/csrc/pww_concat.hip
@@ -378,6 +378,7 @@
 struct CatTailCold {
     const void *x1, *x2, *wsc, *bias, *bias2;
     int nsplit, nmain, ntail;
+    int through;
 };
 
 __device__ __forceinline__ int xcd_remap(int orig, int nwg) {
@@ -402,7 +403,12 @@
     typedef typename Vec<T>::v8 V8;
     constexpr int BM = CT_BM, PF = CT_PF, XL = BM * 8 / CT_THREADS, WL = BN * 8 / CT_THREADS, RM = 4, RN = BN / 32;
     constexpr int XBYTES = BM * 128, STAGE = (BM + BN) * 128;
-    __shared__ __attribute__((aligned(16))) char lds[2 * STAGE];
+    constexpr bool DYN = 2 * STAGE > 64 * 1024;
+    __shared__ __attribute__((aligned(16))) char lds[DYN ? 16 : 2 * STAGE];
+    auto stage = [&](int buf) -> char * {
+        if constexpr (DYN) return launch_lds() + buf * STAGE;
+        else return lds + buf * STAGE;
+    };
 
     const int tid = threadIdx.x, lane = tid & 63, wave = tid >> 6, wm = wave >> 1, wn = wave & 1;
     const int ntm = (M + BM - 1) / BM;
@@ -469,7 +475,7 @@
         ps = cross ? C2 : ps;
     };
     auto store = [&](int p, int buf) {
-        char *base = lds + buf * STAGE;
+        char *base = stage(buf);
 #pragma unroll
         for (int i = 0; i < XL; ++i) {
             const u32x4 z = {0u, 0u, 0u, 0u};
@@ -487,7 +493,7 @@
 
     const int fr = lane & 15, fq = lane >> 4;
     auto compute = [&](int buf) {
-        const char *bx = lds + buf * STAGE, *bw = bx + XBYTES;
+        const char *bx = stage(buf), *bw = bx + XBYTES;
 #pragma unroll
         for (int kk = 0; kk < 2; ++kk) {
             V8 xf[RM], wf[RN];
@@ -536,6 +542,20 @@
         }
     }
 
+    if (split && cold.through) {
+        const unsigned ws_bytes = (unsigned)cold.nsplit * (unsigned)M * (unsigned)N * 4u;
+#pragma unroll
+        for (int i = 0; i < RM; ++i) {
+            const int m = tm * BM + wm * 64 + i * 16 + fr;
+            if (m >= M) continue;
+#pragma unroll
+            for (int r = 0; r < RN; ++r) {
+                const int n = tn * BN + wn * (BN / 2) + r * 16 + fq * 4;
+                store_partial_through(out, ws_bytes, (((unsigned)ks * (unsigned)M + (unsigned)m) * (unsigned)N + (unsigned)n) * 4u, acc[r][i]);
+            }
+        }
+        return;
+    }
 #pragma unroll
     for (int i = 0; i < RM; ++i) {
         const int m = tm * BM + wm * 64 + i * 16 + fr;
@@ -564,7 +584,7 @@
     {128, 1280, 180, 40, 64, 12},
     {512, 1280, 180, 40, 128, 12}, {512, 1280, 180, 30, 128, 12}, {512, 1280, 180, 10, 128, 12},
     {2048, 640, 90, 30, 128, 6}, {2048, 640, 90, 20, 128, 6}, {2048, 640, 90, 15, 128, 6}, {2048, 640, 90, 5, 128, 6},
-    {8192, 320, 45, 15, 64, 4}, {8192, 320, 45, 10, 64, 4},
+    {8192, 320, 45, 15, 160, 4}, {8192, 320, 45, 10, 160, 4},
 };
 
 struct TailPlan {
@@ -573,10 +593,10 @@
 
 bool cat_tail_plan(const pww_concat_tail_desc_t *d, TailPlan *p) {
     if ((d->dtype != PWW_DTYPE_F16 && d->dtype != PWW_DTYPE_BF16) || d->B < 1 || d->H < 1 || d->W < 1 || d->Cin < 64 || d->Cin % 64 != 0 || d->C1 < 64
-        || d->C1 % 64 != 0 || d->C2 < 64 || d->C2 % 64 != 0 || d->Cout < 64 || d->Cout % 64 != 0 || d->Cin > 65536 || d->C1 > 32768 || d->C2 > 32768
-        || d->Cout > 65536) {
-        set_error("concat_convtail: unsupported (dtype %d B %d %dx%d Cin %d C1 %d C2 %d Cout %d): Cin, C1, C2 and Cout multiples of 64", d->dtype, d->B,
-                  d->H, d->W, d->Cin, d->C1, d->C2, d->Cout);
+        || d->C1 % 64 != 0 || d->C2 < 64 || d->C2 % 64 != 0 || d->Cout < 64 || (d->Cout % 64 != 0 && d->Cout % 160 != 0) || d->Cin > 65536 || d->C1 > 32768
+        || d->C2 > 32768 || d->Cout > 65536) {
+        set_error("concat_convtail: unsupported (dtype %d B %d %dx%d Cin %d C1 %d C2 %d Cout %d): Cin, C1 and C2 multiples of 64, Cout of 64 or 160", d->dtype,
+                  d->B, d->H, d->W, d->Cin, d->C1, d->C2, d->Cout);
         return false;
     }
     const long M = (long)d->B * d->H * d->W, Ct = (long)d->C1 + d->C2;
@@ -591,8 +611,8 @@
     const TailTune *tuned = nullptr;
     for (const TailTune &t : TAIL_TUNED)
         if (t.M == p->M && t.N == d->Cout && t.nmain == p->nmain && t.ntail == p->ntail) tuned = &t;
-    p->bn = d->tile_n ? d->tile_n : tuned ? tuned->bn : (d->Cout % 128 == 0 ? 128 : 64);
-    if ((p->bn != 64 && p->bn != 128) || d->Cout % p->bn != 0) { set_error("concat_convtail: tile_n %d does not divide Cout %d", d->tile_n, d->Cout); return false; }
+    p->bn = d->tile_n ? d->tile_n : tuned ? tuned->bn : (d->Cout % 128 == 0 ? 128 : d->Cout % 64 == 0 ? 64 : 160);
+    if ((p->bn != 64 && p->bn != 128 && p->bn != 160) || d->Cout % p->bn != 0) { set_error("concat_convtail: tile_n %d does not divide Cout %d", d->tile_n, d->Cout); return false; }
     p->ntiles = (p->M + CT_BM - 1) / CT_BM * (d->Cout / p->bn);
     int ns = d->splitk;
     if (ns <= 0 && tuned && p->bn == tuned->bn) ns = tuned->nsplit;
@@ -613,7 +633,12 @@
     const int N = d->Cout;
     const dim3 grid(p.ntiles * p.nsplit), block(CT_THREADS);
     void *out = p.nsplit == 1 ? y : ws;
-    if (p.bn == 128) launch_timed(cat_tail_kernel<T, 128>, grid, block, 0, stream, xt, wt, out, p.M, N, d->Cin, d->C1, d->C2, d->H, d->W, cold);
+    if (p.bn == 160) {
+        constexpr size_t lds = 2 * (CT_BM + 160) * 128;
+        static thread_local LdsRaised raised;
+        if (raise_lds_limit(cat_tail_kernel<T, 160>, lds, raised)) return PWW_EHIP;
+        launch_timed(cat_tail_kernel<T, 160>, grid, block, lds, stream, xt, wt, out, p.M, N, d->Cin, d->C1, d->C2, d->H, d->W, cold);
+    } else if (p.bn == 128) launch_timed(cat_tail_kernel<T, 128>, grid, block, 0, stream, xt, wt, out, p.M, N, d->Cin, d->C1, d->C2, d->H, d->W, cold);
     else launch_timed(cat_tail_kernel<T, 64>, grid, block, 0, stream, xt, wt, out, p.M, N, d->Cin, d->C1, d->C2, d->H, d->W, cold);
     if (p.nsplit == 1) return check_hip(hipGetLastError(), "concat_convtail launch");
     const long MN = (long)p.M * N, n4 = MN / 4;
@@ -675,7 +700,7 @@
         return PWW_EINVAL;
     }
     if (!arch_ok()) return PWW_ENOTSUP;
-    const CatTailCold cold{x1, x2, wsc, bias, bias2, p.nsplit, p.nmain, p.ntail};
+    const CatTailCold cold{x1, x2, wsc, bias, bias2, p.nsplit, p.nmain, p.ntail, need ? partial_stores_through(need) : 0};
     if (d->dtype == PWW_DTYPE_F16) return cat_tail_launch<f16>(p, d, x, w, cold, y, workspace, stream);
     return cat_tail_launch<bf16>(p, d, x, w, cold, y, workspace, stream);
 }
diff --git a/paint-with-words-sd_amd/csrc/pww_conv.hip b/paint-with-words-sd_amd/csrc/pww_conv.hip
--- a/paint-with-words-sd_amd/csrc/pww_conv.hip
+++ b/paint-with-words-sd_amd/csrc/pww_conv.hip
@@ -13,6 +13,7 @@
 struct ConvCold {
     const void *bias, *residual;
     int nsplit, nslab;
+    int through;
 };
 
 __device__ __forceinline__ int xcd_remap(int orig, int nwg) {
@@ -45,7 +46,12 @@
     typedef typename Vec<T>::v8 V8;
     constexpr int BM = CV_BM, PF = CV_PF, XL = BM * 8 / CV_THREADS, WL = BN * 8 / CV_THREADS, RM = 4, RN = BN / 32;
     constexpr int XBYTES = BM * 128, STAGE = (BM + BN) * 128;
-    __shared__ __attribute__((aligned(16))) char lds[2 * STAGE];
+    constexpr bool DYN = 2 * STAGE > 64 * 1024;
+    __shared__ __attribute__((aligned(16))) char lds[DYN ? 16 : 2 * STAGE];
+    auto stage = [&](int buf) -> char * {
+        if constexpr (DYN) return launch_lds() + buf * STAGE;
+        else return lds + buf * STAGE;
+    };
 
     const int geo = cold.nslab >> 24;
     const int nslab = cold.nslab & 0xffffff;
@@ -96,7 +102,7 @@
         if (ci0 == Cin) { ci0 = 0; ++tap; }
     };
     auto store = [&](int p, int buf) {
-        char *base = lds + buf * STAGE;
+        char *base = stage(buf);
 #pragma unroll
         for (int i = 0; i < XL; ++i) {
             const u32x4 z = {0u, 0u, 0u, 0u};
@@ -114,7 +120,7 @@
 
     const int fr = lane & 15, fq = lane >> 4;
     auto compute = [&](int buf) {
-        const char *bx = lds + buf * STAGE, *bw = bx + XBYTES;
+        const char *bx = stage(buf), *bw = bx + XBYTES;
 #pragma unroll
         for (int kk = 0; kk < 2; ++kk) {
             V8 xf[RM], wf[RN];
@@ -162,6 +168,20 @@
         }
     }
 
+    if (split && cold.through) {
+        const unsigned ws_bytes = (unsigned)cold.nsplit * (unsigned)M * (unsigned)N * 4u;
+#pragma unroll
+        for (int i = 0; i < RM; ++i) {
+            const int m = tm * BM + wm * 64 + i * 16 + fr;
+            if (m >= M) continue;
+#pragma unroll
+            for (int r = 0; r < RN; ++r) {
+                const int n = tn * BN + wn * (BN / 2) + r * 16 + fq * 4;
+                store_partial_through(out, ws_bytes, (((unsigned)ks * (unsigned)M + (unsigned)m) * (unsigned)N + (unsigned)n) * 4u, acc[r][i]);
+            }
+        }
+        return;
+    }
 #pragma unroll
     for (int i = 0; i < RM; ++i) {
         const int m = tm * BM + wm * 64 + i * 16 + fr;
@@ -187,10 +207,10 @@
 
 struct ConvTune { int M, N, nslab, bn, nsplit; };
 constexpr ConvTune CONV_TUNED[] = {
-    {8192, 320, 45, 64, 3}, {8192, 320, 90, 64, 4}, {8192, 320, 135, 64, 3}, {8192, 640, 90, 128, 3},
-    {2048, 320, 45, 64, 6}, {2048, 640, 45, 64, 3}, {2048, 640, 90, 128, 6}, {2048, 640, 135, 128, 6}, {2048, 640, 180, 128, 6},
-    {2048, 640, 270, 128, 6}, {2048, 1280, 180, 128, 3},
-    {512, 640, 90, 64, 6}, {512, 1280, 90, 128, 6}, {512, 1280, 180, 128, 12}, {512, 1280, 270, 128, 12}, {512, 1280, 360, 128, 12},
+    {8192, 320, 45, 160, 2}, {8192, 320, 90, 160, 2}, {8192, 320, 135, 160, 4}, {8192, 640, 90, 160, 1},
+    {2048, 320, 45, 64, 6}, {2048, 640, 45, 64, 3}, {2048, 640, 90, 160, 4}, {2048, 640, 135, 160, 4}, {2048, 640, 180, 160, 4},
+    {2048, 640, 270, 128, 6}, {2048, 1280, 180, 160, 4},
+    {512, 640, 90, 64, 6}, {512, 1280, 90, 128, 6}, {512, 1280, 180, 160, 8}, {512, 1280, 270, 160, 8}, {512, 1280, 360, 160, 8},
     {128, 1280, 180, 64, 12}, {128, 1280, 360, 64, 24},
     {65536, 640, 90, 128, 1}, {16384, 1280, 180, 128, 1},
     {4096, 640, 90, 128, 3}, {4096, 1280, 90, 128, 3}, {4096, 1280, 180, 128, 3}, {4096, 1280, 270, 128, 3}, {4096, 1280, 360, 128, 3},
@@ -205,8 +225,9 @@
     if (!d || d->size < sizeof(pww_conv_desc_t)) { set_error("conv3x3: descriptor missing or older than this library (size %u)", d ? d->size : 0u); return false; }
     const int up = d->upsample, s = d->stride;
     if ((d->dtype != PWW_DTYPE_F16 && d->dtype != PWW_DTYPE_BF16) || d->B < 1 || d->Hin < 1 || d->Win < 1 || d->Cin < 64 || d->Cin % 64 != 0
-        || d->Cout < 64 || d->Cout % 64 != 0 || (s != 1 && s != 2) || (up != 0 && up != 1) || (up && s != 1) || d->Cin > 65536 || d->Cout > 65536) {
-        set_error("conv3x3: unsupported (dtype %d B %d %dx%d Cin %d Cout %d stride %d upsample %d): Cin and Cout multiples of 64, stride 1 or 2, "
+        || d->Cout < 64 || (d->Cout % 64 != 0 && d->Cout % 160 != 0) || (s != 1 && s != 2) || (up != 0 && up != 1) || (up && s != 1) || d->Cin > 65536
+        || d->Cout > 65536) {
+        set_error("conv3x3: unsupported (dtype %d B %d %dx%d Cin %d Cout %d stride %d upsample %d): Cin a multiple of 64, Cout of 64 or 160, stride 1 or 2, "
                   "upsample only at stride 1", d->dtype, d->B, d->Hin, d->Win, d->Cin, d->Cout, s, up);
         return false;
     }
@@ -220,8 +241,8 @@
     const ConvTune *tuned = nullptr;
     for (const ConvTune &t : CONV_TUNED)
         if (t.M == p->M && t.N == d->Cout && t.nslab == p->nslab) tuned = &t;
-    p->bn = d->tile_n ? d->tile_n : tuned ? tuned->bn : (d->Cout % 128 == 0 ? 128 : 64);
-    if ((p->bn != 64 && p->bn != 128) || d->Cout % p->bn != 0) { set_error("conv3x3: tile_n %d does not divide Cout %d", d->tile_n, d->Cout); return false; }
+    p->bn = d->tile_n ? d->tile_n : tuned ? tuned->bn : (d->Cout % 128 == 0 ? 128 : d->Cout % 64 == 0 ? 64 : 160);
+    if ((p->bn != 64 && p->bn != 128 && p->bn != 160) || d->Cout % p->bn != 0) { set_error("conv3x3: tile_n %d does not divide Cout %d", d->tile_n, d->Cout); return false; }
     p->ntiles = (p->M + CV_BM - 1) / CV_BM * (d->Cout / p->bn);
     int ns = d->splitk;
     if (ns <= 0 && tuned && p->bn == tuned->bn) ns = tuned->nsplit;
@@ -238,13 +259,23 @@
 template <typename T>
 int conv_launch(const ConvPlan &p, const pww_conv_desc_t *d, const void *x, const void *w, const void *bias, const void *residual, void *y, void *ws,
                 hipStream_t stream) {
-    ConvCold cold{bias, residual, p.nsplit, p.nslab | ((d->stride | (d->upsample << 4)) << 24)};
+    const int N = d->Cout, HWo = p.Ho * p.Wo;
+    ConvCold cold{bias, residual, p.nsplit, p.nslab | ((d->stride | (d->upsample << 4)) << 24),
+                  p.nsplit > 1 ? partial_stores_through((size_t)p.nsplit * p.M * N * sizeof(float)) : 0};
     const T *xt = static_cast<const T *>(x), *wt = static_cast<const T *>(w);
-    const int N = d->Cout, HWo = p.Ho * p.Wo;
     const dim3 grid(p.ntiles * p.nsplit), block(CV_THREADS);
     void *out = p.nsplit == 1 ? y : ws;
+#ifdef PWW_CONV_WIDE_UNIT
+    if (p.bn != 160) { set_error("conv3x3: tile_n %d is launched by libpww_hip.so (pww_conv3x3_fwd)", p.bn); return PWW_ENOTSUP; }
+    constexpr size_t lds = 2 * (CV_BM + 160) * 128;
+    static thread_local LdsRaised raised;
+    if (raise_lds_limit(conv3x3_kernel<T, 160>, lds, raised)) return PWW_EHIP;
+    launch_timed(conv3x3_kernel<T, 160>, grid, block, lds, stream, xt, wt, out, p.M, N, d->Cin, d->Hin, d->Win, p.Wo, HWo, cold);
+#else
+    if (p.bn == 160) { set_error("conv3x3: the 160-wide tile is launched by libpww_hip_convwide.so (pww_convwide_fwd)"); return PWW_ENOTSUP; }
     if (p.bn == 128) launch_timed(conv3x3_kernel<T, 128>, grid, block, 0, stream, xt, wt, out, p.M, N, d->Cin, d->Hin, d->Win, p.Wo, HWo, cold);
     else launch_timed(conv3x3_kernel<T, 64>, grid, block, 0, stream, xt, wt, out, p.M, N, d->Cin, d->Hin, d->Win, p.Wo, HWo, cold);
+#endif
     if (p.nsplit == 1) return check_hip(hipGetLastError(), "conv3x3 launch");
     const long MN = (long)p.M * N, n4 = MN / 4;
     launch_timed(conv3x3_fold_kernel<T>, dim3((unsigned)((n4 + 255) / 256)), dim3(256), 0, stream, static_cast<const float *>(ws), static_cast<T *>(y), n4,
@@ -256,6 +287,11 @@
 
 }
 
+int conv3x3_plans_wide(const pww_conv_desc_t *d) {
+    ConvPlan p;
+    return plan_conv(d, &p) && p.bn == 160 ? 1 : 0;
+}
+
 size_t conv3x3_workspace_bytes(const pww_conv_desc_t *d) {
     ConvPlan p;
     if (!plan_conv(d, &p)) return 0;
@@ -266,6 +302,11 @@
                 size_t workspace_bytes, hipStream_t stream) {
     ConvPlan p;
     if (!plan_conv(d, &p)) return PWW_ENOTSUP;
+#ifdef PWW_CONV_WIDE_UNIT
+    if (p.bn != 160) { set_error("conv3x3: tile_n %d is launched by libpww_hip.so (pww_conv3x3_fwd)", p.bn); return PWW_ENOTSUP; }
+#else
+    if (p.bn == 160) { set_error("conv3x3: the 160-wide tile is launched by libpww_hip_convwide.so (pww_convwide_fwd)"); return PWW_ENOTSUP; }
+#endif
     if (!x || !w || !y) { set_error("conv3x3: x, w and y are required"); return PWW_EINVAL; }
     if (!al16(x) || !al16(w) || !al16(y) || (reinterpret_cast<uintptr_t>(bias) & 7) || (reinterpret_cast<uintptr_t>(residual) & 7)) {
         set_error("conv3x3: x, w, y must be 16-byte aligned, bias and residual 8-byte aligned");
diff --git a/paint-with-words-sd_amd/csrc/pww_conv_tail.hip b/paint-with-words-sd_amd/csrc/pww_conv_tail.hip
--- a/paint-with-words-sd_amd/csrc/pww_conv_tail.hip
+++ b/paint-with-words-sd_amd/csrc/pww_conv_tail.hip
@@ -17,6 +17,7 @@
 struct TailCold {
     const void *x2, *w2, *bias, *bias2;
     int nsplit, nmain, ntail;
+    int through;
 };
 
 __device__ __forceinline__ int xcd_remap(int orig, int nwg) {
@@ -41,7 +42,12 @@
     typedef typename Vec<T>::v8 V8;
     constexpr int BM = CT_BM, PF = CT_PF, XL = BM * 8 / CT_THREADS, WL = BN * 8 / CT_THREADS, RM = 4, RN = BN / 32;
     constexpr int XBYTES = BM * 128, STAGE = (BM + BN) * 128;
-    __shared__ __attribute__((aligned(16))) char lds[2 * STAGE];
+    constexpr bool DYN = 2 * STAGE > 64 * 1024;
+    __shared__ __attribute__((aligned(16))) char lds[DYN ? 16 : 2 * STAGE];
+    auto stage = [&](int buf) -> char * {
+        if constexpr (DYN) return launch_lds() + buf * STAGE;
+        else return lds + buf * STAGE;
+    };
 
     const int tid = threadIdx.x, lane = tid & 63, wave = tid >> 6, wm = wave >> 1, wn = wave & 1;
     const int ntm = (M + BM - 1) / BM;
@@ -101,7 +107,7 @@
         tap += wrap ? 1 : 0;
     };
     auto store = [&](int p, int buf) {
-        char *base = lds + buf * STAGE;
+        char *base = stage(buf);
 #pragma unroll
         for (int i = 0; i < XL; ++i) {
             const u32x4 z = {0u, 0u, 0u, 0u};
@@ -119,7 +125,7 @@
 
     const int fr = lane & 15, fq = lane >> 4;
     auto compute = [&](int buf) {
-        const char *bx = lds + buf * STAGE, *bw = bx + XBYTES;
+        const char *bx = stage(buf), *bw = bx + XBYTES;
 #pragma unroll
         for (int kk = 0; kk < 2; ++kk) {
             V8 xf[RM], wf[RN];
@@ -168,6 +174,20 @@
         }
     }
 
+    if (split && cold.through) {
+        const unsigned ws_bytes = (unsigned)cold.nsplit * (unsigned)M * (unsigned)N * 4u;
+#pragma unroll
+        for (int i = 0; i < RM; ++i) {
+            const int m = tm * BM + wm * 64 + i * 16 + fr;
+            if (m >= M) continue;
+#pragma unroll
+            for (int r = 0; r < RN; ++r) {
+                const int n = tn * BN + wn * (BN / 2) + r * 16 + fq * 4;
+                store_partial_through(out, ws_bytes, (((unsigned)ks * (unsigned)M + (unsigned)m) * (unsigned)N + (unsigned)n) * 4u, acc[r][i]);
+            }
+        }
+        return;
+    }
 #pragma unroll
     for (int i = 0; i < RM; ++i) {
         const int m = tm * BM + wm * 64 + i * 16 + fr;
@@ -196,7 +216,7 @@
     {128, 1280, 180, 40, 64, 12},
     {512, 1280, 180, 40, 128, 12}, {512, 1280, 180, 30, 128, 12}, {512, 1280, 180, 10, 128, 12},
     {2048, 640, 90, 30, 128, 6}, {2048, 640, 90, 20, 128, 6}, {2048, 640, 90, 15, 128, 6}, {2048, 640, 90, 5, 128, 6},
-    {8192, 320, 45, 15, 64, 4}, {8192, 320, 45, 10, 64, 4},
+    {8192, 320, 45, 15, 160, 4}, {8192, 320, 45, 10, 160, 4},
 };
 
 struct TailPlan {
@@ -206,9 +226,9 @@
 bool plan_tail(const pww_convtail_desc_t *d, TailPlan *p) {
     if (!d || d->size < sizeof(pww_convtail_desc_t)) { set_error("convtail: descriptor missing or older than this library (size %u)", d ? d->size : 0u); return false; }
     if ((d->dtype != PWW_DTYPE_F16 && d->dtype != PWW_DTYPE_BF16) || d->B < 1 || d->H < 1 || d->W < 1 || d->Cin < 64 || d->Cin % 64 != 0 || d->C2 < 64
-        || d->C2 % 64 != 0 || d->Cout < 64 || d->Cout % 64 != 0 || d->Cin > 65536 || d->C2 > 65536 || d->Cout > 65536) {
-        set_error("convtail: unsupported (dtype %d B %d %dx%d Cin %d C2 %d Cout %d): Cin, C2 and Cout multiples of 64", d->dtype, d->B, d->H, d->W, d->Cin,
-                  d->C2, d->Cout);
+        || d->C2 % 64 != 0 || d->Cout < 64 || (d->Cout % 64 != 0 && d->Cout % 160 != 0) || d->Cin > 65536 || d->C2 > 65536 || d->Cout > 65536) {
+        set_error("convtail: unsupported (dtype %d B %d %dx%d Cin %d C2 %d Cout %d): Cin and C2 multiples of 64, Cout of 64 or 160", d->dtype, d->B, d->H,
+                  d->W, d->Cin, d->C2, d->Cout);
         return false;
     }
     const long M = (long)d->B * d->H * d->W;
@@ -224,8 +244,8 @@
     const TailTune *tuned = nullptr;
     for (const TailTune &t : TAIL_TUNED)
         if (t.M == p->M && t.N == d->Cout && t.nmain == p->nmain && t.ntail == p->ntail) tuned = &t;
-    p->bn = d->tile_n ? d->tile_n : tuned ? tuned->bn : (d->Cout % 128 == 0 ? 128 : 64);
-    if ((p->bn != 64 && p->bn != 128) || d->Cout % p->bn != 0) { set_error("convtail: tile_n %d does not divide Cout %d", d->tile_n, d->Cout); return false; }
+    p->bn = d->tile_n ? d->tile_n : tuned ? tuned->bn : (d->Cout % 128 == 0 ? 128 : d->Cout % 64 == 0 ? 64 : 160);
+    if ((p->bn != 64 && p->bn != 128 && p->bn != 160) || d->Cout % p->bn != 0) { set_error("convtail: tile_n %d does not divide Cout %d", d->tile_n, d->Cout); return false; }
     p->ntiles = (p->M + CT_BM - 1) / CT_BM * (d->Cout / p->bn);
     int ns = d->splitk;
     if (ns <= 0 && tuned && p->bn == tuned->bn) ns = tuned->nsplit;
@@ -242,12 +262,17 @@
 template <typename T>
 int tail_launch(const TailPlan &p, const pww_convtail_desc_t *d, const void *x, const void *w, const void *x2, const void *w2, const void *bias,
                 const void *bias2, void *y, void *ws, hipStream_t stream) {
-    TailCold cold{x2, w2, bias, bias2, p.nsplit, p.nmain, p.ntail};
+    const int N = d->Cout;
+    TailCold cold{x2, w2, bias, bias2, p.nsplit, p.nmain, p.ntail, p.nsplit > 1 ? partial_stores_through((size_t)p.nsplit * p.M * N * sizeof(float)) : 0};
     const T *xt = static_cast<const T *>(x), *wt = static_cast<const T *>(w);
-    const int N = d->Cout;
     const dim3 grid(p.ntiles * p.nsplit), block(CT_THREADS);
     void *out = p.nsplit == 1 ? y : ws;
-    if (p.bn == 128) launch_timed(convtail_kernel<T, 128>, grid, block, 0, stream, xt, wt, out, p.M, N, d->Cin, d->C2, d->H, d->W, cold);
+    if (p.bn == 160) {
+        constexpr size_t lds = 2 * (CT_BM + 160) * 128;
+        static thread_local LdsRaised raised;
+        if (raise_lds_limit(convtail_kernel<T, 160>, lds, raised)) return PWW_EHIP;
+        launch_timed(convtail_kernel<T, 160>, grid, block, lds, stream, xt, wt, out, p.M, N, d->Cin, d->C2, d->H, d->W, cold);
+    } else if (p.bn == 128) launch_timed(convtail_kernel<T, 128>, grid, block, 0, stream, xt, wt, out, p.M, N, d->Cin, d->C2, d->H, d->W, cold);
     else launch_timed(convtail_kernel<T, 64>, grid, block, 0, stream, xt, wt, out, p.M, N, d->Cin, d->C2, d->H, d->W, cold);
     if (p.nsplit == 1) return check_hip(hipGetLastError(), "convtail launch");
     const long MN = (long)p.M * N, n4 = MN / 4;
diff --git a/paint-with-words-sd_amd/csrc/pww_convwide.hip b/paint-with-words-sd_amd/csrc/pww_convwide.hip
--- /dev/null
+++ b/paint-with-words-sd_amd/csrc/pww_convwide.hip
@@ -0,0 +1,17 @@
+#define PWW_SIDE_LIB "libpww_hip_convwide"
+#include "pww_side_host.h"
+#include "../../include/pww_hip_convwide.h"
+
+#define PWW_CONVWIDE_API extern "C" __attribute__((visibility("default")))
+
+#define PWW_CONV_WIDE_UNIT 1
+#include "pww_conv.hip"
+
+PWW_CONVWIDE_API int pww_convwide_version(void) { return PWW_CONVWIDE_VERSION; }
+PWW_CONVWIDE_API const char *pww_convwide_last_error(void) { return pww::last_error(); }
+PWW_CONVWIDE_API int pww_convwide_takes(const pww_conv_desc_t *desc) { return pww::conv3x3_plans_wide(desc); }
+PWW_CONVWIDE_API size_t pww_convwide_workspace_bytes(const pww_conv_desc_t *desc) { return pww::conv3x3_workspace_bytes(desc); }
+PWW_CONVWIDE_API int pww_convwide_fwd(const void *x, const void *w, const void *bias, const void *residual, void *y, const pww_conv_desc_t *desc,
+                                      void *workspace, size_t workspace_bytes, void *stream) {
+    return pww::conv3x3_fwd(x, w, bias, residual, y, desc, workspace, workspace_bytes, static_cast<hipStream_t>(stream));
+}
diff --git a/paint-with-words-sd_amd/csrc/pww_linear.hip b/paint-with-words-sd_amd/csrc/pww_linear.hip
--- a/paint-with-words-sd_amd/csrc/pww_linear.hip
+++ b/paint-with-words-sd_amd/csrc/pww_linear.hip
@@ -18,6 +18,7 @@
     const void *bias, *residual;
     long ys, rs;
     int nsplit, nslab, mode, inner;
+    int through;
 };
 
 __device__ __forceinline__ int xcd_remap(int orig, int nwg) {
@@ -170,6 +171,21 @@
         }
     }
 
+    if (split && cold.through) {
+        const unsigned ws_bytes = (unsigned)cold.nsplit * (unsigned)M * (unsigned)N * 4u;
+#pragma unroll
+        for (int i = 0; i < RM; ++i) {
+            const int m = tm * BM + wm * 64 + i * 16 + fr;
+            if (m >= M) continue;
+#pragma unroll
+            for (int r = 0; r < RN; ++r) {
+                const int col = geglu ? (r >= RN / 2 ? cold.inner : 0) + tn * (BN / 2) + wn * (BN / 4) + (r % (RN / 2)) * 16 + fq * 4
+                                      : tn * BN + wn * (BN / 2) + r * 16 + fq * 4;
+                store_partial_through(out, ws_bytes, (((unsigned)ks * (unsigned)M + (unsigned)m) * (unsigned)N + (unsigned)col) * 4u, acc[r][i]);
+            }
+        }
+        return;
+    }
 #pragma unroll
     for (int i = 0; i < RM; ++i) {
         const int m = tm * BM + wm * 64 + i * 16 + fr;
@@ -265,7 +281,8 @@
 template <typename T>
 int linear_launch(const LinPlan &p, const pww_linear_desc_t *d, const void *x, const void *w, const void *bias, const void *residual, void *y, void *ws,
                   hipStream_t stream) {
-    LinCold cold{bias, residual, p.ys, p.rs, p.nsplit, p.nslab, d->epilogue, d->N / 2};
+    LinCold cold{bias, residual, p.ys, p.rs, p.nsplit, p.nslab, d->epilogue, d->N / 2,
+                 p.nsplit > 1 ? partial_stores_through((size_t)p.nsplit * d->M * d->N * sizeof(float)) : 0};
     const T *xt = static_cast<const T *>(x), *wt = static_cast<const T *>(w);
     const dim3 grid(p.ntiles * p.nsplit), block(LN_THREADS);
     void *out = p.nsplit == 1 ? y : ws;
diff --git a/paint-with-words-sd_amd/pww_hip/_lib.py b/paint-with-words-sd_amd/pww_hip/_lib.py
--- a/paint-with-words-sd_amd/pww_hip/_lib.py
+++ b/paint-with-words-sd_amd/pww_hip/_lib.py
@@ -14,6 +14,7 @@
 CANVAS_LIB_PATH = os.environ.get("PWW_HIP_CANVAS_LIB", os.path.join(_HERE, "libpww_hip_canvas.so"))
 CONCAT_LIB_PATH = os.environ.get("PWW_HIP_CONCAT_LIB", os.path.join(_HERE, "libpww_hip_concat.so"))
 HOLD_LIB_PATH = os.environ.get("PWW_HIP_HOLD_LIB", os.path.join(_HERE, "libpww_hip_hold.so"))
+CONVWIDE_LIB_PATH = os.environ.get("PWW_HIP_CONVWIDE_LIB", os.path.join(_HERE, "libpww_hip_convwide.so"))
 
 PWW_OK, PWW_EINVAL, PWW_ENOTSUP, PWW_EHIP = 0, -22, -95, -5
 MIN_VERSION = 127
@@ -78,6 +79,10 @@
                 "pww_hold_thresholds")
 HOLD_MIN_VERSION = 100
 HOLD_MAX_COLORS, HOLD_MAX_FEATHER, HOLD_MAX_RADIUS, HOLD_MAX_STEPS = 8, 8.0, 24, 100000
+
+
+CONVWIDE_EXPORTS = ("pww_convwide_version", "pww_convwide_last_error", "pww_convwide_takes", "pww_convwide_workspace_bytes", "pww_convwide_fwd")
+CONVWIDE_MIN_VERSION = 100
 
 
 class AttnDesc(ctypes.Structure):
@@ -332,6 +337,10 @@
         "pww_hold_apply": ([_vp, _vp, _vp, _vp, _f32, _f32, _f32, _i32, _i32, _i64, _vp], _int),
         "pww_hold_taps": ([_f32, _P(_f32), _i32], _int),
         "pww_hold_thresholds": ([_i32, _P(_f32)], _int)}),
+    "convwide": dict(path="CONVWIDE_LIB_PATH", exports=CONVWIDE_EXPORTS, min_version=CONVWIDE_MIN_VERSION, missing_ok=False, needs="the 160-wide tile of conv3x3 needs it", sigs={
+        "pww_convwide_takes": ([_P(ConvDesc)], _int),
+        "pww_convwide_workspace_bytes": ([_P(ConvDesc)], _sz),
+        "pww_convwide_fwd": ([_vp, _vp, _vp, _vp, _vp, _P(ConvDesc), _vp, _sz, _vp], _int)}),
 }
 _side = {}
 
@@ -417,6 +426,11 @@
     return lib if lib is not None else load_side("hold")
 
 
+def load_convwide():
+    lib = _side.get("convwide")
+    return lib if lib is not None else load_side("convwide")
+
+
 class experiments:
 
     def __enter__(self):
diff --git a/paint-with-words-sd_amd/pww_hip/ops.py b/paint-with-words-sd_amd/pww_hip/ops.py
--- a/paint-with-words-sd_amd/pww_hip/ops.py
+++ b/paint-with-words-sd_amd/pww_hip/ops.py
@@ -1036,7 +1036,7 @@
         return False
     B, C, H, W = x.shape
     Cout = weight.shape[0]
-    return (tuple(weight.shape[1:]) == (C, 3, 3) and C % 64 == 0 and Cout % 64 == 0 and stride in (1, 2) and not (upsample and stride != 1)
+    return (tuple(weight.shape[1:]) == (C, 3, 3) and C % 64 == 0 and (Cout % 64 == 0 or Cout % 160 == 0) and Cout >= 64 and stride in (1, 2) and not (upsample and stride != 1)
             and x.is_contiguous(memory_format=torch.channels_last) and x.data_ptr() % 16 == 0
             and B * H * W * C < 2 ** 31 // 4)
 
@@ -1060,11 +1060,19 @@
         residual = residual.contiguous(memory_format=torch.channels_last)
     d = _lib.ConvDesc(ctypes.sizeof(_lib.ConvDesc), _DT[x.dtype], B, H, W, C, Cout, int(stride), int(bool(upsample)), int(tile_n), int(splitk), 0)
     lib = _lib.load()
+    side = _lib.load_convwide()
+    wide = side.pww_convwide_takes(ctypes.byref(d)) == 1
+    ws_bytes, fwd, what = ((side.pww_convwide_workspace_bytes, side.pww_convwide_fwd, "pww_convwide_fwd") if wide else
+                           (lib.pww_conv3x3_workspace_bytes, lib.pww_conv3x3_fwd, "pww_conv3x3_fwd"))
     y = torch.empty((B, Cout, Ho, Wo), dtype=x.dtype, device=x.device, memory_format=torch.channels_last)
-    nbytes = int(lib.pww_conv3x3_workspace_bytes(ctypes.byref(d)))
+    nbytes = int(ws_bytes(ctypes.byref(d)))
     ws = torch.empty(nbytes // 4, dtype=torch.float32, device=x.device) if nbytes else None
     with torch.cuda.device(x.device):
-        _lib.check(lib.pww_conv3x3_fwd(_ptr(x), _ptr(w), _ptr(bias), _ptr(residual), _ptr(y), ctypes.byref(d), _ptr(ws), nbytes, _stream()), "pww_conv3x3_fwd")
+        rc = fwd(_ptr(x), _ptr(w), _ptr(bias), _ptr(residual), _ptr(y), ctypes.byref(d), _ptr(ws), nbytes, _stream())
+        if wide:
+            _lib.check(rc, what, side)
+        else:
+            _lib.check(rc, what)
     return y
 
 
```
